# GuoYi0/alphaFive

Hardware: AMD Instinct MI355X
Metric: self-play moves/sec (11x11, 500 sims/move) (higher is better)
Workload: dtype f32 (fp16x2 split operands: 3 fp16 MFMA products per MAC, fp32 accumulate)

## Files before the change

alphafive_amd/csrc/af_conv_f16s.h:

```cpp
#ifndef AF_CONV_F16S_H
#define AF_CONV_F16S_H

#include <hip/hip_runtime.h>

#include <map>
#include <string>
#include <vector>

struct f16s_net;

int f16s_supported(int board_size);
int f16s_create(f16s_net** out, int board_size, int max_batch, int device, const std::map<std::string, std::vector<float>>& vars);
void f16s_destroy(f16s_net* n);
int f16s_trunk(f16s_net* n, hipStream_t st, const float* planes_dev, int batch);
int f16s_value_branch(f16s_net* n, hipStream_t st, int batch, float* o3_dev, int WP, int PP, float* value);
int f16s_policy_branch(f16s_net* n, hipStream_t st, int batch, float* o5_dev, int WP, int PP, float* policy);
int f16s_small_branches_ok(const f16s_net* n, int batch);
int f16s_small_branches(f16s_net* n, hipStream_t st, int batch, float* value, float* policy);
int f16s_small_forward_ok(const f16s_net* n, int batch);
int f16s_small_forward(f16s_net* n, hipStream_t st, const float* planes_dev, int batch, float* value, float* policy);
int f16s_small_forward_error(f16s_net* n);
void f16s_set_ablation(f16s_net* n, int bits);
int f16s_read_activation(f16s_net* n, int which, int batch, float* host);

#endif
```

alphafive_amd/csrc/af_conv_f16s.hip:

```cpp
#include <hip/hip_runtime.h>
#include <stdint.h>
#include <stdio.h>
#include <stdlib.h>
#include <string.h>

#include <algorithm>
#include <atomic>
#include <cmath>
#include <map>
#include <string>
#include <vector>

#include "af_conv_f16s.h"

typedef _Float16 h8 __attribute__((ext_vector_type(8)));
typedef float f32x16 __attribute__((ext_vector_type(16)));
typedef float f32x4 __attribute__((ext_vector_type(4)));

#define FS_HIP_OK(x) do { hipError_t e_ = (x); if (e_ != hipSuccess) { fprintf(stderr, "[af_conv_f16s] %s failed: %s\n", #x, hipGetErrorString(e_)); return -2; } } while (0)

namespace {

template <int S_> struct Geo;
template <> struct Geo<11> {
// ... 92 lines not shown
}
__device__ __forceinline__ f32x2 elu2(f32x2 x) {
    const f32x2 t = x * 1.44269504088896341f;
    f32x2 e;
    e.x = fminf(fmaxf(__builtin_amdgcn_exp2f(t.x), 0.0f), 1.0f);
    e.y = fminf(fmaxf(__builtin_amdgcn_exp2f(t.y), 0.0f), 1.0f);
    const f32x2 em1 = e - 1.0f;
    return f32x2{fmaxf(x.x, em1.x), fmaxf(x.y, em1.y)};
}

#ifndef AF_F16S_XCD_SWIZZLE
#define AF_F16S_XCD_SWIZZLE 1
#endif
#ifdef AF_F16S_TIMING
__device__ unsigned long long g_f16s_cycles[10][512][4][9];
__device__ unsigned long long g_f16s_wall[10][512][2];
#define AF_T(var) const unsigned long long var = __builtin_readcyclecounter()
#define AF_TACC(slot, a, b) tacc[slot] += (b) - (a)
#else
#define AF_T(var)
#define AF_TACC(slot, a, b)
#endif

#ifdef AF_DF_TIMING
__device__ unsigned long long g_df_wall[256][5];
#define DF_T(i) if (threadIdx.x == 0 && blockIdx.x < 256) g_df_wall[blockIdx.x][i] = wall_clock64()
#else
#define DF_T(i)
#endif
__device__ __forceinline__ void df_signal(int* ctr) {
    DF_T(2);
    asm volatile("s_waitcnt vmcnt(0)" ::: "memory");
    __syncthreads();
    if (threadIdx.x == 0) __hip_atomic_fetch_add(ctr, 1, __ATOMIC_RELAXED, __HIP_MEMORY_SCOPE_AGENT);
    DF_T(3);
}
__device__ __forceinline__ void df_poll(const int* ctr, int need, int* err) {
    int it = 0;
    while (__hip_atomic_load(ctr, __ATOMIC_RELAXED, __HIP_MEMORY_SCOPE_AGENT) < need) {
        __builtin_amdgcn_s_sleep(2);
        if (++it > (1 << 22)) { __hip_atomic_store(err, 1, __ATOMIC_RELAXED, __HIP_MEMORY_SCOPE_AGENT); break; }
    }
}
__device__ __forceinline__ void df_wait_one(const int* ctr, int need, int* err) {
    if (threadIdx.x == 0) df_poll(ctr, need, err);
    DF_T(1);
    __syncthreads();
}
__device__ __forceinline__ void df_wait_inv(const int* ctr, int need, int* err) {
    if (threadIdx.x == 0) {
        df_poll(ctr, need, err);
        __builtin_amdgcn_fence(__ATOMIC_ACQUIRE, "agent");
    }
    DF_T(1);
    __syncthreads();
}

struct F16sArgs {
    const char* in;
    const char* in2;
    const uint4* w;
    const float* bias;
    char* out;
    float* out32;
    float inv_scale;
    const uint4* pw;
    float* pbuf;
    float inv_scale_p;
    const uint4* hw;
    const float* hbias;
    char* hx;
    float inv_scale_h;
    int batch, WP, PP;
    const uint4* w2;
    const float* bias2;
    float inv_scale2;
    int gx0;
    char* stash;
    const int* df_wait;
    int df_need;
    int* df_done;
    int* df_err;
    int abl;
};

template <class G, int NSM, int NSP, int CT, int KS, int PS, bool OUT32, bool XACC, int PJ, int HD, int DIST, int WPE, int NTW, int HSEL, int FU = 0, int DF = 0>
__device__ __forceinline__ void f16s_body(const F16sArgs& A, char* smem, const int bx, const int gxw, const int tb = 0,
                                          const int by = (int)blockIdx.y, const int gy = (int)gridDim.y) {
    using L = Lay<G>;
    constexpr uint32_t kRowH = L::kRowH, kHalfH = L::kHalfH, kSlabH = L::kSlabH, kRowL = L::kRowL, kHalfL = L::kHalfL, kSlotL = L::kSlotL;
    constexpr uint32_t kZoff = Lds<G, DIST>::kZoff, kBiasOff = Lds<G, DIST>::kBiasOff, kScrOff = Lds<G, DIST>::kScrOff;
    constexpr int kDist = DIST, kRing = DIST + 2;
    constexpr int NPC = G::NPC, HV = G::HALVES;
    static_assert(FU == 0 || (G::HALVES == 1 && PJ == 1 && HD == 0 && !OUT32 && NSP == 0 && CT == 1 && HSEL < 0 &&
                              ((KS == 1 && NTW == 1) || (KS == 2 && NTW == 2))), "fused block: see above");
    constexpr uint32_t kScrBytes = KS == 2 ? (uint32_t)(CT * PS * NTW) * 4096u * (PJ == 1 ? 2u : 1u) : 0u;
    constexpr uint32_t kGOff = Lds<G, DIST>::kScrOff;
    constexpr uint32_t kW2Off = kGOff + (kScrBytes > Lay<G>::kSlotL ? kScrBytes : Lay<G>::kSlotL);
    constexpr int NT = NTW;
    static_assert(HSEL < 0 || (HV == 2 && PJ == 0 && HD == 0 && !OUT32), "half classes: plain 15x15 layers only");
    static_assert(NT % KS == 0 || PJ == 0, "an odd tile count under a k-split has no projection exchange");
    constexpr int C16 = 2 / KS;
    constexpr int ITP = C16, ITM = 9 * C16;
    constexpr int NIT = NSP * ITP + NSM * ITM;
    constexpr int SPP = NSP + NSM;
    constexpr int NFIN = NT / KS;
    static_assert(CT * KS * PS == 4 && NT >= KS, "4 waves");
    static_assert(PJ == 0 || NSP == 0, "a producer / consumer of the separate projection has no projection slabs");
    constexpr int NPW = PJ == 1 ? NSM * C16 : 0;
    static_assert(NPC * (DIST > 1 ? DIST - 1 : 1) < 64, "vmcnt is a 6-bit field");
    static_assert(DIST >= 2 || (NSP == 0 && ITM - 1 >= NPC), "distance 1: a slab's pieces must all be issued before its predecessor's last item");
    const int lane = threadIdx.x & 63, kg = lane >> 5, nn = lane & 31;
    const int wv = __builtin_amdgcn_readfirstlane((int)(threadIdx.x >> 6));
    const int ct = wv % CT, ks = (wv / CT) % KS, ps = wv / (CT * KS);
    const int rot = KS == 2 ? ks * ((NT + 1) / 2) : 0;
#define AF_OWN(jj) (KS == 1 || (jj) < NT / 2 || ((jj) < (NT + 1) / 2 && ks == 0))
    const int ctg = by * CT + ct, nso = gy * CT;
    const uint32_t lds = (uint32_t)(uintptr_t)smem;

    const int nq = HSEL >= 0 ? A.batch : A.batch * HV;
    int qpos = bx;
    if (AF_F16S_XCD_SWIZZLE && (gxw & (8 * (HSEL >= 0 ? 1 : HV) - 1)) == 0) qpos = (bx >> 3) + (gxw >> 3) * (bx & 7);
    if (qpos >= nq) return;
    const int hv = HSEL >= 0 ? HSEL : (HV == 1 ? 0 : qpos % HV);
    const uint32_t wsrc = G::wbase(hv) * 16u;
    AF_T(t_entry);
#ifdef AF_F16S_TIMING
    const unsigned long long wall_entry = wall_clock64();
#endif

    auto slab_src = [&](int qq, int j) -> const char* {
        const int p_ = (HV == 1 || HSEL >= 0) ? qq : qq / HV;
        const int p = (A.abl & 0x1000) ? (p_ & 127) : p_;
        return (j < NSM ? A.in + ((size_t)p * NSM + j) * kSlabH : A.in2 + ((size_t)p * NSP + (j - NSM)) * kSlabH) + wsrc;
    };
    auto dma_piece = [&](const char* src, uint32_t slot_off, int k) {
        const int piece = wv + 4 * k, row = piece / G::PR;
        const uint32_t su = G::seg_unit(piece % G::PR) * 16u;
        const uint32_t offh = (uint32_t)(row >> 2) * kHalfH + (uint32_t)(row & 3) * kRowH + su;
        const uint32_t offl = (uint32_t)(row >> 2) * kHalfL + (uint32_t)(row & 3) * kRowL + su;
        if (DF != 0) glds16_sc1(src + offh + lane * 16, (uint32_t)__builtin_amdgcn_readfirstlane((int)(lds + kLds0 + slot_off + offl)));
        else glds16(src + offh + lane * 16, (uint32_t)__builtin_amdgcn_readfirstlane((int)(lds + kLds0 + slot_off + offl)));
    };
    const int q0 = qpos;
    auto stream_src = [&](uint32_t idx) -> const char* {
        const int p = q0 + (int)(idx / SPP) * gxw, j = (int)(idx % SPP);
        return slab_src(p, j);
    };
    const uint32_t nslabs = (uint32_t)((nq - q0 + gxw - 1) / gxw) * SPP;

    if (DF == 0) {
#pragma unroll
        for (int d = 0; d < kDist; ++d) {
            if ((uint32_t)d < nslabs) {
#pragma unroll
                for (int k = 0; k < NPC; ++k) dma_piece(stream_src(d), (uint32_t)d * kSlotL, k);
            }
        }
    }

    h8 W[2 * NIT];
    {
        const uint4* wp = A.w + ((size_t)(ctg * KS + ks) * (2 * NIT)) * 64 + lane;
#pragma unroll
        for (int f = 0; f < 2 * NIT; ++f) {
            const uint4 v = wp[f * 64];
            __builtin_memcpy(&W[f], &v, 16);
        }
    }
    h8 PW[PJ == 1 ? 2 * NPW : 1];
    if (PJ == 1) {
        const uint4* wp = A.pw + ((size_t)(ctg * KS + ks) * (2 * NPW)) * 64 + lane;
#pragma unroll
        for (int f = 0; f < 2 * NPW; ++f) {
            const uint4 v = wp[f * 64];
            __builtin_memcpy(&PW[f], &v, 16);
        }
    }
    constexpr int HDS = HD > 0 ? HD : FU;
    h8 HA[HDS > 0 ? 4 : 1];
    float hb[HDS > 0 ? 8 : 1];
    if (FU > 0) {
        const uint4* w2 = A.w2;
#pragma unroll
        for (int i = 0; i < 9; ++i) *reinterpret_cast<uint4*>(smem + kW2Off + (uint32_t)(i * 256 + (int)threadIdx.x) * 16u) = w2[i * 256 + threadIdx.x];
        if (threadIdx.x < 32) reinterpret_cast<float*>(smem + kBiasOff + 256u)[threadIdx.x] = A.bias2[threadIdx.x];
        if (KS == 1) {
            for (uint32_t u = threadIdx.x; u < kSlotL / 16; u += 256) *reinterpret_cast<uint4*>(smem + kGOff + u * 16) = uint4{0, 0, 0, 0};
        }
    }
    if (HDS > 0) {
#pragma unroll
        for (int f = 0; f < 4; ++f) {
            const uint4 v = A.hw[f * 64 + lane];
            __builtin_memcpy(&HA[f], &v, 16);
        }
#pragma unroll
        for (int r = 0; r < 8; ++r) hb[r] = A.hbias[8 * kg + r];
    }
    if (threadIdx.x < kLds0 / 16) *reinterpret_cast<uint4*>(smem + threadIdx.x * 16) = uint4{0, 0, 0, 0};
    if (G::PADL + G::PADR > 0) {
        static_assert(G::PADL + G::PADR == 0 || (G::PADL == 8 && G::PADR == 8), "pad zeroing is written for 8 + 8 units");
        for (uint32_t u = threadIdx.x; u < (uint32_t)kRing * 128u; u += 256) {
            const uint32_t off = kLds0 + (u >> 7) * kSlotL + ((u >> 4) & 7u) * kRowL + (((u >> 3) & 1u) ? (G::WINU - 8u) * 16u : 0u) + (u & 7u) * 16u;
            *reinterpret_cast<uint4*>(smem + off) = uint4{0, 0, 0, 0};
        }
    }
    for (uint32_t u = threadIdx.x; u < kSlotL / 16; u += 256) *reinterpret_cast<uint4*>(smem + kZoff + u * 16) = uint4{0, 0, 0, 0};
    if (threadIdx.x < CT * 32) reinterpret_cast<float*>(smem + kBiasOff)[threadIdx.x] = A.bias[by * CT * 32 + threadIdx.x];
    uint32_t lb[NT], zb[NT];
    int pix[NT];
    bool ok[NT], edgeL[NT], edgeR[NT];
#pragma unroll
    for (int jj = 0; jj < NT; ++jj) {
        const int n = 128 * hv + 32 * (tb + ps * NT + ((jj + rot) % NT)) + nn;
        ok[jj] = n < G::NPIX;
        const int nc = ok[jj] ? n : 128 * hv;
        pix[jj] = nc;
        const int x = nc % G::S;
        edgeL[jj] = x == 0; edgeR[jj] = x == G::S - 1;
        lb[jj] = kLds0 + (uint32_t)((KS == 2 ? 2 * ks : 0) + kg) * kRowL + (uint32_t)((nc + G::POFF - G::S - 1 - (int)G::wbase(hv)) * 16);
        zb[jj] = kZoff + (lb[jj] & 255u);
    }
    constexpr int kAccRegs = 16 * NT * (1 + (XACC ? 1 : 0) + (PJ == 1 ? 1 : 0));
    constexpr int kWRegs = 4 * (2 * NIT + (PJ == 1 ? 2 * NPW : 0) + (HDS > 0 ? 4 : 0));
    constexpr int kNAmax = (256 - kAccRegs - 16) / 4, kNAwant = (kWRegs - AF_F16S_VW + 3) / 4;
    constexpr int NA = (AF_F16S_APIN && WPE == 1 && kNAwant > 0) ? (kNAwant < kNAmax ? kNAwant : kNAmax) : 0;
#pragma unroll
    for (int f = 0; f < 2 * NIT; ++f) {
        if (f < 2 * NIT - NA) asm volatile("" : "+v"(W[f]));
        else asm volatile("" : "+a"(W[f]));
    }
// ... 16 lines not shown
        }
    }
    asm volatile("s_waitcnt vmcnt(0) lgkmcnt(0)" ::: "memory");
    __builtin_amdgcn_s_barrier();
    AF_T(t_ready);

    auto rd = [](const char* sm, bool proj, int it, int p, uint32_t c_, uint32_t l_, uint32_t r_) -> h8 {
        const int c = proj ? it : it / 9, tap = proj ? 4 : it % 9, ky = tap / 3, kx = tap % 3;
        const uint32_t base = kx == 0 ? l_ : (kx == 2 ? r_ : c_);
        const uint32_t imm = (uint32_t)p * kHalfL + (KS == 1 ? 2u * c * kRowL : 0u) + (uint32_t)(ky * G::S + kx) * 16u;
        return *reinterpret_cast<const h8*>(sm + base + imm);
    };

    auto head_tile = [&](const float (&v)[16], const int jj, const int pos) {
      if constexpr (HDS > 0) {
        h8 bh[2], bl[2];
#pragma unroll
        for (int st_ = 0; st_ < 2; ++st_)
#pragma unroll
            for (int e = 0; e < 8; ++e) {
                const float f = v[8 * st_ + e];
                const _Float16 h = (_Float16)f;
                bh[st_][e] = h;
                bl[st_][e] = (_Float16)(f - (float)h);
            }
        f32x16 a2;
#pragma unroll
        for (int r = 0; r < 16; ++r) a2[r] = 0.0f;
#pragma unroll
        for (int st_ = 0; st_ < 2; ++st_) {
            a2 = __builtin_amdgcn_mfma_f32_32x32x16_f16(HA[2 * st_], bh[st_], a2, 0, 0, 0);
            a2 = __builtin_amdgcn_mfma_f32_32x32x16_f16(HA[2 * st_], bl[st_], a2, 0, 0, 0);
            a2 = __builtin_amdgcn_mfma_f32_32x32x16_f16(HA[2 * st_ + 1], bh[st_], a2, 0, 0, 0);
        }
        constexpr int NR = HDS == 1 ? 4 : 8;
        _Float16 uh[8], ul[8];
#pragma unroll
        for (int r = 0; r < NR; ++r) {
            const float f = elu1(a2[r] * A.inv_scale_h + hb[r]);
            const _Float16 h = (_Float16)f;
            uh[r] = h;
            ul[r] = (_Float16)(f - (float)h);
        }
        if (ok[jj] && !(A.abl & 2)) {
            if (HDS == 1) {
                if (kg == 0) {
                    typedef _Float16 h4 __attribute__((ext_vector_type(4)));
                    char* o = A.hx + (size_t)pos * Hx<G>::kValPos + (uint32_t)pix[jj] * 8u;
                    if (DF != 0) {
                        st8_sc1(o, h4{uh[0], uh[1], uh[2], uh[3]});
                        st8_sc1(o + Hx<G>::kValLo, h4{ul[0], ul[1], ul[2], ul[3]});
                    } else {
                        *reinterpret_cast<h4*>(o) = h4{uh[0], uh[1], uh[2], uh[3]};
                        *reinterpret_cast<h4*>(o + Hx<G>::kValLo) = h4{ul[0], ul[1], ul[2], ul[3]};
                    }
                }
            } else {
                char* o = A.hx + (size_t)pos * Hx<G>::kPolPos + (uint32_t)pix[jj] * 32u + (uint32_t)kg * 16u;
                if (DF != 0) {
                    st16_sc1(o, h8{uh[0], uh[1], uh[2], uh[3], uh[4], uh[5], uh[6], uh[7]});
                    st16_sc1(o + Hx<G>::kPolLo, h8{ul[0], ul[1], ul[2], ul[3], ul[4], ul[5], ul[6], ul[7]});
                } else {
                    *reinterpret_cast<h8*>(o) = h8{uh[0], uh[1], uh[2], uh[3], uh[4], uh[5], uh[6], uh[7]};
                    *reinterpret_cast<h8*>(o + Hx<G>::kPolLo) = h8{ul[0], ul[1], ul[2], ul[3], ul[4], ul[5], ul[6], ul[7]};
                }
            }
        }
      }
    };
    uint32_t t = 0;
    uint32_t cur = 0u, nxd = (uint32_t)kDist * kSlotL;
    constexpr bool XPOS = !(NT >= 3 && NIT >= 36) && FU == 0;
    h8 fr[2][NT][2];
#define AF_FIRST_ITEM(slot)                                                                                      \
    _Pragma("unroll") for (int jj = 0; jj < NT; ++jj) {                                                          \
        const uint32_t c_ = (AF_F16S_ZPAD && !ok[jj]) ? zb[jj] : lb[jj] + (slot), l_ = edgeL[jj] ? zb[jj] : c_, r_ = edgeR[jj] ? zb[jj] : c_; \
        fr[0][jj][0] = rd(smem, false, 0, 0, c_, l_, r_);                                                        \
        fr[0][jj][1] = rd(smem, false, 0, 1, c_, l_, r_);                                                        \
    }
    if (XPOS) { AF_FIRST_ITEM(0u) }
#ifdef AF_F16S_TIMING
    unsigned long long tacc[8] = {0, 0, 0, 0, 0, 0, 0, 0};
#endif
    for (; qpos < nq; qpos += gxw) {
        const int pos = (HV == 1 || HSEL >= 0) ? qpos : qpos / HV;
        AF_T(tp0);
        if (!XPOS) { AF_FIRST_ITEM(cur) }
#undef AF_FIRST_ITEM
        f32x16 acc[NT], acx[XACC ? NT : 1], pac[PJ == 1 ? NT : 1];
#pragma unroll
        for (int jj = 0; jj < NT; ++jj)
#pragma unroll
            for (int r = 0; r < 16; ++r) { acc[jj][r] = 0.0f; if (XACC) acx[jj][r] = 0.0f; if (PJ == 1) pac[jj][r] = 0.0f; }
        f32x4 padd[PJ == 2 ? NFIN : 1][4];
        if (PJ == 2) {
#pragma unroll
            for (int jf = 0; jf < NFIN; ++jf) {
                const int tile = tb + ps * NT + (KS == 2 ? ks * NFIN : 0) + jf;
                const f32x4* src = reinterpret_cast<const f32x4*>(A.pbuf) + ((((size_t)qpos * nso + ctg) * 4 + tile) * 4) * 64 + lane;
#pragma unroll
                for (int q = 0; q < 4; ++q) padd[jf][q] = src[q * 64];
            }
        }

#pragma clang loop unroll(full)
        for (int j = 0; j < SPP; ++j) {
            const bool proj = j >= NSM;
            const bool nproj = (j + 1) % SPP >= NSM;
            const int ms = j, pslab = j - NSM;
            const int NI = proj ? ITP : ITM;
            const int ibase = proj ? pslab * ITP : NSP * ITP + ms * ITM;
            const int seq = proj ? NSM * ITM + pslab * ITP : ms * ITM;
            const int npos = qpos + ((j + kDist) / SPP) * gxw;
            const bool more = npos < nq && !(A.abl & 1);
            const char* nsrc = slab_src((A.abl & 4) ? q0 : (more ? npos : qpos), (j + kDist) % SPP);
            const uint32_t nx1 = cur + kSlotL == kRing * kSlotL ? 0u : cur + kSlotL;
            uint32_t bC[NT], bL[NT], bR[NT];
#pragma unroll
            for (int jj = 0; jj < NT; ++jj) {
                bC[jj] = (AF_F16S_ZPAD && !ok[jj]) ? zb[jj] : lb[jj] + cur;
                bL[jj] = edgeL[jj] ? zb[jj] : bC[jj];
                bR[jj] = edgeR[jj] ? zb[jj] : bC[jj];
            }
            if (HSEL == 1 && wv == (j & 3) && by == 0 && lane < 32) {
                const uint32_t u = (uint32_t)(lane & 3), un = (u < 2 ? 128u + u : 141u + u);
                const uint4 q = *reinterpret_cast<const uint4*>(smem + kLds0 + cur + (uint32_t)(lane >> 4) * kHalfL + (uint32_t)((lane >> 2) & 3) * kRowL + un * 16u);
                *reinterpret_cast<uint4*>(A.stash + (((size_t)pos * SPP + j) * 32 + lane) * 16) = q;
            }
#pragma clang loop unroll(full)
            for (int it = 0; it < NI; ++it) {
                const int b = (seq + it) & 1;
                if (it + 1 < NI) {
#pragma unroll
                    for (int jj = 0; jj < NT; ++jj) {
                        fr[b ^ 1][jj][0] = rd(smem, proj, it + 1, 0, bC[jj], bL[jj], bR[jj]);
                        fr[b ^ 1][jj][1] = rd(smem, proj, it + 1, 1, bC[jj], bL[jj], bR[jj]);
                    }
                } else {
                    const int issued = NI - 1 < NPC ? NI - 1 : NPC;
                    AF_T(tw0);
                    if (more) {
                        wait_vmcnt(NPC * (kDist - 2) + issued);
                    } else {
                        asm volatile("s_waitcnt vmcnt(0)" ::: "memory");
                    }
                    AF_T(tw1);
                    __builtin_amdgcn_s_barrier();
                    AF_T(tw2);
                    AF_TACC(1, tw0, tw1);
                    AF_TACC(2, tw1, tw2);
                    if ((XPOS || j + 1 < SPP) && t + 1 < nslabs) {
#pragma unroll
                        for (int jj = 0; jj < NT; ++jj) {
                            const uint32_t c_ = (AF_F16S_ZPAD && !ok[jj]) ? zb[jj] : lb[jj] + nx1, l_ = edgeL[jj] ? zb[jj] : c_, r_ = edgeR[jj] ? zb[jj] : c_;
                            fr[b ^ 1][jj][0] = rd(smem, nproj, 0, 0, c_, l_, r_);
                            fr[b ^ 1][jj][1] = rd(smem, nproj, 0, 1, c_, l_, r_);
                        }
                    }
                }
                const h8 wh = W[2 * (ibase + it)], wl = W[2 * (ibase + it) + 1];
#pragma unroll
                for (int jj = 0; jj < NT; ++jj) acc[jj] = __builtin_amdgcn_mfma_f32_32x32x16_f16(wh, fr[b][jj][0], acc[jj], 0, 0, 0);
                if (XACC) {
#pragma unroll
                    for (int jj = 0; jj < NT; ++jj) acx[jj] = __builtin_amdgcn_mfma_f32_32x32x16_f16(wh, fr[b][jj][1], acx[jj], 0, 0, 0);
#pragma unroll
                    for (int jj = 0; jj < NT; ++jj) acx[jj] = __builtin_amdgcn_mfma_f32_32x32x16_f16(wl, fr[b][jj][0], acx[jj], 0, 0, 0);
                } else {
#pragma unroll
                    for (int jj = 0; jj < NT; ++jj) acc[jj] = __builtin_amdgcn_mfma_f32_32x32x16_f16(wh, fr[b][jj][1], acc[jj], 0, 0, 0);
#pragma unroll
                    for (int jj = 0; jj < NT; ++jj) acc[jj] = __builtin_amdgcn_mfma_f32_32x32x16_f16(wl, fr[b][jj][0], acc[jj], 0, 0, 0);
                }
                if (PJ == 1 && !proj && it % 9 == 4) {
                    const int pi = ms * C16 + it / 9;
                    const h8 ph = PW[2 * pi], pl = PW[2 * pi + 1];
#pragma unroll
                    for (int jj = 0; jj < NT; ++jj) pac[jj] = __builtin_amdgcn_mfma_f32_32x32x16_f16(ph, fr[b][jj][0], pac[jj], 0, 0, 0);
#pragma unroll
                    for (int jj = 0; jj < NT; ++jj) pac[jj] = __builtin_amdgcn_mfma_f32_32x32x16_f16(ph, fr[b][jj][1], pac[jj], 0, 0, 0);
#pragma unroll
                    for (int jj = 0; jj < NT; ++jj) pac[jj] = __builtin_amdgcn_mfma_f32_32x32x16_f16(pl, fr[b][jj][0], pac[jj], 0, 0, 0);
                }
#pragma unroll
                for (int q = 0; q < 2 * NT; ++q) {
                    __builtin_amdgcn_sched_group_barrier(0x008, 1, 0);
                    __builtin_amdgcn_sched_group_barrier(0x100, 1, 0);
                }
                __builtin_amdgcn_sched_group_barrier(0x008, NT, 0);
                if (more) {
                    if (it < NI - 1 && it < NPC) dma_piece(nsrc, nxd, it);
                    if (it == NI - 1) {
#pragma unroll
                        for (int k = (NI - 1 < NPC ? NI - 1 : NPC); k < NPC; ++k) dma_piece(nsrc, nxd, k);
                    }
                }
            }
// ... 163 lines not shown
            {
                const f32x4* bp = reinterpret_cast<const f32x4*>(smem + kBiasOff + 256u + (uint32_t)(16 * kg) * 4u);
#pragma unroll
                for (int q = 0; q < 4; ++q) { const f32x4 v = bp[q]; bs2[4 * q] = v[0]; bs2[4 * q + 1] = v[1]; bs2[4 * q + 2] = v[2]; bs2[4 * q + 3] = v[3]; }
            }
#pragma unroll
            for (int r = 0; r < 16; r += 2) {
                f32x2 pre = f32x2{a2[r], a2[r + 1]} * A.inv_scale2 + f32x2{bs2[r], bs2[r + 1]};
                pre += f32x2{pj[r], pj[r + 1]};
                const f32x2 y = elu2(pre);
                v2[r] = y.x; v2[r + 1] = y.y;
            }
            head_tile(v2, 0, pos);
        }
#ifdef AF_F16S_TIMING
        {
            AF_T(tp3);
            tacc[3] += tp2 - tp1; tacc[4] += tp3 - tp2; tacc[5] += tp3 - tp0; tacc[6] += 1;
        }
#endif
    }
    if (DF != 0) df_signal(A.df_done + q0);
#ifdef AF_F16S_TIMING
    if (lane == 0) {
        tacc[0] = tacc[5] - tacc[1] - tacc[2] - tacc[3] - tacc[4];
        const int layer = (A.abl >> 8) & 15;
        for (int q = 0; q < 8; ++q) g_f16s_cycles[layer][blockIdx.x + 256 * blockIdx.y][wv][q] = tacc[q];
        g_f16s_cycles[layer][blockIdx.x + 256 * blockIdx.y][wv][8] = t_ready - t_entry;
        if (wv == 0) { g_f16s_wall[layer][blockIdx.x + 256 * blockIdx.y][0] = wall_entry; g_f16s_wall[layer][blockIdx.x + 256 * blockIdx.y][1] = wall_clock64(); }
    }
#endif
#undef AF_OWN
}

template <class G, int NSM, int NSP, int CT, int KS, int PS, bool OUT32, bool XACC, int PJ, int HD, int DIST = kDist, int WPE = 1>
__global__ __launch_bounds__(256, WPE) __attribute__((amdgpu_waves_per_eu(WPE, WPE))) void af_conv_f16s(F16sArgs A) {
    extern __shared__ __attribute__((aligned(16))) char smem[];
    f16s_body<G, NSM, NSP, CT, KS, PS, OUT32, XACC, PJ, HD, DIST, WPE, 4 / PS, -1>(A, smem, (int)blockIdx.x, (int)gridDim.x);
}

template <class G, int NSM, int KS, int PS, bool XACC, int FU, int DIST>
__global__ __launch_bounds__(256, 1) __attribute__((amdgpu_waves_per_eu(1, 1))) void af_block_f16s(F16sArgs A) {
    extern __shared__ __attribute__((aligned(16))) char smem[];
    f16s_body<G, NSM, 0, 1, KS, PS, false, XACC, 1, 0, DIST, 1, 4 / PS, -1, FU>(A, smem, (int)blockIdx.x, (int)gridDim.x);
}

template <class G>
__global__ __launch_bounds__(256, 1) __attribute__((amdgpu_waves_per_eu(1, 1))) void af_small_pair_f16s(F16sArgs P, F16sArgs V) {
    extern __shared__ __attribute__((aligned(16))) char smem[];
    const int nb = P.batch, id = (int)blockIdx.x;
    if (id < 2 * nb) f16s_body<G, 4, 0, 2, 2, 1, false, false, 0, 0, kDist, 1, 2, -1>(P, smem, id % nb, nb, (id / nb) * 2);
    else f16s_body<G, 4, 0, 1, 2, 2, false, false, 1, 0, 2, 1, 2, -1, 1>(V, smem, id - 2 * nb, nb);
}

template <class G>
__global__ __launch_bounds__(256, 1) __attribute__((amdgpu_waves_per_eu(1, 1))) void af_big_pair_f16s(F16sArgs P, F16sArgs V) {
    extern __shared__ __attribute__((aligned(16))) char smem[];
    const int gp = P.gx0, id = (int)blockIdx.x;
    if (id < gp) f16s_body<G, 4, 0, 2, 2, 1, false, false, 0, 0, kDist, 1, 4, -1>(P, smem, id, gp);
    else f16s_body<G, 4, 0, 1, 2, 2, false, false, 1, 0, 2, 1, 2, -1, 1>(V, smem, id - gp, (int)gridDim.x - gp);
}

template <class G, int NSM, int NSP, int CT, int KS, int PS, bool OUT32, bool XACC, int PJ, int HD, int DIST, int WPE, int NTW>
__global__ __launch_bounds__(256, WPE) __attribute__((amdgpu_waves_per_eu(WPE, WPE))) void af_conv_f16s_sb(F16sArgs A) {
    extern __shared__ __attribute__((aligned(16))) char smem[];
    f16s_body<G, NSM, NSP, CT, KS, PS, OUT32, XACC, PJ, HD, DIST, WPE, NTW, -1>(A, smem, (int)blockIdx.x, (int)gridDim.x, (int)blockIdx.z * PS * NTW);
}

template <class G, int NSM, int NSP, int CT, int KS, bool XACC>
__global__ __launch_bounds__(256, 1) __attribute__((amdgpu_waves_per_eu(1, 1))) void af_conv_f16s_h15(F16sArgs A) {
    extern __shared__ __attribute__((aligned(16))) char smem[];
    const int gx0 = A.gx0;
    if ((int)blockIdx.x < gx0) f16s_body<G, NSM, NSP, CT, KS, 1, false, XACC, 0, 0, kDist, 1, 4, 0>(A, smem, (int)blockIdx.x, gx0);
    else f16s_body<G, NSM, NSP, CT, KS, 1, false, XACC, 0, 0, kDist, 1, 3, 1>(A, smem, (int)blockIdx.x - gx0, (int)gridDim.x - gx0);
}

struct CornerArgs {
    const char* stash;
    const uint4* w;
    const float* bias;
    char* out;
    float inv_scale;
    int batch, NCT;
};
template <class G, int KS, bool XACC, int NSM, int NSP>
__global__ __launch_bounds__(256) void af_corner_f16s(CornerArgs A) {
    using L = Lay<G>;
    constexpr int CPIX = G::NPIX - 1;
    constexpr int C16 = 2 / KS, NIT = NSP * C16 + NSM * 9 * C16;
    constexpr int NST = NSM * 8 + NSP * 2;
    constexpr int D = NST < 12 ? NST : 12;
    const int lane = threadIdx.x & 63, kg = lane >> 5, nn = lane & 31;
    const int tile = (int)blockIdx.y * 4 + (int)(threadIdx.x >> 6);
    if (tile >= A.NCT) return;
    const int p = 32 * (int)blockIdx.x + nn;
    const bool valid = p < A.batch;
    const size_t pc = (size_t)(valid ? p : A.batch - 1);
    f32x16 acc[KS], acx[XACC ? KS : 1];
#pragma unroll
    for (int h = 0; h < KS; ++h)
#pragma unroll
        for (int r = 0; r < 16; ++r) { acc[h][r] = 0.0f; if (XACC) acx[h][r] = 0.0f; }
    const uint4* const wbase = A.w + (size_t)tile * KS * NIT * 2 * 64 + lane;
    constexpr int SPP = NSM + NSP;
    const char* const st0 = A.stash + (pc * SPP * 32 + (uint32_t)kg * 4u) * 16;
    struct Ops { uint4 a0, a1, b0, b1; };
    auto half_of = [](int t) constexpr -> int {
        const int k16 = t < NSM * 8 ? (t >> 2) & 1 : (t - NSM * 8) & 1;
        return KS == 2 ? k16 : 0;
    };
    auto fetch = [&](int t) -> Ops {
        int k16, item;
        const char* bsrc;
        if (t < NSM * 8) {
            const int s_ = t >> 3, tq = t & 3, ky = tq >> 1, kx = tq & 1;
            k16 = (t >> 2) & 1;
            item = NSP * C16 + s_ * 9 * C16 + (KS == 2 ? 0 : k16) * 9 + 3 * ky + kx;
            bsrc = st0 + (uint32_t)((s_ * 32 + 2 * k16 * 4 + tq) * 16);
        } else {
            const int u = t - NSM * 8, s_ = u >> 1;
            k16 = u & 1;
            item = s_ * C16 + (KS == 2 ? 0 : k16);
            bsrc = st0 + (uint32_t)(((NSM + s_) * 32 + 2 * k16 * 4 + 3) * 16);
        }
        const uint4* wp = wbase + ((size_t)((KS == 2 ? k16 : 0) * NIT + item) * 2) * 64;
        Ops o;
        o.a0 = wp[0]; o.a1 = wp[64];
        o.b0 = *reinterpret_cast<const uint4*>(bsrc); o.b1 = *reinterpret_cast<const uint4*>(bsrc + 256);
        return o;
    };
    Ops ring[D];
#pragma unroll
    for (int t = 0; t < D; ++t) ring[t] = fetch(t);
    __builtin_amdgcn_sched_barrier(0);
#pragma unroll
    for (int t = 0; t < NST; ++t) {
        const Ops o = ring[t % D];
        if (t + D < NST) ring[t % D] = fetch(t + D);
        const int h = half_of(t);
        h8 wh, wl, bh, bl;
        __builtin_memcpy(&wh, &o.a0, 16); __builtin_memcpy(&wl, &o.a1, 16); __builtin_memcpy(&bh, &o.b0, 16); __builtin_memcpy(&bl, &o.b1, 16);
        acc[h] = __builtin_amdgcn_mfma_f32_32x32x16_f16(wh, bh, acc[h], 0, 0, 0);
        if (XACC) {
            acx[h] = __builtin_amdgcn_mfma_f32_32x32x16_f16(wh, bl, acx[h], 0, 0, 0);
            acx[h] = __builtin_amdgcn_mfma_f32_32x32x16_f16(wl, bh, acx[h], 0, 0, 0);
        } else {
            acc[h] = __builtin_amdgcn_mfma_f32_32x32x16_f16(wh, bl, acc[h], 0, 0, 0);
            acc[h] = __builtin_amdgcn_mfma_f32_32x32x16_f16(wl, bh, acc[h], 0, 0, 0);
        }
        __builtin_amdgcn_sched_group_barrier(0x008, 3, 0);
        __builtin_amdgcn_sched_group_barrier(0x020, 4, 0);
    }
    if (XACC) {
#pragma unroll
        for (int h = 0; h < KS; ++h)
#pragma unroll
            for (int r = 0; r < 16; ++r) acc[h][r] += acx[h][r];
    }
    if (KS == 2) {
#pragma unroll
        for (int r = 0; r < 16; ++r) acc[0][r] = acc[KS - 1][r] + acc[0][r];
    }
    if (!valid) return;
    float v[16];
#pragma unroll
    for (int r = 0; r < 16; r += 2) {
        const f32x2 pre = f32x2{acc[0][r], acc[0][r + 1]} * A.inv_scale + f32x2{A.bias[32 * tile + 16 * kg + r], A.bias[32 * tile + 16 * kg + r + 1]};
        const f32x2 y = elu2(pre);
        v[r] = y.x; v[r + 1] = y.y;
    }
    char* o = A.out + ((size_t)p * A.NCT + tile) * L::kSlabH + (uint32_t)(2 * kg) * L::kRowH + (uint32_t)(CPIX + G::POFF) * 16u;
#pragma unroll
    for (int hf = 0; hf < 2; ++hf) {
        h8 hi, lo;
#pragma unroll
        for (int e = 0; e < 8; ++e) {
            const float f = v[8 * hf + e];
            const _Float16 h = (_Float16)f;
            hi[e] = h;
            lo[e] = (_Float16)(f - (float)h);
        }
        st16(o + hf * L::kRowH, hi);
        st16(o + hf * L::kRowH + L::kHalfH, lo);
    }
}

template <class G>
__global__ __launch_bounds__(256) void af_stem_f16s(const float* __restrict__ planes, const float* __restrict__ w,
                                                    const float* __restrict__ bias, char* __restrict__ out, int batch) {
    constexpr int S = G::S, NPIX = G::NPIX, SP = S + 4;
    constexpr uint32_t kRowH = Lay<G>::kRowH, kHalfH = Lay<G>::kHalfH, kSlabH = Lay<G>::kSlabH;
    __shared__ float sx[3 * SP * SP];
    __shared__ float sw[75 * 32];
    __shared__ float sb[32];
    const int t = threadIdx.x;
    for (int i = t; i < 75 * 32; i += 256) sw[i] = w[i];
    if (t < 32) sb[t] = bias[t];
    for (int i = t; i < 3 * SP * SP; i += 256) sx[i] = 0.0f;
    for (int b = blockIdx.x; b < batch; b += gridDim.x) {
        __syncthreads();
        for (int i = t; i < 3 * NPIX; i += 256) {
            const int c = i / NPIX, p = i - c * NPIX, y = p / S, x = p - y * S;
            sx[c * SP * SP + (y + 2) * SP + x + 2] = planes[(size_t)b * 3 * NPIX + i];
        }
        __syncthreads();
        if (t < NPIX) {
            const int y = t / S, x = t - y * S;
            float acc[32];
#pragma unroll
            for (int co = 0; co < 32; ++co) acc[co] = sb[co];
            for (int ky = 0; ky < 5; ++ky)
                for (int kx = 0; kx < 5; ++kx)
#pragma unroll
                    for (int c = 0; c < 3; ++c) {
                        const float xv = sx[c * SP * SP + (y + ky) * SP + x + kx];
                        const float* wr = sw + ((ky * 5 + kx) * 3 + c) * 32;
#pragma unroll
                        for (int co = 0; co < 32; ++co) acc[co] = fmaf(xv, wr[co], acc[co]);
                    }
            char* o = out + (size_t)b * kSlabH + (uint32_t)(t + G::POFF) * 16u;
#pragma unroll
            for (int u = 0; u < 4; ++u) {
                h8 hi, lo;
#pragma unroll
                for (int e = 0; e < 8; ++e) {
                    const float f = elu1(acc[8 * u + e]);
                    const _Float16 h = (_Float16)f;
                    hi[e] = h;
                    lo[e] = (_Float16)(f - (float)h);
                }
                *reinterpret_cast<h8*>(o + u * kRowH) = hi;
                *reinterpret_cast<h8*>(o + u * kRowH + kHalfH) = lo;
            }
        }
    }
}

template <class G> struct StemLds {
    static constexpr int SR = G::S + 4, IW = G::S + 5;
    static constexpr int kEnt = 3 * SR * G::S + 1, kImg = 3 * SR * IW;
    static constexpr uint32_t kImgOff = (uint32_t)((kEnt * 16 + 255) / 256 * 256), kBytes = kImgOff + (uint32_t)kImg * 2u;
};
template <class G, bool SC1 = false>
__device__ __forceinline__ void f16s_stem_body(const float* __restrict__ planes, const uint4* __restrict__ w ,
                                               const float* __restrict__ bias, float inv_scale, char* __restrict__ out, int batch,
                                               const int bx, const int gx, uint4* ent, _Float16* img) {
    constexpr int S = G::S, NPIX = G::NPIX, SR = S + 4, IW = S + 5;
    constexpr int NPL = 3 * NPIX, NLD = (NPL + 255) / 256;
    constexpr int NTL = (NPIX + 31) / 32, NRND = (NTL + 3) / 4;
    constexpr uint32_t kRowH = Lay<G>::kRowH, kHalfH = Lay<G>::kHalfH, kSlabH = Lay<G>::kSlabH;
    const int lane = threadIdx.x & 63, kg = lane >> 5, nn = lane & 31;
    const int wv = __builtin_amdgcn_readfirstlane((int)(threadIdx.x >> 6));
    h8 W[16];
#pragma unroll
    for (int f = 0; f < 16; ++f) {
        const uint4 v = w[f * 64 + lane];
        __builtin_memcpy(&W[f], &v, 16);
    }
    float bs[16];
#pragma unroll
    for (int r = 0; r < 16; ++r) bs[r] = bias[16 * kg + r];
    for (int i = threadIdx.x; i < 3 * SR * IW; i += 256) img[i] = (_Float16)0.0f;
    auto img_at = [](int i) -> int { const int c = i / NPIX, p = i - c * NPIX, y = p / S, x = p - y * S; return (c * SR + y + 2) * IW + x + 2; };
    int at[NLD];
    float nx[NLD];
#pragma unroll
    for (int q = 0; q < NLD; ++q) {
        const int i = (int)threadIdx.x + 256 * q;
        at[q] = img_at(i < NPL ? i : 0);
        nx[q] = 0.0f;
        if (i < NPL && bx < batch) nx[q] = planes[(size_t)bx * NPL + i];
    }
    for (int pos = bx; pos < batch; pos += gx) {
        __syncthreads();
#pragma unroll
        for (int q = 0; q < NLD; ++q)
            if ((int)threadIdx.x + 256 * q < NPL) img[at[q]] = (_Float16)nx[q];
        if (pos + gx < batch) {
            const float* pl = planes + (size_t)(pos + gx) * NPL;
#pragma unroll
            for (int q = 0; q < NLD; ++q)
                if ((int)threadIdx.x + 256 * q < NPL) nx[q] = pl[threadIdx.x + 256 * q];
        }
        __syncthreads();
        for (int en = threadIdx.x; en < 3 * SR * S; en += 256) {
            const int cin = en / (SR * S), rem = en - cin * SR * S, yy = rem / S, x = rem - yy * S;
            const _Float16* src = img + (cin * SR + yy) * IW + x;
            const h8 v = {src[0], src[1], src[2], src[3], src[4], 0, 0, 0};
            __builtin_memcpy(&ent[en], &v, 16);
        }
        __syncthreads();
#pragma unroll
        for (int rd_ = 0; rd_ < NRND; ++rd_) {
            const int n = 32 * (wv + 4 * rd_) + nn;
            const bool ok = n < NPIX;
            const int nc = ok ? n : 0;
            if (32 * (wv + 4 * rd_) >= NPIX) continue;
            f32x16 acc;
#pragma unroll
            for (int r = 0; r < 16; ++r) acc[r] = 0.0f;
#pragma unroll
            for (int s_ = 0; s_ < 8; ++s_) {
                const int ga = 2 * s_, gb = 2 * s_ + 1 < 15 ? 2 * s_ + 1 : 0;
                const uint32_t offa = (uint32_t)((ga / 5) * SR + ga % 5) * S, offb = (uint32_t)((gb / 5) * SR + gb % 5) * S;
                h8 b;
                __builtin_memcpy(&b, &ent[(uint32_t)nc + (kg ? offb : offa)], 16);
                acc = __builtin_amdgcn_mfma_f32_32x32x16_f16(W[2 * s_], b, acc, 0, 0, 0);
                acc = __builtin_amdgcn_mfma_f32_32x32x16_f16(W[2 * s_ + 1], b, acc, 0, 0, 0);
            }
            char* o = out + (size_t)pos * kSlabH + (uint32_t)(2 * kg) * kRowH + (uint32_t)(nc + G::POFF) * 16u;
#pragma unroll
            for (int hf = 0; hf < 2; ++hf) {
                h8 hi, lo;
#pragma unroll
                for (int e = 0; e < 8; ++e) {
                    const float f = elu1(acc[8 * hf + e] * inv_scale + bs[8 * hf + e]);
                    const _Float16 h = (_Float16)f;
                    hi[e] = h;
                    lo[e] = (_Float16)(f - (float)h);
                }
                if (ok) {
                    if (SC1) { st16_sc1(o + hf * kRowH, hi); st16_sc1(o + hf * kRowH + kHalfH, lo); }
                    else {
                        *reinterpret_cast<h8*>(o + hf * kRowH) = hi;
                        *reinterpret_cast<h8*>(o + hf * kRowH + kHalfH) = lo;
                    }
                }
            }
        }
    }
}

template <class G>
__global__ __launch_bounds__(256) void af_stem_mfma_f16s(const float* __restrict__ planes, const uint4* __restrict__ w, const float* __restrict__ bias,
                                                         float inv_scale, char* __restrict__ out, int batch) {
    __shared__ __attribute__((aligned(16))) uint4 ent[StemLds<G>::kEnt];
    __shared__ _Float16 img[StemLds<G>::kImg];
    f16s_stem_body<G>(planes, w, bias, inv_scale, out, batch, (int)blockIdx.x, (int)gridDim.x, ent, img);
}

template <class G>
__device__ __forceinline__ void f16s_vfc_body(const char* __restrict__ xv, const uint4* __restrict__ a, const float* __restrict__ b1,
                                              const float* __restrict__ w2, const float* __restrict__ b2, float inv_scale,
                                              float* __restrict__ value, int batch, const int bx) {
    __shared__ float red[2][32];
    constexpr int NS = Hx<G>::VSTEPS;
    const bool act = threadIdx.x < 128;
    const int lane = threadIdx.x & 63, mt = (threadIdx.x >> 6) & 1, n = lane & 31, kg = lane >> 5;
    const int pos = bx * 32 + n, posc = pos < batch ? pos : batch - 1;
    const char* xb = xv + (size_t)posc * Hx<G>::kValPos + (uint32_t)kg * 16u;
    const uint4* ap = a + (size_t)mt * 128 + lane;
    f32x16 acc;
#pragma unroll
    for (int r = 0; r < 16; ++r) acc[r] = 0.0f;
#pragma unroll
    for (int half = 0; half < (NS + 15) / 16; ++half) {
        uint4 bh[16], bl[16], ah[16], al[16];
#pragma unroll
        for (int q = 0; q < 16; ++q) {
            const int s_ = 16 * half + q;
            if (s_ < NS) {
                bh[q] = *reinterpret_cast<const uint4*>(xb + s_ * 32);
                bl[q] = *reinterpret_cast<const uint4*>(xb + Hx<G>::kValLo + s_ * 32);
                ah[q] = ap[(size_t)s_ * 256];
                al[q] = ap[(size_t)s_ * 256 + 64];
            }
        }
        typedef uint32_t u32x4 __attribute__((ext_vector_type(4)));
#pragma unroll
        for (int q = 0; q < 16; ++q) {
            if (16 * half + q < NS) {
                u32x4 t0, t1, t2, t3;
                __builtin_memcpy(&t0, &bh[q], 16); __builtin_memcpy(&t1, &bl[q], 16); __builtin_memcpy(&t2, &ah[q], 16); __builtin_memcpy(&t3, &al[q], 16);
                asm volatile("" : "+v"(t0), "+v"(t1), "+v"(t2), "+v"(t3));
                __builtin_memcpy(&bh[q], &t0, 16); __builtin_memcpy(&bl[q], &t1, 16); __builtin_memcpy(&ah[q], &t2, 16); __builtin_memcpy(&al[q], &t3, 16);
            }
        }
#pragma unroll
        for (int q = 0; q < 16; ++q) {
            if (16 * half + q < NS) {
                h8 xh, xl, wh, wl;
                __builtin_memcpy(&xh, &bh[q], 16); __builtin_memcpy(&xl, &bl[q], 16);
                __builtin_memcpy(&wh, &ah[q], 16); __builtin_memcpy(&wl, &al[q], 16);
                acc = __builtin_amdgcn_mfma_f32_32x32x16_f16(wh, xh, acc, 0, 0, 0);
                acc = __builtin_amdgcn_mfma_f32_32x32x16_f16(wh, xl, acc, 0, 0, 0);
                acc = __builtin_amdgcn_mfma_f32_32x32x16_f16(wl, xh, acc, 0, 0, 0);
            }
        }
    }
    float part = 0.0f;
#pragma unroll
    for (int r = 0; r < 16; ++r) {
        const int j = 32 * mt + 16 * kg + r;
        part += elu1(acc[r] * inv_scale + b1[j]) * w2[j];
    }
    part += __shfl_xor(part, 32);
    if (act && kg == 0) red[mt][n] = part;
    __syncthreads();
    if (act && mt == 0 && kg == 0 && pos < batch) value[pos] = tanhf((red[0][n] + red[1][n] + b2[0]) * 0.5f);
}
template <class G>
__global__ __launch_bounds__(128) __attribute__((amdgpu_waves_per_eu(1, 2))) void af_value_fc_f16s(
    const char* __restrict__ xv, const uint4* __restrict__ a , const float* __restrict__ b1, const float* __restrict__ w2,
    const float* __restrict__ b2, float inv_scale, float* __restrict__ value, int batch) {
    f16s_vfc_body<G>(xv, a, b1, w2, b2, inv_scale, value, batch, (int)blockIdx.x);
}
struct VfcArgs { const char* xv; const uint4* a; const float *b1, *w2, *b2; float inv_scale; float* value; };
template <class G>
__global__ __launch_bounds__(256, 1) __attribute__((amdgpu_waves_per_eu(1, 1))) void af_small_l7v_f16s(F16sArgs P, VfcArgs V) {
    extern __shared__ __attribute__((aligned(16))) char smem[];
    const int nb = P.batch, id = (int)blockIdx.x;
    if (id < 2 * nb) f16s_body<G, 2, 4, 2, 2, 1, false, true, 0, 0, kDist, 1, 2, -1>(P, smem, id % nb, nb, (id / nb) * 2);
    else f16s_vfc_body<G>(V.xv, V.a, V.b1, V.w2, V.b2, V.inv_scale, V.value, nb, id - 2 * nb);
}
template <class G>
__global__ __launch_bounds__(256, 1) __attribute__((amdgpu_waves_per_eu(1, 1))) void af_big_l7v_f16s(F16sArgs P, VfcArgs V) {
    extern __shared__ __attribute__((aligned(16))) char smem[];
    const int gp = P.gx0, id = (int)blockIdx.x;
    if (id < gp) f16s_body<G, 2, 4, 2, 2, 1, false, true, 0, 0, kDist, 1, 4, -1>(P, smem, id, gp);
    else f16s_vfc_body<G>(V.xv, V.a, V.b1, V.w2, V.b2, V.inv_scale, V.value, P.batch, id - gp);
}
// ... 412 lines not shown
int launch_cfg(hipStream_t st, const F16sArgs& a, int gy, int ncu) {
    constexpr int NT = 4 / PS;
    constexpr size_t lds = Lds<G, DIST>::kScrOff + (KS == 2 ? (size_t)CT * PS * NT * 4096 * (PJ == 1 ? 2 : 1) : 0);
    static_assert(WPE * lds <= 160 * 1024, "LDS budget of the workgroups sharing a CU");
#ifndef AF_F16S_NO_LDS_ASSERT
    static_assert(lds <= 160 * 1024, "LDS budget");
#endif
    static std::atomic<uint64_t> attr_devs{0};
    int dev = 0;
    FS_HIP_OK(hipGetDevice(&dev));
    const uint64_t bit = 1ull << (dev & 63);
    if (!(attr_devs.load(std::memory_order_relaxed) & bit)) {
        FS_HIP_OK(hipFuncSetAttribute(reinterpret_cast<const void*>(af_conv_f16s<G, NSM, NSP, CT, KS, PS, OUT32, XACC, PJ, HD, DIST, WPE>),
                                      hipFuncAttributeMaxDynamicSharedMemorySize, 160 * 1024));
        attr_devs.fetch_or(bit, std::memory_order_relaxed);
    }
    constexpr int NTS = KS == 2 ? 2 : 1;
    if constexpr (NTS < NT && HD == 0) {
        if (a.batch <= kSmallBatch && !(a.abl & 128)) {
            static std::atomic<uint64_t> attr_sb{0};
            if (!(attr_sb.load(std::memory_order_relaxed) & bit)) {
                FS_HIP_OK(hipFuncSetAttribute(reinterpret_cast<const void*>(af_conv_f16s_sb<G, NSM, NSP, CT, KS, PS, OUT32, XACC, PJ, HD, DIST, WPE, NTS>),
                                              hipFuncAttributeMaxDynamicSharedMemorySize, 160 * 1024));
                attr_sb.fetch_or(bit, std::memory_order_relaxed);
            }
            hipLaunchKernelGGL((af_conv_f16s_sb<G, NSM, NSP, CT, KS, PS, OUT32, XACC, PJ, HD, DIST, WPE, NTS>),
                               dim3(a.batch * G::HALVES, gy, NT / NTS), dim3(256), lds, st, a);
            FS_HIP_OK(hipGetLastError());
            return 0;
        }
    }
    int gx = std::max(1, std::min(a.batch * G::HALVES, WPE * ncu / gy));
    gx = std::max(G::HALVES, gx / G::HALVES * G::HALVES);
    hipLaunchKernelGGL((af_conv_f16s<G, NSM, NSP, CT, KS, PS, OUT32, XACC, PJ, HD, DIST, WPE>), dim3(gx, gy), dim3(256), lds, st, a);
    FS_HIP_OK(hipGetLastError());
    return 0;
}

template <class G, int NSM, int KS, int PS, bool XACC, int FU>
int launch_block(hipStream_t st, const F16sArgs& a, int ncu) {
    constexpr int DIST = 2;
    constexpr size_t scr = KS == 2 ? (size_t)PS * (4 / PS) * 4096 * 2 : 0;
    constexpr size_t lds = Lds<G, DIST>::kScrOff + (scr > Lay<G>::kSlotL ? scr : Lay<G>::kSlotL) + 36864;
    static_assert(lds <= 160 * 1024, "LDS budget of the fused block");
    static std::atomic<uint64_t> attr_devs{0};
    int dev = 0;
    FS_HIP_OK(hipGetDevice(&dev));
    const uint64_t bit = 1ull << (dev & 63);
    if (!(attr_devs.load(std::memory_order_relaxed) & bit)) {
        FS_HIP_OK(hipFuncSetAttribute(reinterpret_cast<const void*>(af_block_f16s<G, NSM, KS, PS, XACC, FU, DIST>),
                                      hipFuncAttributeMaxDynamicSharedMemorySize, 160 * 1024));
        attr_devs.fetch_or(bit, std::memory_order_relaxed);
    }
    const int gx = std::max(1, std::min(a.batch, ncu));
    hipLaunchKernelGGL((af_block_f16s<G, NSM, KS, PS, XACC, FU, DIST>), dim3(gx), dim3(256), lds, st, a);
    FS_HIP_OK(hipGetLastError());
    return 0;
}

template <class G, int NSM, int NSP, int CT, int KS, bool XACC>
int launch_h15(hipStream_t st, F16sArgs a, int gy, int ncu) {
    constexpr size_t lds = Lds<G, kDist>::kScrOff + (KS == 2 ? (size_t)CT * 4 * 4096 : 0);
    static_assert(lds <= 160 * 1024, "LDS budget");
    static std::atomic<uint64_t> attr_devs{0};
    int dev = 0;
    FS_HIP_OK(hipGetDevice(&dev));
    const uint64_t bit = 1ull << (dev & 63);
    if (!(attr_devs.load(std::memory_order_relaxed) & bit)) {
        FS_HIP_OK(hipFuncSetAttribute(reinterpret_cast<const void*>(af_conv_f16s_h15<G, NSM, NSP, CT, KS, XACC>),
                                      hipFuncAttributeMaxDynamicSharedMemorySize, 160 * 1024));
        attr_devs.fetch_or(bit, std::memory_order_relaxed);
    }
    const int gx = std::max(16, ncu / gy / 16 * 16);
    static const int num1 = [] { const char* e = getenv("AF_F16S_H15_NUM1"); const int v = e ? atoi(e) : 0; return v > 0 && v < 32 ? v : 18; }();
    static const int num2 = [] { const char* e = getenv("AF_F16S_H15_NUM2"); const int v = e ? atoi(e) : 0; return v > 0 && v < 32 ? v : 17; }();
    static const int rnd = [] { const char* e = getenv("AF_F16S_H15_ROUND"); return e ? atoi(e) : 1; }();
    const int num = KS == 1 ? num1 : num2;
    a.gx0 = rnd ? std::max(8, (gx * num / 32 + 4) / 8 * 8) : std::max(1, gx * num / 32);
    if (a.gx0 >= gx) a.gx0 = gx - 8;
    hipLaunchKernelGGL((af_conv_f16s_h15<G, NSM, NSP, CT, KS, XACC>), dim3(gx, gy), dim3(256), lds, st, a);
    FS_HIP_OK(hipGetLastError());
    CornerArgs c;
    c.stash = a.stash; c.w = a.w; c.bias = a.bias; c.out = a.out; c.inv_scale = a.inv_scale;
    c.batch = a.batch; c.NCT = gy * CT;
    hipLaunchKernelGGL((af_corner_f16s<G, KS, XACC, NSM, NSP>), dim3((a.batch + 31) / 32, (c.NCT + 3) / 4), dim3(256), 0, st, c);
    FS_HIP_OK(hipGetLastError());
    return 0;
}

}

struct f16s_net {
    int S = 11;
    int max_batch = 0, device = 0, ncu = 256;
    std::vector<void*> allocs;
    float *stem_w = nullptr, *stem_b = nullptr;
    uint4* stem_wm = nullptr;
    float stem_inv_scale = 1.0f;
    uint4* w[10] = {};
    uint4* pw[10] = {};
    float* pbuf[5] = {};
    float* bias[10] = {};
    float inv_scale[10] = {}, inv_scale_p[10] = {};
    char *f0 = nullptr, *g[5] = {}, *o[5] = {};
    uint4 *hcw[2] = {}, *hfw[2] = {};
    float *hcb[2] = {}, *hfb[2] = {}, *v2w = nullptr, *v2b = nullptr;
    float hc_inv[2] = {}, hf_inv[2] = {};
    char* hx[2] = {};
    int* df = nullptr;
    float* pfx = nullptr;
    char* stash = nullptr;
    int abl = 0;
};

int f16s_supported(int board_size) { return board_size == 11 || board_size == 15; }

int f16s_create(f16s_net** out, int board_size, int max_batch, int device, const std::map<std::string, std::vector<float>>& V) {
    if (!f16s_supported(board_size)) return -1;
    FS_HIP_OK(hipSetDevice(device));
    f16s_net* n = new f16s_net();
    n->S = board_size; n->max_batch = max_batch; n->device = device;
    const bool s11 = board_size == 11;
    const int halves = s11 ? 1 : 2;
    const size_t slab_bytes = s11 ? Lay<Geo<11>>::kSlabH : Lay<Geo<15>>::kSlabH;
    FS_HIP_OK(hipDeviceGetAttribute(&n->ncu, hipDeviceAttributeMultiprocessorCount, device));
    if (const char* e = getenv("AF_F16S_NCU")) {
        const int v = atoi(e);
        if (v >= 8 && v <= n->ncu) n->ncu = v / 8 * 8;
    }
    int rc = 0;
    auto get = [&](const std::string& k) -> const std::vector<float>& { return V.at(k); };
    rc = dev_upload(n->allocs, &n->stem_w, get("bone/conv1/kernel").data(), 75 * 32 * 4);
    if (!rc) rc = dev_upload(n->allocs, &n->stem_b, get("bone/conv1/bias").data(), 32 * 4);
    if (!rc) {
        const std::vector<float>& ks = get("bone/conv1/kernel");
        const float sc = pick_scale(ks, nullptr);
        std::vector<_Float16> pk((size_t)8 * 2 * 64 * 8, (_Float16)0.0f);
        for (int s_ = 0; s_ < 8; ++s_)
            for (int lane = 0; lane < 64; ++lane)
                for (int e = 0; e < 5; ++e) {
                    const int m = lane & 31, g = 2 * s_ + (lane >> 5);
                    if (g >= 15) continue;
                    const int co = 16 * ((m >> 2) & 1) + 8 * (m >> 4) + 4 * ((m >> 3) & 1) + (m & 3), cin = g / 5, ky = g % 5;
                    const float v = ks[(size_t)((ky * 5 + e) * 3 + cin) * 32 + co] * sc;
                    const _Float16 h = (_Float16)v;
                    pk[(((size_t)s_ * 2 + 0) * 64 + lane) * 8 + e] = h;
                    pk[(((size_t)s_ * 2 + 1) * 64 + lane) * 8 + e] = (_Float16)(v - (float)h);
                }
        rc = dev_upload(n->allocs, &n->stem_wm, pk.data(), pk.size() * 2);
        n->stem_inv_scale = 1.0f / sc;
    }
    for (int b = 0; b < 5 && !rc; ++b) {
        const std::string s = kBlockNames[b];
        const std::vector<float>&k1 = get(s + "_conv1/kernel"), &k2 = get(s + "_conv2/kernel"), &kr = get(s + "_res/kernel");
        const LayerCfg &L1 = kLayers[2 * b], &L2 = kLayers[2 * b + 1];
        const bool split_proj = L1.pj == 1;
        const float s1 = pick_scale(k1, nullptr), s2 = pick_scale(k2, split_proj ? nullptr : &kr);
        const std::vector<_Float16> p1 = pack_layer(L1, k1.data(), nullptr, s1), p2 = pack_layer(L2, k2.data(), kr.data(), s2);
        rc = dev_upload(n->allocs, &n->w[2 * b], p1.data(), p1.size() * 2);
        if (!rc && split_proj) {
            const float sp = pick_scale(kr, nullptr);
            const std::vector<_Float16> pp = pack_proj(L1, L2.cout, kr.data(), sp);
            rc = dev_upload(n->allocs, &n->pw[2 * b], pp.data(), pp.size() * 2);
            n->inv_scale_p[2 * b] = 1.0f / sp;
            void* q = nullptr;
            const size_t bytes = (size_t)max_batch * halves * (L2.cout / 32) * 4 * 4 * 64 * 16;
            if (!rc) { FS_HIP_OK(hipMalloc(&q, bytes)); n->allocs.push_back(q); n->pbuf[b] = (float*)q; }
        }

        if (!rc) rc = dev_upload(n->allocs, &n->w[2 * b + 1], p2.data(), p2.size() * 2);
        std::vector<float> bsum(get(s + "_conv2/bias"));
        for (size_t i = 0; i < bsum.size(); ++i) bsum[i] += get(s + "_res/bias")[i];
        if (!rc) rc = dev_upload(n->allocs, &n->bias[2 * b], get(s + "_conv1/bias").data(), L1.cout * 4);
        if (!rc) rc = dev_upload(n->allocs, &n->bias[2 * b + 1], bsum.data(), L2.cout * 4);
        n->inv_scale[2 * b] = 1.0f / s1; n->inv_scale[2 * b + 1] = 1.0f / s2;
    }
    auto act = [&](char** p, int ch) -> int {
        void* q = nullptr;
        const size_t bytes = (size_t)max_batch * (ch / 32) * slab_bytes;
        FS_HIP_OK(hipMalloc(&q, bytes));
        FS_HIP_OK(hipMemset(q, 0, bytes));
        n->allocs.push_back(q);
        *p = (char*)q;
        return 0;
    };
    if (!rc && !s11) {
        void* q = nullptr;
        FS_HIP_OK(hipMalloc(&q, (size_t)max_batch * 6 * 512));
        n->allocs.push_back(q);
        n->stash = (char*)q;
    }
    if (!rc) {
        void* q = nullptr;
        FS_HIP_OK(hipMalloc(&q, kDfWords * sizeof(int)));
        FS_HIP_OK(hipMemset(q, 0, kDfWords * sizeof(int)));
        n->allocs.push_back(q);
        n->df = (int*)q;
        FS_HIP_OK(hipMalloc(&q, 4 * 4 * 64 * 16));
        n->allocs.push_back(q);
        n->pfx = (float*)q;
    }
    if (!rc) rc = act(&n->f0, 32);
    for (int b = 0; b < 5 && !rc; ++b) {
        rc = act(&n->g[b], kLayers[2 * b].cout);
        if (!rc && b != 2 && b != 4) rc = act(&n->o[b], kLayers[2 * b + 1].cout);
    }
    if (!rc) {
        const int npix = board_size * board_size, hxp = 128 * halves, vsteps = (npix + 3) / 4, nlt = (npix + 31) / 32;
        const char* cname[2] = {"value/conv", "policy/conv"};
        const int nco[2] = {4, 16};
        for (int h = 0; h < 2 && !rc; ++h) {
            const std::vector<float>& wc = get(std::string(cname[h]) + "/kernel");
            const float sc = pick_scale(wc, nullptr);
            const int NC = nco[h];
            const std::vector<_Float16> pk = pack_frags(2, [&](int st_, int lane, int e) -> float {
                const int m = lane & 31, co = m < 16 ? 8 * ((m >> 2) & 1) + 4 * (m >> 3) + (m & 3) : 99, ci = 16 * (lane >> 5) + 8 * st_ + e;
                return co < NC ? wc[(size_t)ci * NC + co] * sc : 0.0f;
            });
            rc = dev_upload(n->allocs, &n->hcw[h], pk.data(), pk.size() * 2);
            std::vector<float> bpad(16, 0.0f);
            const std::vector<float>& bc = get(std::string(cname[h]) + "/bias");
            for (int i = 0; i < NC; ++i) bpad[i] = bc[i];
            if (!rc) rc = dev_upload(n->allocs, &n->hcb[h], bpad.data(), 64);
            n->hc_inv[h] = 1.0f / sc;
            void* q = nullptr;
            const size_t bytes = (size_t)max_batch * hxp * (h == 0 ? 16 : 64);
            if (!rc) { FS_HIP_OK(hipMalloc(&q, bytes)); FS_HIP_OK(hipMemset(q, 0, bytes)); n->allocs.push_back(q); n->hx[h] = (char*)q; }
        }
        if (!rc) {
            const std::vector<float>& w1 = get("value/fc1/kernel");
            const float sc = pick_scale(w1, nullptr);
            const std::vector<_Float16> pk = pack_frags(vsteps * 2, [&](int f, int lane, int e) -> float {
                const int s_ = f >> 1, mt = f & 1, px = 4 * s_ + 2 * (lane >> 5) + (e >> 2), ch = e & 3, j = 32 * mt + row_perm(lane & 31);
                return px < npix ? w1[(size_t)(ch * npix + px) * 64 + j] * sc : 0.0f;
            });
            rc = dev_upload(n->allocs, &n->hfw[0], pk.data(), pk.size() * 2);
            n->hf_inv[0] = 1.0f / sc;
            if (!rc) rc = dev_upload(n->allocs, &n->hfb[0], get("value/fc1/bias").data(), 64 * 4);
            if (!rc) rc = dev_upload(n->allocs, &n->v2w, get("value/fc2/kernel").data(), 64 * 4);
            if (!rc) rc = dev_upload(n->allocs, &n->v2b, get("value/fc2/bias").data(), 4);
        }
        if (!rc) {
            const std::vector<float>& wf = get("policy/fc/kernel");
            const float sc = pick_scale(wf, nullptr);
            const std::vector<_Float16> pk = pack_frags(npix * nlt, [&](int f, int lane, int e) -> float {
                const int px = f / nlt, mt = f % nlt, c16 = 8 * (lane >> 5) + e, j = 32 * mt + row_perm(lane & 31);
                return j < npix ? wf[(size_t)(c16 * npix + px) * npix + j] * sc : 0.0f;
            });
            rc = dev_upload(n->allocs, &n->hfw[1], pk.data(), pk.size() * 2);
            n->hf_inv[1] = 1.0f / sc;
            if (!rc) rc = dev_upload(n->allocs, &n->hfb[1], get("policy/fc/bias").data(), npix * 4);
        }
        if (!rc) FS_HIP_OK(hipFuncSetAttribute(reinterpret_cast<const void*>(af_policy_fc_f16s<Geo<11>>), hipFuncAttributeMaxDynamicSharedMemorySize, (int)kPfLds));
        if (!rc) FS_HIP_OK(hipFuncSetAttribute(reinterpret_cast<const void*>(af_policy_fc_f16s<Geo<15>>), hipFuncAttributeMaxDynamicSharedMemorySize, (int)kPfLds));
    }
    if (rc) { f16s_destroy(n); return rc; }
    *out = n;
    return 0;
}

void f16s_destroy(f16s_net* n) {
    if (!n) return;
    (void)hipSetDevice(n->device);
    for (void* p : n->allocs) (void)hipFree(p);
    delete n;
}

void f16s_set_ablation(f16s_net* n, int bits) { if (n) n->abl = bits; }

template <class G>
static int launch_layer_g(f16s_net* n, hipStream_t st, int li, const F16sArgs& a, int head) {
    switch (li) {
        case 0:
            if constexpr (G::S == 11) { if (!(n->abl & 32)) return launch_cfg<G, 1, 0, 2, 1, 2, false, false, 0, 0, 1, 2>(st, a, 1, n->ncu); }
            return launch_cfg<G, 1, 0, 2, 1, 2, false, true>(st, a, 1, n->ncu);
        case 1: return launch_cfg<G, 2, 1, 2, 1, 2, false, true>(st, a, 1, n->ncu);
        case 2:
            if constexpr (G::S == 15) { if (!(n->abl & 64) && a.batch >= 128) return launch_h15<G, 2, 0, 4, 1, false>(st, a, 1, n->ncu); }
            return launch_cfg<G, 2, 0, 4, 1, 1, false, false>(st, a, 1, n->ncu);
        case 3:
            if constexpr (G::S == 15) { if (!(n->abl & 64) && a.batch >= 128) return launch_h15<G, 4, 2, 2, 2, false>(st, a, 2, n->ncu); }
            return launch_cfg<G, 4, 2, 2, 2, 1, false, false>(st, a, 2, n->ncu);
        case 4: return launch_cfg<G, 4, 0, 1, 2, 2, false, false, 1>(st, a, 1, n->ncu);
        case 5:
            if constexpr (G::S == 11) { if (head == 0 && !(n->abl & 32)) return launch_cfg<G, 1, 0, 1, 1, 4, true, true, 2, 1, 1, 2>(st, a, 1, n->ncu); }
            if (head == 0) return launch_cfg<G, 1, 0, 1, 1, 4, true, true, 2, 1>(st, a, 1, n->ncu);
            return launch_cfg<G, 1, 0, 1, 1, 4, true, true, 2>(st, a, 1, n->ncu);
        case 6:
            if constexpr (G::S == 15) { if (!(n->abl & 64) && a.batch >= 128) return launch_h15<G, 4, 0, 2, 2, false>(st, a, 1, n->ncu); }
            return launch_cfg<G, 4, 0, 2, 2, 1, false, false>(st, a, 1, n->ncu);
        case 7:
            if constexpr (G::S == 15) { if (!(n->abl & 64) && a.batch >= 128) return launch_h15<G, 2, 4, 2, 2, true>(st, a, 1, n->ncu); }
            return launch_cfg<G, 2, 4, 2, 2, 1, false, true>(st, a, 1, n->ncu);
        case 8: return launch_cfg<G, 2, 0, 1, 1, 4, false, true, 1>(st, a, 1, n->ncu);
        default:
            if constexpr (G::S == 11) { if (head == 1 && !(n->abl & 32)) return launch_cfg<G, 1, 0, 1, 1, 4, true, true, 2, 2, 1, 2>(st, a, 1, n->ncu); }
            if (head == 1) return launch_cfg<G, 1, 0, 1, 1, 4, true, true, 2, 2>(st, a, 1, n->ncu);
            return launch_cfg<G, 1, 0, 1, 1, 4, true, true, 2>(st, a, 1, n->ncu);
    }
}

static int launch_layer(f16s_net* n, hipStream_t st, int li, const char* in, const char* in2, char* out, float* out32, int batch,
                        int WP, int PP, int head = -1) {
    F16sArgs a;
    a.hw = nullptr; a.hbias = nullptr; a.hx = nullptr; a.inv_scale_h = 1.0f;
    if (head >= 0) { a.hw = n->hcw[head]; a.hbias = n->hcb[head]; a.hx = n->hx[head]; a.inv_scale_h = n->hc_inv[head]; }
    a.in = in; a.in2 = in2; a.w = n->w[li]; a.bias = n->bias[li]; a.out = out; a.out32 = out32;
    a.inv_scale = n->inv_scale[li]; a.batch = batch; a.WP = WP; a.PP = PP; a.abl = (n->abl & 0xf0ff) | (li << 8); a.gx0 = 0; a.stash = n->stash;
    {
        static const int mask = [] { const char* e = getenv("AF_F16S_ABL_LAYERS"); return e ? (int)strtol(e, nullptr, 0) : 0x3ff; }();
        if (!((mask >> li) & 1)) a.abl &= ~0x100f;
    }
    a.w2 = nullptr; a.bias2 = nullptr; a.inv_scale2 = 1.0f;
    a.pw = n->pw[li]; a.pbuf = n->pbuf[li / 2]; a.inv_scale_p = n->inv_scale_p[li];
    return n->S == 11 ? launch_layer_g<Geo<11>>(n, st, li, a, head) : launch_layer_g<Geo<15>>(n, st, li, a, head);
}

int f16s_trunk(f16s_net* n, hipStream_t st, const float* planes, int batch) {
    if (!n || batch < 1 || batch > n->max_batch) return -1;
    if (n->abl & 16) {
        if (n->S == 15) hipLaunchKernelGGL(af_stem_f16s<Geo<15>>, dim3(std::min(batch, 2048)), dim3(256), 0, st, planes, n->stem_w, n->stem_b, n->f0, batch);
        else hipLaunchKernelGGL(af_stem_f16s<Geo<11>>, dim3(std::min(batch, 2048)), dim3(256), 0, st, planes, n->stem_w, n->stem_b, n->f0, batch);
    } else if (n->S == 15) {
        hipLaunchKernelGGL(af_stem_mfma_f16s<Geo<15>>, dim3(std::min(batch, 1024)), dim3(256), 0, st, planes, n->stem_wm, n->stem_b, n->stem_inv_scale,
                           n->f0, batch);
    } else {
        hipLaunchKernelGGL(af_stem_mfma_f16s<Geo<11>>, dim3(std::min(batch, 1024)), dim3(256), 0, st, planes, n->stem_wm, n->stem_b, n->stem_inv_scale,
                           n->f0, batch);
    }
    int rc = launch_layer(n, st, 0, n->f0, nullptr, n->g[0], nullptr, batch, 0, 0);
    if (!rc) rc = launch_layer(n, st, 1, n->g[0], n->f0, n->o[0], nullptr, batch, 0, 0);
    if (!rc) rc = launch_layer(n, st, 2, n->o[0], nullptr, n->g[1], nullptr, batch, 0, 0);
    if (!rc) rc = launch_layer(n, st, 3, n->g[1], n->o[0], n->o[1], nullptr, batch, 0, 0);
    return rc;
}

static F16sArgs block_args(f16s_net* n, int li, const char* in, int batch, int head) {
    F16sArgs a;
    memset(&a, 0, sizeof(a));
    a.in = in; a.w = n->w[li]; a.bias = n->bias[li]; a.inv_scale = n->inv_scale[li];
    a.pw = n->pw[li]; a.inv_scale_p = n->inv_scale_p[li];
    a.w2 = n->w[li + 1]; a.bias2 = n->bias[li + 1]; a.inv_scale2 = n->inv_scale[li + 1];
    a.hw = n->hcw[head]; a.hbias = n->hcb[head]; a.hx = n->hx[head]; a.inv_scale_h = n->hc_inv[head];
    a.batch = batch; a.abl = (n->abl & 0xf0ff) | (li << 8); a.stash = n->stash;
    return a;
}

int f16s_value_branch(f16s_net* n, hipStream_t st, int batch, float* o3, int WP, int PP, float* value) {
    int rc;
    if (n->S == 11 && value && !(n->abl & 256)) {
        rc = launch_block<Geo<11>, 4, 2, 2, false, 1>(st, block_args(n, 4, n->o[1], batch, 0), n->ncu);
    } else {
        rc = launch_layer(n, st, 4, n->o[1], nullptr, n->g[2], nullptr, batch, 0, 0);
        if (!rc) rc = launch_layer(n, st, 5, n->g[2], n->o[1], nullptr, o3, batch, WP, PP, value ? 0 : -1);
    }
    if (!rc && value) {
        if (n->S == 11)
            hipLaunchKernelGGL(af_value_fc_f16s<Geo<11>>, dim3((batch + 31) / 32), dim3(128), 0, st, n->hx[0], n->hfw[0], n->hfb[0], n->v2w, n->v2b,
                               n->hf_inv[0], value, batch);
        else
            hipLaunchKernelGGL(af_value_fc_f16s<Geo<15>>, dim3((batch + 31) / 32), dim3(128), 0, st, n->hx[0], n->hfw[0], n->hfb[0], n->v2w, n->v2b,
                               n->hf_inv[0], value, batch);
    }
    return rc;
}

int f16s_policy_branch(f16s_net* n, hipStream_t st, int batch, float* o5, int WP, int PP, float* policy) {
    int rc = launch_layer(n, st, 6, n->o[1], nullptr, n->g[3], nullptr, batch, 0, 0);
    if (!rc) rc = launch_layer(n, st, 7, n->g[3], n->o[1], n->o[3], nullptr, batch, 0, 0);
    if (!rc && n->S == 11 && policy && !(n->abl & 256)) {
        rc = launch_block<Geo<11>, 2, 1, 4, true, 2>(st, block_args(n, 8, n->o[3], batch, 1), n->ncu);
    } else {
        if (!rc) rc = launch_layer(n, st, 8, n->o[3], nullptr, n->g[4], nullptr, batch, 0, 0);
        if (!rc) rc = launch_layer(n, st, 9, n->g[4], n->o[3], nullptr, o5, batch, WP, PP, policy ? 1 : -1);
    }
    if (!rc && policy) {
        if (n->S == 11)
            hipLaunchKernelGGL(af_policy_fc_f16s<Geo<11>>, dim3((batch + kPfPos - 1) / kPfPos), dim3(512), kPfLds, st, n->hx[1], n->hfw[1], n->hfb[1],
                               n->hf_inv[1], policy, batch);
        else
            hipLaunchKernelGGL(af_policy_fc_f16s<Geo<15>>, dim3((batch + kPfPos - 1) / kPfPos), dim3(512), kPfLds, st, n->hx[1], n->hfw[1], n->hfb[1],
                               n->hf_inv[1], policy, batch);
    }
    return rc;
}

int f16s_small_branches(f16s_net* n, hipStream_t st, int batch, float* value, float* policy) {
    if (!n || n->S != 11 || batch < 1 || !value || !policy) return -1;
    using G = Geo<11>;
    const bool small = batch <= kSmallBatch;
    F16sArgs P;
    memset(&P, 0, sizeof(P));
    P.in = n->o[1]; P.w = n->w[6]; P.bias = n->bias[6]; P.out = n->g[3]; P.inv_scale = n->inv_scale[6];
    P.batch = batch; P.abl = (n->abl & 0xf0ff) | (6 << 8); P.stash = n->stash; P.inv_scale2 = 1.0f; P.inv_scale_h = 1.0f;
    const F16sArgs V = block_args(n, 4, n->o[1], batch, 0);
    constexpr size_t ldsP = Lds<G, kDist>::kScrOff + (size_t)2 * 1 * 4 * 4096;
    constexpr size_t ldsV = Lds<G, 2>::kScrOff + (size_t)2 * 2 * 4096 * 2 + 36864;
    constexpr size_t lds = ldsP > ldsV ? ldsP : ldsV;
    static_assert(lds <= 160 * 1024, "LDS budget");
    static std::atomic<uint64_t> attr_devs{0};
    int dev = 0;
    FS_HIP_OK(hipGetDevice(&dev));
    const uint64_t bit = 1ull << (dev & 63);
    if (!(attr_devs.load(std::memory_order_relaxed) & bit)) {
        FS_HIP_OK(hipFuncSetAttribute(reinterpret_cast<const void*>(af_small_pair_f16s<G>), hipFuncAttributeMaxDynamicSharedMemorySize, 160 * 1024));
        FS_HIP_OK(hipFuncSetAttribute(reinterpret_cast<const void*>(af_big_pair_f16s<G>), hipFuncAttributeMaxDynamicSharedMemorySize, 160 * 1024));
        attr_devs.fetch_or(bit, std::memory_order_relaxed);
    }
    const int gp = std::max(1, std::min(batch, n->ncu));
    if (small) {
        hipLaunchKernelGGL(af_small_pair_f16s<G>, dim3(3 * batch), dim3(256), lds, st, P, V);
    } else {
        P.gx0 = gp;
        hipLaunchKernelGGL(af_big_pair_f16s<G>, dim3(2 * gp), dim3(256), lds, st, P, V);
    }
    FS_HIP_OK(hipGetLastError());
    {
        F16sArgs Q;
        memset(&Q, 0, sizeof(Q));
        Q.in = n->g[3]; Q.in2 = n->o[1]; Q.w = n->w[7]; Q.bias = n->bias[7]; Q.out = n->o[3]; Q.inv_scale = n->inv_scale[7];
        Q.batch = batch; Q.abl = (n->abl & 0xf0ff) | (7 << 8); Q.stash = n->stash; Q.inv_scale2 = 1.0f; Q.inv_scale_h = 1.0f;
        const VfcArgs F = {n->hx[0], n->hfw[0], n->hfb[0], n->v2w, n->v2b, n->hf_inv[0], value};
        constexpr size_t lds7 = Lds<G, kDist>::kScrOff + (size_t)2 * 1 * 4 * 4096;
        static std::atomic<uint64_t> attr7{0};
        if (!(attr7.load(std::memory_order_relaxed) & bit)) {
            FS_HIP_OK(hipFuncSetAttribute(reinterpret_cast<const void*>(af_small_l7v_f16s<G>), hipFuncAttributeMaxDynamicSharedMemorySize, (int)lds7));
            FS_HIP_OK(hipFuncSetAttribute(reinterpret_cast<const void*>(af_big_l7v_f16s<G>), hipFuncAttributeMaxDynamicSharedMemorySize, (int)lds7));
            attr7.fetch_or(bit, std::memory_order_relaxed);
        }
        if (small) {
            hipLaunchKernelGGL(af_small_l7v_f16s<G>, dim3(2 * batch + 1), dim3(256), lds7, st, Q, F);
        } else {
            Q.gx0 = gp;
            hipLaunchKernelGGL(af_big_l7v_f16s<G>, dim3(gp + (batch + 31) / 32), dim3(256), lds7, st, Q, F);
        }
        FS_HIP_OK(hipGetLastError());
    }
    int rc = launch_block<G, 2, 1, 4, true, 2>(st, block_args(n, 8, n->o[3], batch, 1), n->ncu);
    if (!rc) hipLaunchKernelGGL(af_policy_fc_f16s<G>, dim3((batch + kPfPos - 1) / kPfPos), dim3(512), kPfLds, st, n->hx[1], n->hfw[1], n->hfb[1],
                                n->hf_inv[1], policy, batch);
    FS_HIP_OK(hipGetLastError());
    return rc;
}

int f16s_small_forward_ok(const f16s_net* n, int batch) {
    return n && n->S == 11 && batch >= 1 && batch <= kSmallBatch && !(n->abl & (16 | 32 | 128 | 256 | 512 | 2048));
}
static F16sArgs layer_args(f16s_net* n, int li, const char* in, const char* in2, char* out, int batch) {
    F16sArgs a;
    memset(&a, 0, sizeof(a));
    a.in = in; a.in2 = in2; a.w = n->w[li]; a.bias = n->bias[li]; a.out = out; a.inv_scale = n->inv_scale[li]; a.batch = batch;
    a.abl = (n->abl & 0xf0ff) | (li << 8); a.stash = n->stash; a.inv_scale2 = 1.0f; a.inv_scale_h = 1.0f;
    a.pw = n->pw[li]; a.pbuf = n->pbuf[li / 2]; a.inv_scale_p = n->inv_scale_p[li];
    return a;
}
int f16s_small_forward(f16s_net* n, hipStream_t st, const float* planes, int batch, float* value, float* policy) {
    if (!f16s_small_forward_ok(n, batch) || !planes || !value || !policy) return -1;
    using G = Geo<11>;
    SmallFwdArgs S;
    memset(&S, 0, sizeof(S));
    S.planes = planes; S.stem_w = n->stem_wm; S.stem_b = n->stem_b; S.stem_inv = n->stem_inv_scale; S.f0 = n->f0;
    S.df = n->df; S.batch = batch;
    auto role = [&](F16sArgs a, int wait, int need, int done) { a.df_wait = n->df + wait; a.df_need = need; a.df_done = n->df + done; a.df_err = n->df + kDfErr; return a; };
    S.L0 = role(layer_args(n, 0, n->f0, nullptr, n->g[0], batch), kDfStem, 1, kDfL0);
    S.L1 = role(layer_args(n, 1, n->g[0], n->f0, n->o[0], batch), kDfL0, 2, kDfL1);
    S.L2 = role(layer_args(n, 2, n->o[0], nullptr, n->g[1], batch), kDfL1, 2, kDfL2);
    S.L3 = role(layer_args(n, 3, n->g[1], n->o[0], n->o[1], batch), kDfL2, 4, kDfL3);
    S.P = role(layer_args(n, 6, n->o[1], nullptr, n->g[3], batch), kDfL3, 4, kDfP);
    S.P.pw = nullptr; S.P.pbuf = nullptr;
    S.V = role(block_args(n, 4, n->o[1], batch, 0), kDfL3, 4, kDfV);
    S.Q = role(layer_args(n, 7, n->g[3], n->o[1], n->o[3], batch), kDfP, 2, kDfQ);
    S.Q.pw = nullptr; S.Q.pbuf = nullptr;
    S.B5 = role(block_args(n, 8, n->o[3], batch, 1), kDfQ, 2, kDfB5);
    S.F = VfcArgs{n->hx[0], n->hfw[0], n->hfb[0], n->v2w, n->v2b, n->hf_inv[0], value};
    constexpr size_t ldsC = Lds<G, kDist>::kScrOff + (size_t)2 * 1 * 4 * 4096;
    constexpr size_t ldsV = Lds<G, 2>::kScrOff + (size_t)2 * 2 * 4096 * 2 + 36864;
    constexpr size_t ldsB = Lds<G, 2>::kScrOff + Lay<G>::kSlotL + 36864;
    constexpr size_t lds = std::max(std::max(ldsC, ldsV), std::max(ldsB, (size_t)StemLds<G>::kBytes));
    static_assert(lds + 256 <= 160 * 1024, "LDS budget (dynamic + the value head's static reduction buffer)");
    static std::atomic<uint64_t> attr_devs{0};
    int dev = 0;
    FS_HIP_OK(hipGetDevice(&dev));
    const uint64_t bit = 1ull << (dev & 63);
    if (!(attr_devs.load(std::memory_order_relaxed) & bit)) {
        FS_HIP_OK(hipFuncSetAttribute(reinterpret_cast<const void*>(af_small_forward_f16s<G>), hipFuncAttributeMaxDynamicSharedMemorySize, (int)lds));
        attr_devs.fetch_or(bit, std::memory_order_relaxed);
    }
    S.xp = n->hx[1]; S.pfa = n->hfw[1]; S.pfb = n->hfb[1]; S.pf_inv = n->hf_inv[1]; S.policy = policy; S.pfx = n->pfx;
    hipLaunchKernelGGL(af_small_forward_f16s<G>, dim3(19 * batch + 3), dim3(256), lds, st, S);
    FS_HIP_OK(hipGetLastError());
    return 0;
}
int f16s_small_forward_error(f16s_net* n) {
    if (!n || !n->df) return -1;
    int e = 0;
    FS_HIP_OK(hipDeviceSynchronize());
    FS_HIP_OK(hipMemcpy(&e, n->df + kDfErr, sizeof(int), hipMemcpyDeviceToHost));
    return e;
}
int f16s_small_branches_ok(const f16s_net* n, int batch) {
    if (!n || n->S != 11 || (n->abl & 256)) return 0;
    return batch <= kSmallBatch ? !(n->abl & (128 | 512)) : !(n->abl & 1024);
}

// ... 42 lines not shown
```

alphafive_amd/csrc/af_engine.hip:

```cpp

#include <hip/hip_runtime.h>
#include <stdint.h>
#include <stdio.h>
#include <stdlib.h>
#include <string.h>

#include <type_traits>
#include <vector>

#include "af_engine.h"
#include "af_noise.h"

typedef unsigned long long u64;

enum { PH_IDLE = 0, PH_MOVE_START = 1, PH_SEARCH = 2, PH_MOVE_DONE = 3, PH_ERROR = 4, PH_DESCENT = 5  };
enum { CT_SIMS = 0, CT_SELECTS, CT_EXPANDS, CT_TERMINALS, CT_PLIES, CT_EPISODES, CT_LSUM, CT_LEXP,
       CT_GC, CT_GC_SCANNED, CT_YIELDS, CT_STALLS, CT_N };
enum { HIST_WORK = 0, HIST_TIME = 64, HIST_MAXTIME = 96, HIST_N = 97 };

struct EngineParams {
    int G, S, C, goal, sims, upper, training, mode, node_cap, max_ply, budget, budget_hard;
    uint32_t hash_mask;
    double init_temp, tau_decay, tau_decay_r, alpha, c_puct;
    float c_puct32;
// ... 738 lines not shown
            }
            uint32_t slot = 0xffffffffu;
            int idx;
            if (hint) {
                idx = hint - 1;
            } else {
                idx = tree_lookup<KW>(P, g, cm, ctb, lane, &slot);
                if (idx >= 0 && pidx >= 0 && lane == 0) ec[(size_t)pidx * CP + pcl] = idx + 1;
            }
            if (idx < 0) {
                if constexpr (MEMO) {
                    if (slot != 0xffffffffu && bb_count<KW>(cm) + bb_count<KW>(ctb) <= P.memo_max_stones) {
                        uint32_t unused;
                        const int me = memo_probe<KW>(P, memo_bucket<KW>(P, cm, ctb, last), cm, ctb, last, lane, &unused);
                        ++memo_probes;
                        if (me >= 0) {
                            ++memo_hits;
#pragma unroll
                            for (int k = 0; k < KW; ++k) { lm[k] = cm[k]; lt[k] = ctb[k]; }
                            c_depth = depth; c_slot = slot;
                            c_pol = P.memo_pv + (size_t)me * CP;
                            c_val = P.memo_val + me;
                            have_eval = true;
                            break;
                        }
                    }
                }
                if (lane < 2 * KW) P.leaf[(size_t)g * 2 * KW + lane] = key_word<KW>(cm, ctb, lane);
                if (lane == 0) { P.depth[g] = depth; P.leaf_last[g] = last; P.leaf_slot[g] = (int32_t)slot; }
                float* out = planes_out + (size_t)g * 3 * C;
#pragma unroll
                for (int k = 0; k < KW; ++k) {
                    const int c = lane + 64 * k;
                    if (c < C) {
                        out[c] = ((cm[k] >> lane) & 1ull) ? 1.0f : 0.0f;
                        out[C + c] = ((ctb[k] >> lane) & 1ull) ? 1.0f : 0.0f;
                        out[2 * C + c] = c == last ? 1.0f : 0.0f;
                    }
                }
                status = AF_STATUS_NEED_EVAL;
                parked = true;
                break;
            }
            if (work >= P.budget_hard) {
                if (lane < 2 * KW) P.leaf[(size_t)g * 2 * KW + lane] = key_word<KW>(cm, ctb, lane);
                if (lane == 0) { P.depth[g] = depth; P.leaf_last[g] = last; }
                phase = PH_DESCENT; status = AF_STATUS_YIELD; parked = true; ct[CT_YIELDS]++;
                break;
            }
            TK_T(tk_b);
            TK_ACC(3, tk_a, tk_b);
            const bool is_root = depth == 0;
            u64 legal[KW];
#pragma unroll
            for (int k = 0; k < KW; ++k) legal[k] = ~(cm[k] | ctb[k]) & P.boardmask[k];
            if (!r_have) {
                r_sum = nsum[idx];
#pragma unroll
                for (int k = 0; k < KW; ++k) {
                    const size_t off = (size_t)idx * CP + lane + 64 * k;
                    r_raw[k] = en[off];
                    r_c[k] = ec[off];
                    if constexpr (W64) r_w[k] = ew64[off]; else r_w[k] = ew[off];
                    r_p[k] = ep[off];
                }
            }
            r_have = false;
            const int sum_n = rfli(r_sum) + 1;
            if (lane == 0) nsum[idx] = sum_n;
            const uint32_t sel_id = sel++;
            int nn[KW];
            float pp[KW];
            wrow_t ww[KW];
            bool ff[KW];
            int32_t cc[KW];
#pragma unroll
            for (int k = 0; k < KW; ++k) {
                nn[k] = r_raw[k] & 0x7fffffff;
                ff[k] = r_raw[k] < 0;
                cc[k] = r_c[k];
                ww[k] = r_w[k];
                pp[k] = r_p[k];
            }
            double dd[KW];
            if (P.training) {
#ifdef AF_TICK_TIMING
                int tk_myit = 0;
#endif
                {
                    const float a_ = (float)P.alpha, inv_a = 1.0f / a_, one_m_a = 1.0f - a_;
                    uint32_t todo = 0;
#pragma unroll
                    for (int k = 0; k < KW; ++k) { dd[k] = 0.0; todo |= ((legal[k] >> lane) & 1ull) ? (1u << k) : 0u; }
                    af_u32x4 rk[KW];
                    uint32_t pend = 0;
#pragma unroll
                    for (int k = 0; k < KW; ++k) {
                        rk[k] = af_philox4x32(sel_id, episode, (AF_STREAM_GAMMA << 24) | (uint32_t)(lane + 64 * k), 0u, k0, k1);
                        float X;
                        const int ok = af_gamma_round(a_, inv_a, one_m_a, rk[k].v[0], rk[k].v[1], &X);
                        const bool lg = (todo >> k) & 1u;
                        dd[k] = (lg && ok) ? (double)X : 0.0;
                        pend |= (lg && !ok) ? (1u << k) : 0u;
                        if (KW > 2 && (k & 1)) __builtin_amdgcn_sched_barrier(0);
                    }
#ifdef AF_TICK_TIMING
                    ++tk_myit;
#endif
                    todo = pend;
                    {
                    uint32_t it = 1;
                    af_u32x4 r = rk[0];
#pragma unroll
                    for (int q = 1; q < KW; ++q) if (!(todo & ((1u << q) - 1u))) r = rk[q];
                    while (todo) {
#ifdef AF_TICK_TIMING
                        ++tk_myit;
#endif
                        const int k = __builtin_ctz(todo);
                        if ((it & 1u) == 0u) r = af_philox4x32(sel_id, episode, (AF_STREAM_GAMMA << 24) | (uint32_t)(lane + 64 * k), it >> 1, k0, k1);
                        const uint32_t wu = (it & 1u) ? r.v[2] : r.v[0], wv = (it & 1u) ? r.v[3] : r.v[1];
                        float X;
                        const int ok = af_gamma_round(a_, inv_a, one_m_a, wu, wv, &X);
                        if (ok || it == 0xFFFFu) {
                            const double Xd = ok ? (double)X : 0.0;
#pragma unroll
                            for (int q = 0; q < KW; ++q) dd[q] = q == k ? Xd : dd[q];
                            todo &= todo - 1u;
                            it = 1;
#pragma unroll
                            for (int q = 1; q < KW; ++q) if (todo && !(todo & ((1u << q) - 1u))) r = rk[q];
                        } else {
                            ++it;
                        }
                    }
                    }
                }
#ifdef AF_TICK_TIMING
                tk[12] += (unsigned long long)wave_max_i32(tk_myit);
#endif
                TK_T(tk_n1);
                TK_ACC(8, tk_b, tk_n1);
                double acc = 0.0;
#pragma unroll
                for (int k = 0; k < KW; ++k) acc = k == 0 ? dd[0] : acc + dd[k];
                acc = wave_sum_f64_tree(acc);
                if (acc == 0.0) {
                    int cnt = 0;
#pragma unroll
                    for (int k = 0; k < KW; ++k) cnt += __popcll(legal[k]);
                    const double u = 1.0 / (double)cnt;
#pragma unroll
                    for (int k = 0; k < KW; ++k) dd[k] = ((legal[k] >> lane) & 1ull) ? u : 0.0;
                } else {
                    const double inv = 1.0 / acc;
#pragma unroll
                    for (int k = 0; k < KW; ++k) dd[k] = dd[k] * inv;
                }
                TK_T(tk_n1e);
                TK_ACC(9, tk_n1, tk_n1e);
            }
            TK_T(tk_n2);
            const double sq = sqrt((double)(sum_n + 1));
            float sc[KW];
            float mx = -3.0e38f;
#pragma unroll
            for (int k = 0; k < KW; ++k) {
                const bool lg = (legal[k] >> lane) & 1ull;
                double q64;
                if (nn[k] == 0) q64 = 0.0;
                else if (!W64 && ff[k]) q64 = (double)((float)ww[k] / (float)nn[k]);
                else q64 = (double)ww[k] / (double)nn[k];
                double t;
                if (P.training) {
                    double p_;
                    if (is_root) p_ = (double)(0.75f * pp[k]) + 0.25 * dd[k];
                    else p_ = (double)(0.9f * pp[k]) + 0.1 * dd[k];
                    t = ((P.c_puct * p_) * sq) / (double)(1 + nn[k]);
                } else {
                    t = ((double)(P.c_puct32 * pp[k]) * sq) / (double)(1 + nn[k]);
                }
                sc[k] = lg ? (float)(q64 + t) : -3.0e38f;
                mx = sc[k] > mx ? sc[k] : mx;
            }
            TK_T(tk_n3);
            TK_ACC(10, tk_n2, tk_n3);
            int cell = -1;
            if (is_root && P.training) {
                u64 cand[KW];
#pragma unroll
                for (int k = 0; k < KW; ++k) cand[k] = __ballot(((legal[k] >> lane) & 1ull) && nn[k] == 0);
                int m = bb_count<KW>(cand);
                if (m == 0) {
#pragma unroll
                    for (int k = 0; k < KW; ++k) cand[k] = __ballot(((legal[k] >> lane) & 1ull) && nn[k] == 1);
                    m = bb_count<KW>(cand);
                }
                if (m > 0) cell = bb_select_wave<KW>(cand, (int)af_pick((uint32_t)m, sel_id, episode, AF_STREAM_PICK, k0, k1), lane);
            }
            if (cell < 0) {
                mx = wave_max_f32(mx);
                u64 cand[KW];
#pragma unroll
                for (int k = 0; k < KW; ++k) cand[k] = __ballot(((legal[k] >> lane) & 1ull) && sc[k] == mx);
                const int m = bb_count<KW>(cand);
                cell = bb_select_wave<KW>(cand, (int)af_pick((uint32_t)m, sel_id, episode, AF_STREAM_PICK, k0, k1), lane);
            }
            cell = rfli(cell);
            hint = 0;
#pragma unroll
            for (int k = 0; k < KW; ++k) { const int t_ = __builtin_amdgcn_readlane(cc[k], cell & 63); if ((cell >> 6) == k) hint = t_; }
            hint = rfli(hint);
            pidx = idx; pcl = cell;
            if (hint) {
                const int ci = hint - 1;
                r_sum = nsum[ci];
#pragma unroll
                for (int k = 0; k < KW; ++k) {
                    const size_t off = (size_t)ci * CP + lane + 64 * k;
                    r_raw[k] = en[off];
                    r_c[k] = ec[off];
                    if constexpr (W64) r_w[k] = ew64[off]; else r_w[k] = ew[off];
                    r_p[k] = ep[off];
                }
                r_have = true;
            }
            ++work;
            ct[CT_SELECTS]++;
            ct[CT_LSUM] += (uint32_t)bb_count<KW>(legal);
            if (lane == 0) { pnode[depth] = idx; pcell[depth] = cell; }
            ++depth;
            {
                u64 nm[KW], nt[KW];
#pragma unroll
                for (int k = 0; k < KW; ++k) { nm[k] = ctb[k]; nt[k] = cm[k]; }
                bb_set<KW>(nt, cell);
#pragma unroll
                for (int k = 0; k < KW; ++k) { cm[k] = nm[k]; ctb[k] = nt[k]; }
            }
            last = cell;
            __syncthreads();
            TK_T(tk_c);
            TK_ACC(4, tk_b, tk_c);
            TK_ACC(11, tk_n3, tk_c);
#ifdef AF_TICK_TIMING
            tk[7] += 1;
#endif
        }
    }
    if (!MEMO || !have_eval) break;
  }
    TK_T(tk_parked);
    if constexpr (MEMO) {
        if (lane == 0 && memo_probes) {
            atomicAdd(reinterpret_cast<unsigned long long*>(&P.memo_stats[MEMO_PROBES]), (unsigned long long)memo_probes);
            if (memo_hits) atomicAdd(reinterpret_cast<unsigned long long*>(&P.memo_stats[MEMO_HITS]), (unsigned long long)memo_hits);
        }
    }

    if (err) { phase = PH_ERROR; status = err; }
    if (lane < 2 * KW) P.root[(size_t)g * 2 * KW + lane] = key_word<KW>(root_m, root_t, lane);
    if (lane == 0) {
        P.phase[g] = phase;
        P.pending[g] = status == AF_STATUS_NEED_EVAL ? 1 : 0;
        P.root_last[g] = root_last;
        P.sims_left[g] = sims_left;
        P.ply[g] = ply;
        P.nodes[g] = nodes;
        P.nfree[g] = nfree;
        P.tau[g] = tau;
        P.episode[g] = episode;
        P.sel[g] = sel;
        P.plyctr[g] = plyctr;
        P.status[g] = status;
        for (int i = 0; i < CT_N; ++i)
            if (ct[i]) atomicAdd(reinterpret_cast<unsigned long long*>(&P.counters[(size_t)g * CT_N + i]), (unsigned long long)ct[i]);
        const u64 dt = wall_clock64() - t_start;
        atomicAdd(&P.hist[HIST_WORK + (work < 63 ? work : 63)], 1ull);
        const u64 tb = dt / 800ull;
        atomicAdd(&P.hist[HIST_TIME + (tb < 31ull ? tb : 31ull)], 1ull);
        atomicMax(&P.hist[HIST_MAXTIME], dt);
    }
#ifdef AF_TICK_TIMING
// ... 286 lines not shown
}

int32_t af_engine_num_games(const af_engine* e) { return e->P.G; }
int32_t af_engine_cells(const af_engine* e) { return e->P.C; }
int32_t af_engine_key_words(const af_engine* e) { return 2 * e->KW; }
int32_t af_engine_max_plies(const af_engine* e) { return e->P.max_ply; }

int af_engine_tick(af_engine* e, void* stream, const float* policy_dev, const float* value_dev, float* planes_dev) {
    if (!e || !planes_dev) return AF_ERR_ARG;
    hipStream_t st = (hipStream_t)stream;
#define AF_TICK(KW_, W_, M_) hipLaunchKernelGGL((af_tick_kernel<KW_, W_, M_>), dim3(e->P.G), dim3(64), 0, st, e->P, policy_dev, value_dev, planes_dev)
    if (e->memo) {
        if (e->KW == 2) { if (e->P.w64) AF_TICK(2, true, true); else AF_TICK(2, false, true); }
        else { if (e->P.w64) AF_TICK(4, true, true); else AF_TICK(4, false, true); }
    } else {
        if (e->KW == 2) { if (e->P.w64) AF_TICK(2, true, false); else AF_TICK(2, false, false); }
        else { if (e->P.w64) AF_TICK(4, true, false); else AF_TICK(4, false, false); }
    }
#undef AF_TICK
    HIP_OK(hipGetLastError());
    return AF_OK;
}

int af_engine_memo_enable(af_engine* e, int32_t log2_buckets, int32_t max_stones) {
    if (!e || e->memo || log2_buckets < 4 || log2_buckets > 28 || max_stones < 0) return AF_ERR_ARG;
    HIP_OK(hipSetDevice(e->device));
    EngineParams& P = e->P;
    const size_t NE = (size_t)4 << log2_buckets, CP = 64 * (size_t)e->KW, MK = 4 * (size_t)e->KW;
    int rc = AF_OK;
    if (rc == AF_OK) rc = dalloc(e, &P.memo_key, NE * MK);
    if (rc == AF_OK) rc = dalloc(e, &P.memo_pv, NE * CP);
    if (rc == AF_OK) rc = dalloc(e, &P.memo_val, NE);
    if (rc == AF_OK) rc = dalloc(e, &P.memo_lock, NE);
    if (rc == AF_OK) rc = dalloc(e, &P.memo_stats, (size_t)MEMO_N);
    if (rc != AF_OK) return rc;
    P.memo_bucket_mask = (uint32_t)((1ull << log2_buckets) - 1ull);
    P.memo_max_stones = max_stones;
    P.memo_epoch = 1;
    P.memo_budget = P.budget < 6 ? P.budget : 6;
    if (const char* b = getenv("AF_MEMO_BUDGET")) { const int v = atoi(b); if (v > 0) { P.memo_budget = v; e->memo_budget_fixed = true; } }
    e->memo_entries = NE;
    e->memo = true;
    return AF_OK;
}

int af_engine_memo_insert(af_engine* e, void* stream, const float* policy_dev, const float* value_dev) {
    if (!e || !e->memo || !policy_dev || !value_dev) return AF_ERR_ARG;
    hipStream_t st = (hipStream_t)stream;
    if (e->KW == 2) hipLaunchKernelGGL((af_memo_insert_kernel<2>), dim3(e->P.G), dim3(64), 0, st, e->P, policy_dev, value_dev);
    else hipLaunchKernelGGL((af_memo_insert_kernel<4>), dim3(e->P.G), dim3(64), 0, st, e->P, policy_dev, value_dev);
    HIP_OK(hipGetLastError());
    return AF_OK;
}

int af_engine_memo_clear(af_engine* e, void* stream) {
    if (!e || !e->memo) return AF_ERR_ARG;
    hipStream_t st = (hipStream_t)stream;
    if (e->P.memo_epoch == 0xffffffffu) {
        HIP_OK(hipMemsetAsync(e->P.memo_key, 0, e->memo_entries * 4 * (size_t)e->KW * 8, st));
        e->P.memo_epoch = 1;
    } else {
        ++e->P.memo_epoch;
    }
    return AF_OK;
}

int64_t af_engine_memo_epoch(af_engine* e) { return (e && e->memo) ? (int64_t)e->P.memo_epoch : 0; }

int af_engine_memo_stats(af_engine* e, void* stream, uint64_t* out) {
    if (!e || !e->memo || !out) return AF_ERR_ARG;
    hipStream_t st = (hipStream_t)stream;
    HIP_OK(hipMemcpyAsync(out, e->P.memo_stats, (size_t)MEMO_N * 8, hipMemcpyDeviceToHost, st));
    HIP_OK(hipStreamSynchronize(st));
    out[MEMO_N] = (uint64_t)e->memo_entries;
    return AF_OK;
}

int af_engine_status(af_engine* e, void* stream, int32_t* status_host) {
    if (!e || !status_host) return AF_ERR_ARG;
    hipStream_t st = (hipStream_t)stream;
    HIP_OK(hipMemcpyAsync(status_host, e->P.status, (size_t)e->P.G * 4, hipMemcpyDeviceToHost, st));
    HIP_OK(hipStreamSynchronize(st));
    for (int g = 0; g < e->P.G; ++g) if (status_host[g] < 0) return status_host[g];
    return AF_OK;
}

int af_engine_set_training(af_engine* e, int32_t training) {
    if (!e) return AF_ERR_ARG;
    e->P.training = training ? 1 : 0;
    return AF_OK;
}

int af_engine_set_simulations(af_engine* e, int32_t sims, int32_t upper) {
    if (!e || sims < 1 || upper < 1 || sims + 8 > e->P.node_cap) return AF_ERR_ARG;
    e->P.sims = sims;
    e->P.upper = upper;
    return AF_OK;
}

int af_engine_set_root(af_engine* e, int32_t game, const uint64_t* key, int32_t last_cell, int32_t random_a,
                       int32_t reset_tree) {
    if (!e || !key || game < 0 || game >= e->P.G || e->P.mode != AF_MODE_EXTERNAL) return AF_ERR_ARG;
    EngineParams& P = e->P;
    const int KW = e->KW;
    for (int k = 0; k < KW; ++k) {
        if ((key[k] | key[KW + k]) & ~P.boardmask[k]) return AF_ERR_ARG;
        if (key[k] & key[KW + k]) return AF_ERR_ARG;
    }
    if (last_cell < -1 || last_cell >= P.C) return AF_ERR_ARG;
    HIP_OK(hipDeviceSynchronize());
    if (reset_tree) {
        const size_t hcap = (size_t)P.hash_mask + 1;
        HIP_OK(hipMemset(P.hash + (size_t)game * hcap, 0, hcap * 4));
        int32_t zero = 0;
        HIP_OK(hipMemcpy(P.nodes + game, &zero, 4, hipMemcpyHostToDevice));
        HIP_OK(hipMemcpy(P.nfree + game, &zero, 4, hipMemcpyHostToDevice));
        double tau = P.init_temp;
        HIP_OK(hipMemcpy(P.tau + game, &tau, 8, hipMemcpyHostToDevice));
        uint32_t ep;
        HIP_OK(hipMemcpy(&ep, P.episode + game, 4, hipMemcpyDeviceToHost));
        ep += 1;
        HIP_OK(hipMemcpy(P.episode + game, &ep, 4, hipMemcpyHostToDevice));
        uint32_t z = 0;
        HIP_OK(hipMemcpy(P.sel + game, &z, 4, hipMemcpyHostToDevice));
        HIP_OK(hipMemcpy(P.plyctr + game, &z, 4, hipMemcpyHostToDevice));
    }
    HIP_OK(hipMemcpy(P.root + (size_t)game * 2 * KW, key, (size_t)2 * KW * 8, hipMemcpyHostToDevice));
    int32_t v = last_cell;
    HIP_OK(hipMemcpy(P.root_last + game, &v, 4, hipMemcpyHostToDevice));
    v = random_a ? 1 : 0;
    HIP_OK(hipMemcpy(P.random_a + game, &v, 4, hipMemcpyHostToDevice));
    v = PH_MOVE_START;
    HIP_OK(hipMemcpy(P.phase + game, &v, 4, hipMemcpyHostToDevice));
    v = 0;
    HIP_OK(hipMemcpy(P.pending + game, &v, 4, hipMemcpyHostToDevice));
    HIP_OK(hipMemcpy(P.status + game, &v, 4, hipMemcpyHostToDevice));
    return AF_OK;
}

int af_engine_set_roots(af_engine* e, void* stream, int32_t n, const int32_t* games, const uint64_t* keys, const int32_t* last_cells,
                        const int32_t* random_a, const int32_t* reset_tree) {
    if (!e || e->P.mode != AF_MODE_EXTERNAL || n < 0 || (n > 0 && (!games || !keys || !last_cells))) return AF_ERR_ARG;
    if (n == 0) return AF_OK;
    EngineParams& P = e->P;
    const int KW = e->KW, KW2 = 2 * KW;
    std::vector<int32_t> req((size_t)4 * n);
    for (int i = 0; i < n; ++i) {
        if (games[i] < 0 || games[i] >= P.G || last_cells[i] < -1 || last_cells[i] >= P.C) return AF_ERR_ARG;
        const uint64_t* k = keys + (size_t)i * KW2;
        for (int q = 0; q < KW; ++q)
            if (((k[q] | k[KW + q]) & ~P.boardmask[q]) || (k[q] & k[KW + q])) return AF_ERR_ARG;
        req[4 * i] = games[i]; req[4 * i + 1] = last_cells[i]; req[4 * i + 2] = random_a ? random_a[i] : 0; req[4 * i + 3] = reset_tree ? reset_tree[i] : 0;
    }
    hipStream_t st = (hipStream_t)stream;
    const size_t rb = (size_t)4 * n * 4, kb = (size_t)n * KW2 * 8, need = rb + kb;
    if (e->stage_cap < need) {
        if (e->stage_dev) (void)hipFree(e->stage_dev);
        e->stage_dev = nullptr; e->stage_cap = 0;
        HIP_OK(hipMalloc((void**)&e->stage_dev, need * 2));
        e->stage_cap = need * 2;
    }
    HIP_OK(hipMemcpyAsync(e->stage_dev, req.data(), rb, hipMemcpyHostToDevice, st));
    HIP_OK(hipMemcpyAsync(e->stage_dev + rb, keys, kb, hipMemcpyHostToDevice, st));
    hipLaunchKernelGGL(af_set_roots_kernel, dim3(n), dim3(64), 0, st, P, n, (const int32_t*)e->stage_dev, (const u64*)(e->stage_dev + rb), KW2);
    HIP_OK(hipGetLastError());
    HIP_OK(hipStreamSynchronize(st));
// ... 369 lines not shown
```

alphafive_amd/csrc/af_net.hip:

```cpp

#include <hip/hip_runtime.h>
#include <stdint.h>
#include <stdio.h>
#include <string.h>

#include <map>
#include <string>
#include <vector>

#include "af_net.h"
#include "af_conv_f16s.h"

typedef float f32x16 __attribute__((ext_vector_type(16)));
typedef float f4u __attribute__((ext_vector_type(4), aligned(4)));
typedef float f2u __attribute__((ext_vector_type(2), aligned(4)));
typedef float f2a __attribute__((ext_vector_type(2)));

__device__ __forceinline__ float elu1(float x) { return x > 0.0f ? x : __expf(x) - 1.0f; }

struct WinoArgs {
    const float* in;
    const float* u;
    const float* in2;
    const float* u2;
// ... 427 lines not shown
    const float* xb = X + i16 * KS + kq;
    f32x4 acc0 = {0, 0, 0, 0}, acc1 = {0, 0, 0, 0};
    constexpr int PF = 16;
    float a0[PF], a1[PF];
    const int nsteps = K / 4;
#pragma unroll
    for (int q = 0; q < PF; ++q) { a0[q] = w0[(size_t)q * 4 * HW]; a1[q] = w1[(size_t)q * 4 * HW]; }
    int s0 = 0;
    for (; s0 + PF <= nsteps; s0 += PF) {
#pragma unroll
        for (int q = 0; q < PF; ++q) {
            const int s_ = s0 + q;
            const float bx = xb[s_ * 4];
            const float ca0 = a0[q], ca1 = a1[q];
            const int sn = s_ + PF < nsteps ? s_ + PF : nsteps - 1;
            a0[q] = w0[(size_t)sn * 4 * HW];
            a1[q] = w1[(size_t)sn * 4 * HW];
            acc0 = __builtin_amdgcn_mfma_f32_16x16x4f32(ca0, bx, acc0, 0, 0, 0);
            acc1 = __builtin_amdgcn_mfma_f32_16x16x4f32(ca1, bx, acc1, 0, 0, 0);
        }
    }
#pragma unroll
    for (int q = 0; q < PF; ++q) {
        if (s0 + q < nsteps) {
            const float bx = xb[(s0 + q) * 4];
            acc0 = __builtin_amdgcn_mfma_f32_16x16x4f32(a0[q], bx, acc0, 0, 0, 0);
            acc1 = __builtin_amdgcn_mfma_f32_16x16x4f32(a1[q], bx, acc1, 0, 0, 0);
        }
    }
    __syncthreads();
    float* Lg = smem;
#pragma unroll
    for (int r = 0; r < 4; ++r) {
        const int ja = wave * 32 + kq * 4 + r, jb = ja + 16;
        Lg[i16 * 128 + ja] = acc0[r] + (ja < HW ? bf[ja] : 0.0f);
        Lg[i16 * 128 + jb] = acc1[r] + (jb < HW ? bf[jb] : 0.0f);
    }
    __syncthreads();
    const int p = t >> 4, sub = t & 15;
    float v[8], m = -3.0e38f;
#pragma unroll
    for (int q = 0; q < 8; ++q) {
        const int j = sub + 16 * q;
        v[q] = j < HW ? Lg[p * 128 + j] : -3.0e38f;
        m = fmaxf(m, v[q]);
    }
#pragma unroll
    for (int off = 8; off >= 1; off >>= 1) m = fmaxf(m, __shfl_xor(m, off));
    float sum = 0.0f;
#pragma unroll
    for (int q = 0; q < 8; ++q) { v[q] = (sub + 16 * q) < HW ? expf(v[q] - m) : 0.0f; sum += v[q]; }
#pragma unroll
    for (int off = 8; off >= 1; off >>= 1) sum += __shfl_xor(sum, off);
    if (b0 + p < batch) {
#pragma unroll
        for (int q = 0; q < 8; ++q) {
            const int j = sub + 16 * q;
            if (j < HW) policy[(size_t)(b0 + p) * HW + j] = v[q] / sum;
        }
    }
}

#define NET_HIP_OK(x) do { hipError_t e_ = (x); if (e_ != hipSuccess) { fprintf(stderr, "[af_net] %s failed: %s\n", #x, hipGetErrorString(e_)); return AF_NET_ERR_HIP; } } while (0)

struct Block { const char* name; int cin, cout; };
static const Block kBlocks[5] = {{"bone/block1", 32, 64}, {"bone/block2", 64, 128}, {"value/block3", 128, 32},
                                 {"policy/block4", 128, 64}, {"policy/block5", 64, 32}};

struct af_net {
    int S, HW, WP, PP, max_batch, device;
    bool ready = false;
    std::map<std::string, std::vector<float>> vars;
    std::map<std::string, size_t> expect;
    std::vector<void*> allocs;
    float *stem_w, *stem_b;
    float *conv1_b[5], *sum_b[5];
    float *wino1_u[5], *wino2_u[5], *winor_u[5];
    int T;
    hipStream_t branch_stream = nullptr;
    hipEvent_t ev_trunk = nullptr, ev_value = nullptr;
    float *vc_w, *vc_b, *v1_w, *v1_b, *v2_w, *v2_b, *pc_w, *pc_b, *pf_w, *pf_b;
    float *f0, *g[5], *o[5];
    f16s_net* f16s = nullptr;
};

static int pad32(int c) { return (c + 31) / 32 * 32; }

template <typename T>
static int net_alloc(af_net* n, T** p, size_t count, bool zero) {
    void* q = nullptr;
    NET_HIP_OK(hipMalloc(&q, count * sizeof(T)));
    if (zero) NET_HIP_OK(hipMemset(q, 0, count * sizeof(T)));
    n->allocs.push_back(q);
    *p = (T*)q;
    return AF_NET_OK;
}
static int net_upload(af_net* n, float** p, const std::vector<float>& h) {
    int rc = net_alloc(n, p, h.size(), false);
    if (rc) return rc;
    NET_HIP_OK(hipMemcpy(*p, h.data(), h.size() * 4, hipMemcpyHostToDevice));
    return AF_NET_OK;
}

static std::vector<float> pack_wino(const std::vector<float>& w, int taps, int cin, int cout) {
    static const double G[4][3] = {{1, 0, 0}, {0.5, 0.5, 0.5}, {0.5, -0.5, 0.5}, {0, 0, 1}};
    static const int kCentre[4] = {5, 6, 9, 10};
    const int npos = taps == 9 ? 16 : 4;
    std::vector<float> out((size_t)cin * npos * cout, 0.0f);
    for (int c = 0; c < cin; ++c)
        for (int co = 0; co < cout; ++co) {
            double g[3][3] = {{0, 0, 0}, {0, 0, 0}, {0, 0, 0}};
            if (taps == 9) {
                for (int t = 0; t < 9; ++t) g[t / 3][t % 3] = w[((size_t)t * cin + c) * cout + co];
            } else {
                g[1][1] = w[(size_t)c * cout + co];
            }
            for (int p = 0; p < npos; ++p) {
                const int x = taps == 9 ? p : kCentre[p];
                const int xi = x / 4, nu = x % 4;
                double u = 0.0;
                for (int i = 0; i < 3; ++i)
                    for (int j = 0; j < 3; ++j) u += G[xi][i] * g[i][j] * G[nu][j];
                out[((((size_t)(c / 2) * 2) + (c & 1)) * cout + co) * npos + p] = (float)u;
            }
        }
    return out;
}
static std::vector<float> pad_bias(const std::vector<float>& a, const std::vector<float>* b, int cout) {
    std::vector<float> out(pad32(cout), 0.0f);
    for (int i = 0; i < cout; ++i) out[i] = a[i] + (b ? (*b)[i] : 0.0f);
    return out;
}

extern "C" {

const char* af_net_strerror(int code) {
    switch (code) {
        case AF_NET_OK: return "ok";
        case AF_NET_ERR_ARG: return "bad argument";
        case AF_NET_ERR_HIP: return "HIP runtime error";
        case AF_NET_ERR_NAME: return "unknown variable name or wrong element count";
        case AF_NET_ERR_STATE: return "network not finalized or variables missing";
        default: return "unknown error";
    }
}

int af_net_create(int32_t S, int32_t max_batch, int32_t device, af_net** out) {
    if (!out || S < 3 || S > 16 || max_batch < 1) return AF_NET_ERR_ARG;
    NET_HIP_OK(hipSetDevice(device));
    af_net* n = new af_net();
    n->S = S; n->HW = S * S;
    n->T = (S + 1) / 2;
    n->WP = 2 * n->T + 2;
    n->PP = (n->WP * n->WP + 15) / 16 * 16;
    n->max_batch = max_batch; n->device = device;
    if ((uint64_t)max_batch * 128u * (uint64_t)n->PP * 4u >= (1ull << 32)) { delete n; return AF_NET_ERR_ARG; }
    const size_t HW = n->HW;
    n->expect["bone/conv1/kernel"] = 75 * 32; n->expect["bone/conv1/bias"] = 32;
    for (const Block& b : kBlocks) {
        const std::string s = b.name;
        n->expect[s + "_res/kernel"] = (size_t)b.cin * b.cout; n->expect[s + "_res/bias"] = b.cout;
        n->expect[s + "_conv1/kernel"] = (size_t)9 * b.cin * b.cout; n->expect[s + "_conv1/bias"] = b.cout;
        n->expect[s + "_conv2/kernel"] = (size_t)9 * b.cout * b.cout; n->expect[s + "_conv2/bias"] = b.cout;
    }
    n->expect["value/conv/kernel"] = 32 * 4; n->expect["value/conv/bias"] = 4;
    n->expect["value/fc1/kernel"] = 4 * HW * 64; n->expect["value/fc1/bias"] = 64;
    n->expect["value/fc2/kernel"] = 64; n->expect["value/fc2/bias"] = 1;
    n->expect["policy/conv/kernel"] = 32 * 16; n->expect["policy/conv/bias"] = 16;
    n->expect["policy/fc/kernel"] = 16 * HW * HW; n->expect["policy/fc/bias"] = HW;
    *out = n;
    return AF_NET_OK;
}

void af_net_destroy(af_net* n) {
    if (!n) return;
    (void)hipSetDevice(n->device);
    for (void* p : n->allocs) (void)hipFree(p);
    f16s_destroy(n->f16s);
    if (n->branch_stream) (void)hipStreamDestroy(n->branch_stream);
    if (n->ev_trunk) (void)hipEventDestroy(n->ev_trunk);
    if (n->ev_value) (void)hipEventDestroy(n->ev_value);
    delete n;
}

int af_net_set_variable(af_net* n, const char* name, const float* data, int64_t count) {
    if (!n || !name || !data) return AF_NET_ERR_ARG;
    auto it = n->expect.find(name);
    if (it == n->expect.end() || (int64_t)it->second != count) return AF_NET_ERR_NAME;
    n->vars[name].assign(data, data + count);
    n->ready = false;
    return AF_NET_OK;
}

int af_net_finalize(af_net* n) {
    if (!n) return AF_NET_ERR_ARG;
    for (auto& kv : n->expect) if (!n->vars.count(kv.first)) return AF_NET_ERR_STATE;
    NET_HIP_OK(hipSetDevice(n->device));
    for (void* p : n->allocs) (void)hipFree(p);
    n->allocs.clear();
    f16s_destroy(n->f16s);
    n->f16s = nullptr;
    if (f16s_supported(n->S) && f16s_create(&n->f16s, n->S, n->max_batch, n->device, n->vars) != 0) return AF_NET_ERR_HIP;
    auto& V = n->vars;
    int rc = AF_NET_OK;
#define UP(dst, vec) if (!rc) rc = net_upload(n, &n->dst, (vec))
    UP(stem_w, V["bone/conv1/kernel"]); UP(stem_b, V["bone/conv1/bias"]);
    for (int i = 0; i < 5; ++i) {
        const Block& b = kBlocks[i];
        const std::string s = b.name;
        UP(conv1_b[i], pad_bias(V[s + "_conv1/bias"], nullptr, b.cout));
        UP(sum_b[i], pad_bias(V[s + "_conv2/bias"], &V[s + "_res/bias"], b.cout));
        UP(wino1_u[i], pack_wino(V[s + "_conv1/kernel"], 9, b.cin, b.cout));
        UP(wino2_u[i], pack_wino(V[s + "_conv2/kernel"], 9, b.cout, b.cout));
        UP(winor_u[i], pack_wino(V[s + "_res/kernel"], 1, b.cin, b.cout));
    }
    UP(vc_w, V["value/conv/kernel"]); UP(vc_b, V["value/conv/bias"]); UP(v1_w, V["value/fc1/kernel"]);
    UP(v1_b, V["value/fc1/bias"]); UP(v2_w, V["value/fc2/kernel"]); UP(v2_b, V["value/fc2/bias"]);
    UP(pc_w, V["policy/conv/kernel"]); UP(pc_b, V["policy/conv/bias"]); UP(pf_w, V["policy/fc/kernel"]);
    UP(pf_b, V["policy/fc/bias"]);
#undef UP
    const size_t plane = (size_t)n->max_batch * n->PP;
    if (!rc) rc = net_alloc(n, &n->f0, plane * 32, true);
    for (int i = 0; i < 5 && !rc; ++i) {
        rc = net_alloc(n, &n->g[i], plane * kBlocks[i].cout, true);
        if (!rc) rc = net_alloc(n, &n->o[i], plane * kBlocks[i].cout, true);
    }
    if (rc) return rc;
    NET_HIP_OK(hipFuncSetAttribute(reinterpret_cast<const void*>(af_policy_head_mfma), hipFuncAttributeMaxDynamicSharedMemorySize,
                                   160 * 1024));
    if (!n->branch_stream) {
        NET_HIP_OK(hipStreamCreateWithFlags(&n->branch_stream, hipStreamNonBlocking));
        NET_HIP_OK(hipEventCreateWithFlags(&n->ev_trunk, hipEventDisableTiming));
        NET_HIP_OK(hipEventCreateWithFlags(&n->ev_value, hipEventDisableTiming));
    }
    n->ready = true;
    return AF_NET_OK;
}

}

static int g_f16s_abl = 0;
static int g_wino = 5;

static void launch_wino(hipStream_t st, const af_net* n, int batch, const float* in, const float* u, int cin,
                        const float* in2, const float* u2, int cin2, const float* bias, float* out, int cout) {
    WinoArgs a;
    a.in = in; a.u = u; a.in2 = in2; a.u2 = u2; a.bias = bias; a.out = out;
    a.cin = cin; a.cin2 = cin2; a.cout = cout; a.T = n->T; a.S = n->S; a.WP = n->WP; a.PP = n->PP;
    a.ntiles = batch * n->T * n->T;
    const int ntb = (a.ntiles + 31) / 32;
    const int ngrp8 = (((ntb + 3) / 4) + 7) / 8 * 8;
    hipLaunchKernelGGL(af_conv_wino, dim3(ngrp8 * (cout / 32)), dim3(256), 0, st, a);
}


static int g_phead = 1;
static int g_branch = 1;
static int g_fhead = 1;

static int forward_range(af_net* n, hipStream_t st, const float* planes_all, int b0, int batch, float* policy_all, float* value_all) {
    const int S = n->S, HW = n->HW, WP = n->WP, PP = n->PP;
    const float* planes = planes_all + (size_t)b0 * 3 * HW;
    float* policy = policy_all + (size_t)b0 * HW;
    float* value = value_all + b0;
    const size_t po = (size_t)b0 * PP;
    float* f0 = n->f0 + po * 32;
    float* g[5];
    float* o[5];
    for (int i = 0; i < 5; ++i) { g[i] = n->g[i] + po * kBlocks[i].cout; o[i] = n->o[i] + po * kBlocks[i].cout; }
    const bool split16 = g_wino == 5 && n->f16s != nullptr;
    const bool fhead = split16 && g_fhead;
    if (split16) {
        f16s_set_ablation(n->f16s, g_f16s_abl);
        if (fhead && f16s_small_forward_ok(n->f16s, batch)) {
            if (f16s_small_forward(n->f16s, st, planes, batch, value, policy)) return AF_NET_ERR_HIP;
            return AF_NET_OK;
        }
        if (f16s_trunk(n->f16s, st, planes, batch)) return AF_NET_ERR_HIP;
    } else {
        hipLaunchKernelGGL(af_stem_conv, dim3(batch), dim3(256), 0, st, planes, n->stem_w, n->stem_b, f0, S, WP, PP);
    }
    if (fhead && f16s_small_branches_ok(n->f16s, batch)) {
        if (f16s_small_branches(n->f16s, st, batch, value, policy)) return AF_NET_ERR_HIP;
        NET_HIP_OK(hipGetLastError());
        return AF_NET_OK;
    }
    const float* block_in[5] = {f0, o[0], o[1], o[1], o[3]};
    hipStream_t vs = st;
    if (g_branch && n->branch_stream && (!split16 || g_branch == 2)) {
        vs = n->branch_stream;
    }
    for (int i = split16 ? 2 : 0; i < 5; ++i) {
        const Block& b = kBlocks[i];
        hipStream_t st_main = st;
        if (i == 2 && vs != st_main) {
            NET_HIP_OK(hipEventRecord(n->ev_trunk, st_main));
            NET_HIP_OK(hipStreamWaitEvent(vs, n->ev_trunk, 0));
        }
        hipStream_t st = (i == 2) ? vs : st_main;
        if (split16) {
            if (i == 2 && f16s_value_branch(n->f16s, st, batch, o[2], WP, PP, fhead ? value : nullptr)) return AF_NET_ERR_HIP;
            if (i == 4 && f16s_policy_branch(n->f16s, st, batch, o[4], WP, PP, fhead ? policy : nullptr)) return AF_NET_ERR_HIP;
        } else {
            launch_wino(st, n, batch, block_in[i], n->wino1_u[i], b.cin, nullptr, nullptr, 0, n->conv1_b[i], g[i], b.cout);
            launch_wino(st, n, batch, g[i], n->wino2_u[i], b.cout, block_in[i], n->winor_u[i], b.cin, n->sum_b[i], o[i], b.cout);
        }
        if (i == 2) {
            if (!fhead)
            hipLaunchKernelGGL(af_value_head, dim3((batch + VPB - 1) / VPB), dim3(256), 0, st, o[2], n->vc_w, n->vc_b, n->v1_w, n->v1_b,
                               n->v2_w, n->v2_b, value, batch, S, WP, PP);
            if (vs != st_main) NET_HIP_OK(hipEventRecord(n->ev_value, vs));
        }
    }
    if (fhead) {
    } else if (HW <= 128 && g_phead) {
        const int K = 16 * HW, KS = K + ((2 - K % 32) + 32) % 32;
        const size_t lds = (size_t)16 * KS * 4;
        hipLaunchKernelGGL(af_policy_head_mfma, dim3((batch + 15) / 16), dim3(256), lds, st, o[4], n->pc_w, n->pc_b, n->pf_w,
                           n->pf_b, policy, batch, S, WP, PP);
    } else if (HW <= 128) {
        const size_t lds = ((size_t)16 * HW * 8 + 512 + 32) * 4;
        hipLaunchKernelGGL((af_policy_head<8>), dim3((batch + 7) / 8), dim3(256), lds, st, o[4], n->pc_w, n->pc_b, n->pf_w,
                           n->pf_b, policy, batch, S, WP, PP);
    } else {
        const size_t lds = ((size_t)16 * HW * 4 + 512 + 16) * 4;
        hipLaunchKernelGGL((af_policy_head<4>), dim3((batch + 3) / 4), dim3(256), lds, st, o[4], n->pc_w, n->pc_b, n->pf_w,
                           n->pf_b, policy, batch, S, WP, PP);
    }
    if (vs != st) NET_HIP_OK(hipStreamWaitEvent(st, n->ev_value, 0));
    NET_HIP_OK(hipGetLastError());
    return AF_NET_OK;
}

extern "C" {

int af_net_forward(af_net* n, void* stream, const float* planes, int32_t batch, float* policy, float* value) {
    if (!n || !planes || !policy || !value || batch < 1 || batch > n->max_batch) return AF_NET_ERR_ARG;
    if (!n->ready) return AF_NET_ERR_STATE;
    return forward_range(n, (hipStream_t)stream, planes, 0, batch, policy, value);
}

int af_net_tune(int32_t key, int32_t value) {
    if (key == 0) { if (value != 1 && value != 5) return AF_NET_ERR_ARG; g_wino = value; return AF_NET_OK; }
    if (key == 5) { g_phead = value; return AF_NET_OK; }
    if (key == 4) { g_branch = value; return AF_NET_OK; }
    if (key == 9) { g_fhead = value ? 1 : 0; return AF_NET_OK; }
    if (key == 7) { g_f16s_abl = value; return AF_NET_OK; }
    return AF_NET_ERR_ARG;
}

int af_net_debug_activation(af_net* n, int32_t which, int32_t batch, float* host_out) {
    if (!n || !host_out || !n->f16s) return AF_NET_ERR_ARG;
    const int c = f16s_read_activation(n->f16s, which, batch, host_out);
    return c < 0 ? AF_NET_ERR_ARG : c;
}

int af_net_small_forward_error(af_net* n) {
    if (!n || !n->f16s) return AF_NET_ERR_ARG;
    return f16s_small_forward_error(n->f16s);
}

int64_t af_net_flops_per_position(const af_net* n) {
    const int64_t HW = n->HW;
    int64_t mac = 75 * 32 * HW;
    for (const Block& b : kBlocks) mac += ((int64_t)9 * b.cin * b.cout + (int64_t)9 * b.cout * b.cout + (int64_t)b.cin * b.cout) * HW;
    mac += 32 * 4 * HW + 4 * HW * 64 + 64 + 32 * 16 * HW + 16 * HW * HW;
    return 2 * mac;
}

}
```

alphafive_amd/engine.py:

```python
import ctypes as C
import os

import numpy as np

_PKG = os.path.dirname(os.path.abspath(__file__))
_LIBPATH = os.environ.get("AF_HIP_LIB") or os.path.join(_PKG, "_lib", "libaf_hip.so")

MODE_SELFPLAY, MODE_EXTERNAL = 0, 1
MODE_VALUE_F64 = 0x100
STATUS_IDLE, STATUS_NEED_EVAL, STATUS_MOVE_DONE, STATUS_YIELD = 0, 1, 2, 3
STAMP_SLOTS = 64
BLACK_WIN, WHITE_WIN, DRAW = 1, -1, 0

CFG_ATTRS = ("board_size", "goal", "simulation_per_step", "upper_simulation_per_step", "init_temp", "gamma",
             "tau_decay_rate", "tau_decay_rate_r", "dirichlet_alpha", "c_puct")


class AfConfig(C.Structure):
    _fields_ = [("board_size", C.c_int32), ("goal", C.c_int32), ("simulation_per_step", C.c_int32),
                ("upper_simulation_per_step", C.c_int32), ("init_temp", C.c_double), ("gamma", C.c_double),
                ("tau_decay_rate", C.c_double), ("tau_decay_rate_r", C.c_double), ("dirichlet_alpha", C.c_double),
                ("c_puct", C.c_double)]

    @classmethod
    def from_cfg(cls, cfg):
        return cls(*[getattr(cfg, a) for a in CFG_ATTRS])


class EngineError(RuntimeError):
    pass


_lib = None


def lib():
    global _lib
    if _lib is None:
        if not os.path.exists(_LIBPATH):
            raise EngineError(f"{_LIBPATH} not found: build the HIP engine first "
                              f"(python -m alphafive_amd.build). There is no CPU fallback.")
        import torch
        L = C.CDLL(_LIBPATH)
        vp = C.c_void_p
        i32p, f32p, u64p, u8p = (C.POINTER(C.c_int32), C.POINTER(C.c_float), C.POINTER(C.c_uint64),
                                 C.POINTER(C.c_uint8))
        L.af_abi_version.restype = C.c_int
        L.af_strerror.restype = C.c_char_p
        L.af_strerror.argtypes = [C.c_int]
        L.af_engine_create.argtypes = [C.POINTER(AfConfig), C.c_int32, C.c_int32, C.c_int32, C.c_int32, C.c_uint64,
                                       C.c_uint32, C.c_int32, C.POINTER(vp)]
        L.af_engine_destroy.argtypes = [vp]
        L.af_engine_destroy.restype = None
        for fn in ("af_engine_num_games", "af_engine_cells", "af_engine_key_words", "af_engine_max_plies"):
            getattr(L, fn).argtypes = [vp]
            getattr(L, fn).restype = C.c_int32
        L.af_engine_tick.argtypes = [vp, vp, vp, vp, vp]
        L.af_engine_status.argtypes = [vp, vp, i32p]
        L.af_engine_set_root.argtypes = [vp, C.c_int32, u64p, C.c_int32, C.c_int32, C.c_int32]
        L.af_engine_move_result.argtypes = [vp, C.c_int32, i32p, i32p, f32p, i32p, C.POINTER(C.c_double)]
        L.af_engine_set_training.argtypes = [vp, C.c_int32]
        L.af_engine_set_simulations.argtypes = [vp, C.c_int32, C.c_int32]
        L.af_engine_set_roots.argtypes = [vp, vp, C.c_int32, i32p, u64p, i32p, i32p, i32p]
        L.af_engine_move_results.argtypes = [vp, vp, C.c_int32, i32p, i32p, i32p, f32p, i32p, C.POINTER(C.c_double)]
        L.af_engine_pop_episodes.argtypes = [vp, vp, C.c_int32, i32p, f32p, u64p, f32p, i32p, i32p, i32p]
        L.af_engine_pack_ints.argtypes = [vp, C.c_int32, C.c_int32]
        L.af_engine_pack_ints.restype = C.c_int64
        L.af_engine_pack_episodes.argtypes = [vp, vp, C.c_int32, C.c_int32, vp]
        L.af_engine_counters.argtypes = [vp, vp, u64p]
        L.af_engine_tree_w64.argtypes = [vp, C.c_int32, C.c_int32, C.POINTER(C.c_double)]
        L.af_engine_set_tree_w64.argtypes = [vp, C.c_int32, C.c_int32, C.POINTER(C.c_double)]
        L.af_engine_progress.argtypes = [vp, vp, u64p]
        L.af_engine_progress_async.argtypes = [vp, vp, vp]
        L.af_engine_stamp.argtypes = [vp, vp, C.c_int32]
        L.af_engine_stamps_async.argtypes = [vp, vp, vp]
        L.af_engine_tick_histogram.argtypes = [vp, vp, u64p, C.c_int32]
        L.af_engine_set_tick_budget.argtypes = [vp, C.c_int32]
        L.af_engine_memo_enable.argtypes = [vp, C.c_int32, C.c_int32]
        L.af_engine_memo_insert.argtypes = [vp, vp, vp, vp]
        L.af_engine_memo_clear.argtypes = [vp, vp]
        L.af_engine_memo_stats.argtypes = [vp, vp, u64p]
        L.af_engine_memo_epoch.argtypes = [vp]
        L.af_engine_memo_epoch.restype = C.c_int64
        L.af_engine_tree_dump.argtypes = [vp, C.c_int32, C.c_int32, u64p, i32p, i32p, f32p, f32p, u8p]
        L.af_engine_load_tree.argtypes = [vp, C.c_int32, C.c_int32, u64p, i32p, i32p, f32p, f32p, u8p]
        L.af_state_to_key.argtypes = [C.c_char_p, C.c_int32, u64p]
        L.af_key_to_state.argtypes = [u64p, C.c_int32, C.c_char_p, C.c_int32]
        _lib = L
    return _lib


def _check(rc, what):
    if rc < 0:
        raise EngineError(f"{what}: {lib().af_strerror(rc).decode()} (code {rc})")
    return rc


def _p(a, ct):
    return a.ctypes.data_as(C.POINTER(ct))


def key_words(S):
    return 4 if S * S <= 128 else 8


def state_to_key(state, S):
    key = np.zeros(key_words(S), np.uint64)
    _check(lib().af_state_to_key(state.encode(), S, _p(key, C.c_uint64)), "af_state_to_key")
    return key


def key_to_state(key, S):
    key = np.ascontiguousarray(key, np.uint64)
    out = C.create_string_buffer(288)
    _check(lib().af_key_to_state(_p(key, C.c_uint64), S, out, 288), "af_key_to_state")
    return out.value.decode()


COUNTER_NAMES = ("sims", "selects", "expands", "terminals", "plies", "episodes", "legal_sum", "legal_sum_expand",
                 "nodes", "collector_runs", "collector_scanned", "yields", "stalls")


class Engine:

    def __init__(self, cfg, num_games, device=0, mode=MODE_SELFPLAY, training=True, seed=0, first_game_id=0,
                 node_cap=0, value_f64=False):
        self._h = C.c_void_p()
        self.cfg = AfConfig.from_cfg(cfg) if not isinstance(cfg, AfConfig) else cfg
        self.value_f64 = bool(value_f64) or bool(mode & MODE_VALUE_F64)
        mode = (mode & ~MODE_VALUE_F64) | (MODE_VALUE_F64 if self.value_f64 else 0)
        _check(lib().af_engine_create(C.byref(self.cfg), num_games, device, mode, int(training), seed, first_game_id,
                                      node_cap, C.byref(self._h)), "af_engine_create")
        self.G = num_games
        self.S = self.cfg.board_size
        self.C = self.S * self.S
        self.KW2 = lib().af_engine_key_words(self._h)
        self.max_plies = lib().af_engine_max_plies(self._h)
        self.mode = mode & ~MODE_VALUE_F64
        self.device = device
        self._status = np.zeros(num_games, np.int32)
        self._params = {"training": int(bool(training)), "sims": int(self.cfg.simulation_per_step),
                        "upper": int(self.cfg.upper_simulation_per_step), "tick_budget": None}

    def close(self):
        if getattr(self, "_h", None):
            lib().af_engine_destroy(self._h)
            self._h = None

    __del__ = close

    def tick(self, policy_ptr, value_ptr, planes_ptr, stream=None):
        _check(lib().af_engine_tick(self._h, stream, policy_ptr, value_ptr, planes_ptr), "af_engine_tick")

    def status(self, stream=None):
        rc = lib().af_engine_status(self._h, stream, _p(self._status, C.c_int32))
        _check(rc, "engine status")
        return self._status

    def params_key(self):
        p = self._params
        return (p["training"], p["sims"], p["upper"], p["tick_budget"], p.get("memo_epoch"), p.get("memo"))

    def set_training(self, training):
        _check(lib().af_engine_set_training(self._h, int(training)), "af_engine_set_training")
        self._params["training"] = int(bool(training))

    def set_simulations(self, sims, upper):
        _check(lib().af_engine_set_simulations(self._h, int(sims), int(upper)), "af_engine_set_simulations")
        self._params["sims"], self._params["upper"] = int(sims), int(upper)

    def set_root(self, game, key, last_cell=-1, random_a=False, reset_tree=False):
        key = np.ascontiguousarray(key, np.uint64)
        _check(lib().af_engine_set_root(self._h, game, _p(key, C.c_uint64), last_cell, int(random_a), int(reset_tree)),
               "af_engine_set_root")

    def move_result(self, game):
        a, hp, tau = C.c_int32(-1), C.c_int32(0), C.c_double(0)
        pol = np.zeros(self.C, np.float32)
        vis = np.zeros(self.C, np.int32)
        _check(lib().af_engine_move_result(self._h, game, C.byref(a), C.byref(hp), _p(pol, C.c_float),
                                           _p(vis, C.c_int32), C.byref(tau)), "af_engine_move_result")
        return a.value, (pol if hp.value else None), vis, tau.value

    def set_roots(self, games, keys, last_cells, random_a=False, reset_tree=False, stream=None):
        n = len(games)
        g = np.ascontiguousarray(games, np.int32)
        k = np.ascontiguousarray(keys, np.uint64).reshape(n, self.KW2)
        lc = np.ascontiguousarray(last_cells, np.int32)
        ra = np.ascontiguousarray(np.broadcast_to(np.asarray(random_a, np.int32), (n,)))
        rt = np.ascontiguousarray(np.broadcast_to(np.asarray(reset_tree, np.int32), (n,)))
        _check(lib().af_engine_set_roots(self._h, stream, n, _p(g, C.c_int32), _p(k, C.c_uint64), _p(lc, C.c_int32),
                                         _p(ra, C.c_int32), _p(rt, C.c_int32)), "af_engine_set_roots")

    def move_results(self, games, stream=None):
        n = len(games)
        g = np.ascontiguousarray(games, np.int32)
        act, hp = np.zeros(n, np.int32), np.zeros(n, np.int32)
        pol, vis, tau = np.zeros((n, self.C), np.float32), np.zeros((n, self.C), np.int32), np.zeros(n, np.float64)
        _check(lib().af_engine_move_results(self._h, stream, n, _p(g, C.c_int32), _p(act, C.c_int32), _p(hp, C.c_int32),
                                            _p(pol, C.c_float), _p(vis, C.c_int32), _p(tau, C.c_double)), "af_engine_move_results")
        return act, hp, pol, vis, tau

    def counters(self, stream=None):
        out = np.zeros(len(COUNTER_NAMES), np.uint64)
        _check(lib().af_engine_counters(self._h, stream, _p(out, C.c_uint64)), "af_engine_counters")
        return {k: int(v) for k, v in zip(COUNTER_NAMES, out)}

    def tick_histogram(self, stream=None, reset=False):
        out = np.zeros(97, np.uint64)
        _check(lib().af_engine_tick_histogram(self._h, stream, _p(out, C.c_uint64), int(reset)), "tick_histogram")
        return dict(selects=out[:64].astype(np.int64), wave_us=out[64:96].astype(np.int64),
                    max_wave_us=float(out[96]) * 0.01)

    def memo_enable(self, log2_buckets=18, max_stones=5):
        _check(lib().af_engine_memo_enable(self._h, int(log2_buckets), int(max_stones)), "af_engine_memo_enable")
        kw = self.KW2 // 2
        self.memo_bytes = (4 << int(log2_buckets)) * (32 * kw + 256 * kw + 12)
        self._params["memo"] = (int(log2_buckets), int(max_stones))
        self._params["memo_epoch"] = int(lib().af_engine_memo_epoch(self._h))

    @property
    def memo(self):
        return self._params.get("memo")

    def memo_insert(self, policy_ptr, value_ptr, stream=None):
        _check(lib().af_engine_memo_insert(self._h, stream, policy_ptr, value_ptr), "af_engine_memo_insert")

    def memo_clear(self, stream=None):
        _check(lib().af_engine_memo_clear(self._h, stream), "af_engine_memo_clear")
        self._params["memo_epoch"] = int(lib().af_engine_memo_epoch(self._h))

    def memo_stats(self, stream=None):
        out = np.zeros(6, np.uint64)
        _check(lib().af_engine_memo_stats(self._h, stream, _p(out, C.c_uint64)), "af_engine_memo_stats")
        return {k: int(v) for k, v in zip(("launches", "probes", "hits", "inserts", "replaced", "entries"), out)}

    def set_tick_budget(self, selects_per_launch):
        _check(lib().af_engine_set_tick_budget(self._h, int(selects_per_launch)), "af_engine_set_tick_budget")
        self._params["tick_budget"] = int(selects_per_launch)

# ... 13 lines not shown

    def tree_dump(self, game):
        cnt = _check(lib().af_engine_tree_dump(self._h, game, 0, None, None, None, None, None, None), "tree_dump")
        keys = np.zeros((cnt, self.KW2), np.uint64)
        sum_n = np.zeros(cnt, np.int32)
        n = np.zeros((cnt, self.C), np.int32)
        w = np.zeros((cnt, self.C), np.float32)
        p = np.zeros((cnt, self.C), np.float32)
        f = np.zeros((cnt, self.C), np.uint8)
        if cnt:
            _check(lib().af_engine_tree_dump(self._h, game, cnt, _p(keys, C.c_uint64), _p(sum_n, C.c_int32),
                                             _p(n, C.c_int32), _p(w, C.c_float), _p(p, C.c_float), _p(f, C.c_uint8)),
                   "tree_dump")
            if self.value_f64:
                w = np.zeros((cnt, self.C), np.float64)
                _check(lib().af_engine_tree_w64(self._h, game, cnt, _p(w, C.c_double)), "af_engine_tree_w64")
        return dict(keys=keys, sum_n=sum_n, n=n, w=w, p=p, f32=f)

    def load_tree(self, game, dump):
        cnt = len(dump["sum_n"])
        arr = {k: np.ascontiguousarray(dump[k], t) for k, t in (("keys", np.uint64), ("sum_n", np.int32), ("n", np.int32),
                                                                 ("w", np.float32), ("p", np.float32), ("f32", np.uint8))}
        _check(lib().af_engine_load_tree(self._h, game, cnt, _p(arr["keys"], C.c_uint64), _p(arr["sum_n"], C.c_int32),
                                         _p(arr["n"], C.c_int32), _p(arr["w"], C.c_float), _p(arr["p"], C.c_float),
                                         _p(arr["f32"], C.c_uint8)), "af_engine_load_tree")
        if self.value_f64:
            w64 = np.ascontiguousarray(dump["w"], np.float64)
            _check(lib().af_engine_set_tree_w64(self._h, game, cnt, _p(w64, C.c_double)), "af_engine_set_tree_w64")

    def pack_ints(self, max_eps, max_plies):
        return int(_check(lib().af_engine_pack_ints(self._h, max_eps, max_plies), "af_engine_pack_ints"))

    def pack_episodes(self, out_ptr, max_eps, max_plies, stream=None):
        _check(lib().af_engine_pack_episodes(self._h, stream, max_eps, max_plies, out_ptr), "af_engine_pack_episodes")


def unpack_episodes(buf, max_eps):
    buf = np.ascontiguousarray(buf, np.int32)
    n, _, K, Cc = (int(x) for x in buf[:4])
    R = 2 * K + 2 * Cc + 2
    head = 4 + 5 * max_eps
    out = []
    for i in range(n):
        g, seq, T, p0 = (int(x) for x in buf[4 + 4 * i:8 + 4 * i])
        rec = buf[head + p0 * R:head + (p0 + T) * R].reshape(T, R)
        out.append(dict(game=g, seq=seq, T=T, final_value=float(buf[4 + 4 * max_eps + i:5 + 4 * max_eps + i].view(np.float32)[0]),
                        keys=np.ascontiguousarray(rec[:, :2 * K]).view(np.uint64).reshape(T, K).copy(),
                        policies=np.ascontiguousarray(rec[:, 2 * K:2 * K + Cc]).view(np.float32).copy(),
                        visits=rec[:, 2 * K + Cc:2 * K + 2 * Cc].copy(),
                        lasts=rec[:, 2 * K + 2 * Cc].copy(), actions=rec[:, 2 * K + 2 * Cc + 1].copy()))
    return out


def packed_used_ints(hdr, max_eps):
    n_plies, K, Cc = int(hdr[1]), int(hdr[2]), int(hdr[3])
    return 4 + 5 * max_eps + n_plies * (2 * K + 2 * Cc + 2)


def assemble_episode(raw, S, gamma):
    from . import utils
    T = raw["T"]
    value = float(raw["final_value"])
    if T % 2 == 1:
        value = -value
    weights = utils.construct_weights(T, gamma=gamma)
    rec = []
    for t in range(T):
        la = None if raw["lasts"][t] < 0 else (int(raw["lasts"][t]) // S, int(raw["lasts"][t]) % S)
        rec.append((key_to_state(raw["keys"][t], S), raw["policies"][t].reshape(S, S).copy(), la, value, weights[t]))
        value = -value
    last_value = rec[-1][-2]
    if last_value == 0.0:
        result = DRAW
    elif T % 2 == 1:
        result = BLACK_WIN
    else:
        result = WHITE_WIN
    return rec, result


class SelfPlayEngine:

    def __init__(self, cfg, num_games, pv_device, device=0, seed=0, first_game_id=0, training=True, node_cap=0,
                 value_f64=False, weights_version=None, eval_memo=None):
        import torch
        if not torch.cuda.is_available():
            raise EngineError("SelfPlayEngine needs a HIP device (torch.cuda.is_available() is False)")
        self.torch = torch
        self.cfg = cfg
        self.dev = torch.device("cuda", device)
        torch.cuda.set_device(self.dev)
        self.engine = Engine(cfg, num_games, device=device, mode=MODE_SELFPLAY, training=training, seed=seed,
                             first_game_id=first_game_id, node_cap=node_cap, value_f64=value_f64)
        S = cfg.board_size
        self.G, self.S, self.C = num_games, S, S * S
        self.planes = torch.zeros((num_games, 3, S, S), dtype=torch.float32, device=self.dev)
        self.policy = torch.zeros((num_games, S * S), dtype=torch.float32, device=self.dev)
        self.value = torch.zeros((num_games,), dtype=torch.float32, device=self.dev)
        self.pv_device = pv_device
        self._weights_version = self._resolve_weights_version(weights_version)
        if hasattr(pv_device, "bind_outputs"):
            pv_device.bind_outputs(self.policy, self.value)
        self._memo_version = None
        if eval_memo:
            if self._weights_version is None:
                raise EngineError("eval_memo: the evaluator exposes no weights_version (the memo could not tell when to forget); "
                                  "pass SelfPlayEngine(..., weights_version=lambda: net.version)")
            self.engine.memo_enable(**({} if eval_memo is True else dict(eval_memo)))
            self._memo_version = self._weights_version()
        self.ticks = 0
        self._boxes = {}
        self._graph = None
        self._prog_host, self._prog_events, self._prog_turn, self._prog_replays = None, None, 0, 0
        self.replay_events = []
        self._graph_stamped, self._stamp_host, self._stamp_event, self._stamp_pending, self.stamp_samples = None, None, None, False, []

    def tick(self, stamp_base=None):
        torch = self.torch
        stream = torch.cuda.current_stream(self.dev).cuda_stream
        if stamp_base is not None:
            self.engine.stamp(stamp_base, stream)
        memo = self.engine.memo is not None
        if memo:
            ver = self._weights_version()
            if ver != self._memo_version:
                self.engine.memo_clear(stream)
                self._memo_version = ver
        self.engine.tick(self.policy.data_ptr(), self.value.data_ptr(), self.planes.data_ptr(), stream)
        if stamp_base is not None:
            self.engine.stamp(stamp_base + 1, stream)
        p, v = self.pv_device(self.planes)
        if p.data_ptr() != self.policy.data_ptr():
            self.policy.copy_(p.reshape(self.G, self.C))
        if v.data_ptr() != self.value.data_ptr():
            self.value.copy_(v.reshape(self.G))
        if memo:
            self.engine.memo_insert(self.policy.data_ptr(), self.value.data_ptr(), stream)
        if stamp_base is not None:
            self.engine.stamp(stamp_base + 2, stream)
        self.ticks += 1

    def run_ticks(self, n, check_every=0):
        for i in range(n):
            self.tick()
            if check_every and (i + 1) % check_every == 0:
                self.check()

    def _resolve_weights_version(self, explicit):
        if explicit is not None:
            return explicit if callable(explicit) else (lambda: explicit)
        pv = self.pv_device
        ver = getattr(pv, "weights_version", None)
        if callable(ver):
            return ver
        owner = getattr(pv, "__self__", None)
        if owner is not None and hasattr(owner, "version"):
            return lambda: owner.version
        if hasattr(pv, "bind_outputs"):
            self._weights_version_missing = True
        return None

    def _graph_key(self, n):
        ver = self._weights_version
        return (int(n), self.engine.params_key(), ver() if ver is not None else None)

    def run_ticks_graph(self, n=16, timed=False, stamped=False):
        torch = self.torch
        if getattr(self, "_weights_version_missing", False):
            raise EngineError("run_ticks_graph: pv_device takes bind_outputs but exposes no weights_version (a replayed graph "
                              "would keep evaluating with stale weights); pass SelfPlayEngine(..., weights_version=lambda: net.version)")
        key = self._graph_key(n)
        if stamped:
            if 3 * n > STAMP_SLOTS:
                raise EngineError("run_ticks_graph(stamped=True): at most %d ticks per replay" % (STAMP_SLOTS // 3))
            if self._graph_stamped is None or self._graph_stamped[0] != key:
                self._graph_stamped = None
                if self._graph is None or self._graph[0] != key:
                    self.run_ticks_graph(n)
                if self._stamp_host is None:
                    self._stamp_host = torch.zeros(STAMP_SLOTS, dtype=torch.int64, pin_memory=True)
                    self._stamp_event = torch.cuda.Event()
                    self.engine.stamp(0, torch.cuda.current_stream(self.dev).cuda_stream)
                torch.cuda.synchronize(self.dev)
                g = torch.cuda.CUDAGraph()
                with torch.cuda.graph(g, capture_error_mode="thread_local"):
                    for i in range(n):
                        self.tick(stamp_base=3 * i)
                    st = torch.cuda.current_stream(self.dev).cuda_stream
                    self.engine.stamps_async(self._stamp_host.data_ptr(), st)
                    self.engine.progress_async(self._prog_host.data_ptr(), st)
                self.ticks -= n
                self._graph_stamped = (self._graph_key(n), g, n)
            if self._stamp_pending:
                self._collect_stamps()
            self._graph_stamped[1].replay()
            self._stamp_event.record(torch.cuda.current_stream(self.dev))
            self._stamp_pending = True
            self.ticks += n
            self._prog_turn ^= 1
            self._prog_events[self._prog_turn].record(torch.cuda.current_stream(self.dev))
            self._prog_replays += 1
            return
        if self._graph is None or self._graph[0] != key:
            self._graph = None
            if self._prog_host is None:
                self._prog_host = torch.zeros(2, dtype=torch.int64, pin_memory=True)
                self._prog_events = [torch.cuda.Event(), torch.cuda.Event()]
            self.tick()
            torch.cuda.synchronize(self.dev)
            g = torch.cuda.CUDAGraph()
            with torch.cuda.graph(g, capture_error_mode="thread_local"):
                for _ in range(n):
                    self.tick()
                st = torch.cuda.current_stream(self.dev).cuda_stream
                self.engine.progress_async(self._prog_host.data_ptr(), st)
            self.ticks -= n
            self._graph = (self._graph_key(n), g)
        if timed:
            e0, e1 = torch.cuda.Event(enable_timing=True), torch.cuda.Event(enable_timing=True)
            e0.record(torch.cuda.current_stream(self.dev))
        self._graph[1].replay()
        if timed:
            e1.record(torch.cuda.current_stream(self.dev))
            self.replay_events.append((n, e0, e1))
        self.ticks += n
        self._prog_turn ^= 1
        self._prog_events[self._prog_turn].record(torch.cuda.current_stream(self.dev))
        self._prog_replays += 1

    def _collect_stamps(self):
        self._stamp_event.synchronize()
        t = self._stamp_host.numpy().astype(np.int64)[:3 * self._graph_stamped[2]].reshape(-1, 3)
        self.stamp_samples.append(np.stack([(t[:, 1] - t[:, 0]) * 1e-5, (t[:, 2] - t[:, 1]) * 1e-5], axis=1))
        self._stamp_pending = False

    def read_stamps(self):
        if self._stamp_pending:
            self._collect_stamps()
        return np.concatenate(self.stamp_samples) if self.stamp_samples else np.zeros((0, 2))

    def progress_lagged(self):
        if self._prog_replays < 2:
            return 0, 0
        self._prog_events[self._prog_turn ^ 1].synchronize()
        return int(self._prog_host[0]), int(self._prog_host[1])

    def check(self):
        stream = self.torch.cuda.current_stream(self.dev).cuda_stream
        return self.engine.status(stream)

    def counters(self):
        return self.engine.counters(self.torch.cuda.current_stream(self.dev).cuda_stream)

    def progress(self):
        return self.engine.progress(self.torch.cuda.current_stream(self.dev).cuda_stream)

    def _pack_plies(self, cap):
        return max(cap * 40, int(self.engine.max_plies))

    def _outbox(self, cap):
        box = self._boxes.get(cap)
        if box is None:
            torch = self.torch
            max_plies = self._pack_plies(cap)
            ints = self.engine.pack_ints(cap, max_plies)
            box = dict(cap=cap, max_plies=max_plies, buf=torch.zeros(ints, dtype=torch.int32, pin_memory=True),
                       event=torch.cuda.Event(), posted=False)
            self._boxes[cap] = box
        return box

    def post_episodes(self, cap=256):
        box = self._outbox(cap)
        if box["posted"]:
            raise EngineError("post_episodes: the previous post has not been collected")
        stream = self.torch.cuda.current_stream(self.dev)
        self.engine.pack_episodes(box["buf"].data_ptr(), cap, box["max_plies"], stream.cuda_stream)
        box["event"].record(stream)
        box["posted"] = True
        return box

    def collect_episodes(self, cap=256, unpack=True):
        box = self._outbox(cap)
        if not box["posted"]:
            return [] if unpack else None
        box["event"].synchronize()
        box["posted"] = False
        return unpack_episodes(box["buf"].numpy(), cap) if unpack else box["buf"].numpy()

    def pop_raw(self, cap=256):
        self.post_episodes(cap)
        return self.collect_episodes(cap)

    def post_episodes_device(self, cap=256):
        key = ("dev", cap)
        buf = self._boxes.get(key)
        if buf is None:
            buf = self.torch.zeros(self.engine.pack_ints(cap, self._pack_plies(cap)), dtype=self.torch.int32, device=self.dev)
            self._boxes[key] = buf
        self.engine.pack_episodes(buf.data_ptr(), cap, self._pack_plies(cap), self.torch.cuda.current_stream(self.dev).cuda_stream)
        return buf

    def pop_episodes(self, cap=256):
        return [assemble_episode(r, self.S, self.cfg.gamma) for r in self.pop_raw(cap)]

    def close(self):
        self.engine.close()
```

alphafive_amd/net_hip.py:

```python
import ctypes as C
import os

import numpy as np
import torch

_PKG = os.path.dirname(os.path.abspath(__file__))
_LIBPATH = os.environ.get("AF_NET_LIB") or os.path.join(_PKG, "_lib", "libaf_net.so")
_lib = None


class NetError(RuntimeError):
    pass


def lib():
    global _lib
    if _lib is None:
        if not os.path.exists(_LIBPATH):
            raise ImportError(f"{_LIBPATH} not built (python -m alphafive_amd.build)")
        import torch
        L = C.CDLL(_LIBPATH)
        vp = C.c_void_p
        L.af_net_create.argtypes = [C.c_int32, C.c_int32, C.c_int32, C.POINTER(vp)]
        L.af_net_destroy.argtypes = [vp]
        L.af_net_destroy.restype = None
        L.af_net_set_variable.argtypes = [vp, C.c_char_p, C.POINTER(C.c_float), C.c_int64]
        L.af_net_finalize.argtypes = [vp]
        L.af_net_forward.argtypes = [vp, vp, vp, C.c_int32, vp, vp]
        L.af_net_flops_per_position.argtypes = [vp]
        L.af_net_flops_per_position.restype = C.c_int64
        L.af_net_small_forward_error.argtypes = [vp]
        L.af_net_strerror.argtypes = [C.c_int]
        L.af_net_strerror.restype = C.c_char_p
        _lib = L
    return _lib


def _check(rc, what):
    if rc < 0:
        raise NetError(f"{what}: {lib().af_net_strerror(rc).decode()} (code {rc})")


class HipNet(object):

    def __init__(self, variables, board_size, max_batch, device):
        self.S, self.max_batch, self.device = board_size, max_batch, torch.device(device)
        self._h = C.c_void_p()
        self._version = 0
        idx = self.device.index if self.device.index is not None else torch.cuda.current_device()
        _check(lib().af_net_create(board_size, max_batch, idx, C.byref(self._h)), "af_net_create")
        self.load(variables)
        self.flops_per_position = int(lib().af_net_flops_per_position(self._h))
        self.policy = torch.empty((max_batch, board_size * board_size), dtype=torch.float32, device=self.device)
        self.value = torch.empty((max_batch,), dtype=torch.float32, device=self.device)

    def load(self, variables):
        torch.cuda.synchronize(self.device)
        for name, arr in variables.items():
            a = np.ascontiguousarray(arr, np.float32)
            _check(lib().af_net_set_variable(self._h, name.encode(), a.ctypes.data_as(C.POINTER(C.c_float)), a.size),
                   f"af_net_set_variable({name})")
        _check(lib().af_net_finalize(self._h), "af_net_finalize")
        self._version += 1

    def weights_version(self):
        return self._version

    def bind_outputs(self, policy, value):
        assert policy.is_contiguous() and value.is_contiguous() and policy.dtype == torch.float32
        assert policy.shape[0] >= self.max_batch or policy.shape[0] == value.shape[0]
        self.policy, self.value = policy, value

    def __call__(self, planes):
        B = planes.shape[0]
        assert B <= self.max_batch and planes.is_contiguous() and planes.dtype == torch.float32
        stream = torch.cuda.current_stream(self.device).cuda_stream
        _check(lib().af_net_forward(self._h, stream, planes.data_ptr(), B, self.policy.data_ptr(), self.value.data_ptr()),
               "af_net_forward")
        return self.policy[:B], self.value[:B]

    def small_forward_error(self):
        return int(lib().af_net_small_forward_error(self._h))

    def close(self):
        if getattr(self, "_h", None):
            try:
                lib().af_net_destroy(self._h)
            except Exception:
                pass
            self._h = None

    __del__ = close


def make_eval(resnet):
    if resnet.device.type != "cuda" or not (3 <= resnet.board_size <= 15):
        return None
    lib()
    state = {"net": None, "out": None, "version": None}

    def pv(planes):
        B = planes.shape[0]
        if state["net"] is None or state["net"].max_batch < B:
            if state["net"] is not None:
                state["net"].close()
            state["net"] = HipNet(resnet.variables, resnet.board_size, B, resnet.device)
            state["version"] = getattr(resnet, "version", None)
            if state["out"] is not None and state["out"][0].shape[0] >= B:
                state["net"].bind_outputs(*state["out"])
        elif state["version"] != getattr(resnet, "version", None):
            state["net"].load(resnet.variables)
            state["version"] = getattr(resnet, "version", None)
        return state["net"](planes)

    def bind_outputs(policy, value):
        state["out"] = (policy, value)
        if state["net"] is not None and policy.shape[0] >= state["net"].max_batch:
            state["net"].bind_outputs(policy, value)

    def close():
        if state["net"] is not None:
            state["net"].close()
            state["net"] = None

    pv.bind_outputs = bind_outputs
    pv.close = close
    pv.weights_version = lambda: getattr(resnet, "version", None)
    return pv


_SPLIT_MAC_PER_PIXEL = sum(9 * ci * co + 9 * co * co + ci * co for ci, co in ((32, 64), (64, 128), (128, 32), (128, 64), (64, 32)))
_SPLIT_BYTES_PER_POSITION = (28 * 16384 + 17 * 15488 + 2 * (4 + 16) * 121 * 2 * 2 + 3 * 121 * 4 + 122 * 4)


_conv_mode = 5


def roofline_info(board_size=11):
    if board_size == 15 and _conv_mode == 5:
        return {"backend": "hip (af_conv_f16s.hip on 15x15: two half-board pseudo-positions per board, fp16 split operands, fp32 "
                           "accumulation; MFMA stem and fused heads as on 11x11)",
                "kernel": "af_net_forward = af_stem_mfma_f16s<Geo<15>> + 10x af_conv_f16s<Geo<15>> (the last conv of each branch also "
                          "applies the head's 1x1 convolution) + af_value_fc_f16s<Geo<15>> + af_policy_fc_f16s<Geo<15>> (whole "
                          "forward timed)",
                "peak_tflops": 2500.0, "issued_flop_per_position": 2 * 3 * _SPLIT_MAC_PER_PIXEL * 256,
                "algorithmic_bytes_per_position": (30 * 2 * 20480 + 19 * 30720 + 2 * 2 * 2 * 16384 + 2 * (4 + 16) * 225 * 2 * 2 + 3 * 225 * 4 + 226 * 4)}
    if board_size == 11 and _conv_mode == 5:
        return {"backend": "hip (af_conv_f16s.hip: stem, convs and heads on v_mfma_f32_32x32x16_f16 with fp16 split operands and "
                           "fp32 accumulation; convs weight-stationary with an LDS-DMA slab ring)",
                "kernel": "af_net_forward = af_stem_mfma_f16s + 6x af_conv_f16s + 2x af_block_f16s (blocks 3 and 5: both convolutions "
                          "and the head's 1x1 convolution in one kernel, the intermediate in LDS) + af_value_fc_f16s + af_policy_fc_f16s "
                          "(whole forward timed; the convolution kernels carry 99 % of the algorithmic FLOPs, each MAC issued as 3 fp16 MFMA MACs)",
                "peak_tflops": 2500.0, "issued_flop_per_position": 2 * 3 * _SPLIT_MAC_PER_PIXEL * 121,
                "algorithmic_bytes_per_position": _SPLIT_BYTES_PER_POSITION}
    return {"backend": "hip (af_net.hip: fp32 MFMA Winograd F(2x2,3x3) convs, fused transforms/bias/ELU/residual)",
            "kernel": "af_net_forward = af_stem_conv + 10x af_conv_wino + af_value_head + af_policy_head "
                      "(whole forward timed; af_conv_wino carries 97 % of the algorithmic FLOPs; achieved = "
                      "direct-convolution FLOPs / time, the MFMAs issued are 2.25x fewer on the 3x3 layers)",
            "peak_tflops": 157.3}


def tune(key, value):
    global _conv_mode
    lib().af_net_tune.argtypes = [C.c_int32, C.c_int32]
    _check(lib().af_net_tune(key, value), "af_net_tune")
    if key == 0:
        _conv_mode = int(value)
```

include/af_engine.h:

```cpp
#ifndef AF_ENGINE_H
#define AF_ENGINE_H

#include <stdint.h>

#ifdef __cplusplus
extern "C" {
#endif

#define AF_ABI_VERSION 6

#define AF_MODE_SELFPLAY 0
#define AF_MODE_EXTERNAL 1
#define AF_MODE_VALUE_F64 0x100

#define AF_STATUS_IDLE      0
#define AF_STATUS_NEED_EVAL 1
#define AF_STATUS_MOVE_DONE 2
#define AF_STATUS_YIELD     3

#define AF_DEFAULT_TICK_BUDGET 8
#define AF_DEFAULT_TICK_BUDGET_HARD 12

#define AF_OK 0
#define AF_ERR_ARG        (-1)
#define AF_ERR_HIP        (-2)
#define AF_ERR_NODE_CAP   (-3)
#define AF_ERR_NO_ROOT    (-4)
#define AF_ERR_EP_OVERRUN (-5)
#define AF_ERR_STATE      (-6)

typedef struct {
    int32_t board_size;
    int32_t goal;
    int32_t simulation_per_step;
    int32_t upper_simulation_per_step;
    double init_temp;
    double gamma;
    double tau_decay_rate;
    double tau_decay_rate_r;
    double dirichlet_alpha;
    double c_puct;
} af_config;

typedef struct af_engine af_engine;

int af_engine_create(const af_config* cfg, int32_t num_games, int32_t device, int32_t mode, int32_t training,
                     uint64_t seed, uint32_t first_game_id, int32_t node_cap, af_engine** out);
void af_engine_destroy(af_engine* e);

int32_t af_engine_num_games(const af_engine* e);
int32_t af_engine_cells(const af_engine* e);
int32_t af_engine_key_words(const af_engine* e);
int32_t af_engine_max_plies(const af_engine* e);

int af_engine_tick(af_engine* e, void* stream, const float* policy_dev, const float* value_dev, float* planes_dev);

int af_engine_status(af_engine* e, void* stream, int32_t* status_host);

int af_engine_set_root(af_engine* e, int32_t game, const uint64_t* key, int32_t last_cell, int32_t random_a,
                       int32_t reset_tree);
int af_engine_move_result(af_engine* e, int32_t game, int32_t* action_cell, int32_t* has_policy, float* policy,
                          int32_t* visits, double* tau);
int af_engine_set_training(af_engine* e, int32_t training);
int af_engine_set_simulations(af_engine* e, int32_t simulation_per_step, int32_t upper_simulation_per_step);

int af_engine_set_roots(af_engine* e, void* stream, int32_t n, const int32_t* games, const uint64_t* keys, const int32_t* last_cells,
                        const int32_t* random_a, const int32_t* reset_tree);
int af_engine_move_results(af_engine* e, void* stream, int32_t n, const int32_t* games, int32_t* action_cells, int32_t* has_policy,
                           float* policies, int32_t* visits, double* taus);

int64_t af_engine_pack_ints(const af_engine* e, int32_t max_episodes, int32_t max_plies);
int af_engine_pack_episodes(af_engine* e, void* stream, int32_t max_episodes, int32_t max_plies, int32_t* out);

int af_engine_pop_episodes(af_engine* e, void* stream, int32_t cap, int32_t* meta, float* final_value,
                           uint64_t* keys, float* policies, int32_t* visits, int32_t* lasts, int32_t* actions);

#define AF_NUM_COUNTERS 13
int af_engine_counters(af_engine* e, void* stream, uint64_t* out);

#define AF_MEMO_STATS 6
int af_engine_memo_enable(af_engine* e, int32_t log2_buckets, int32_t max_stones);
int af_engine_memo_insert(af_engine* e, void* stream, const float* policy_dev, const float* value_dev);
int af_engine_memo_clear(af_engine* e, void* stream);
int af_engine_memo_stats(af_engine* e, void* stream, uint64_t* out);
int64_t af_engine_memo_epoch(af_engine* e);

#define AF_HIST_WORDS 97
int af_engine_tick_histogram(af_engine* e, void* stream, uint64_t* out, int32_t reset);

int af_engine_set_tick_budget(af_engine* e, int32_t selects_per_launch);

int af_engine_progress(af_engine* e, void* stream, uint64_t* out);
int af_engine_progress_async(af_engine* e, void* stream, uint64_t* out_pinned);

#define AF_STAMP_SLOTS 64
int af_engine_stamp(af_engine* e, void* stream, int32_t slot);
int af_engine_stamps_async(af_engine* e, void* stream, uint64_t* out_pinned);

int af_engine_tree_dump(af_engine* e, int32_t game, int32_t cap, uint64_t* keys, int32_t* sum_n, int32_t* n,
                        float* w, float* p, uint8_t* f32);

int af_engine_load_tree(af_engine* e, int32_t game, int32_t count, const uint64_t* keys, const int32_t* sum_n,
                        const int32_t* n, const float* w, const float* p, const uint8_t* f32);

int af_engine_tree_w64(af_engine* e, int32_t game, int32_t cap, double* w);
int af_engine_set_tree_w64(af_engine* e, int32_t game, int32_t count, const double* w);

int af_state_to_key(const char* state, int32_t board_size, uint64_t* key);
int af_key_to_state(const uint64_t* key, int32_t board_size, char* out, int32_t cap);

const char* af_strerror(int code);
int af_abi_version(void);

#ifdef __cplusplus
}
#endif
#endif
```

include/af_net.h:

```cpp
#ifndef AF_NET_H
#define AF_NET_H

#include <stdint.h>

#ifdef __cplusplus
extern "C" {
#endif

typedef struct af_net af_net;

#define AF_NET_OK 0
#define AF_NET_ERR_ARG   (-1)
#define AF_NET_ERR_HIP   (-2)
#define AF_NET_ERR_NAME  (-3)
#define AF_NET_ERR_STATE (-4)

int af_net_create(int32_t board_size, int32_t max_batch, int32_t device, af_net** out);
void af_net_destroy(af_net* n);

int af_net_set_variable(af_net* n, const char* tf_name, const float* host_data, int64_t count);
int af_net_finalize(af_net* n);

int af_net_forward(af_net* n, void* stream, const float* planes_dev, int32_t batch, float* policy_dev, float* value_dev);

int af_net_tune(int32_t key, int32_t value);

int af_net_debug_activation(af_net* n, int32_t which, int32_t batch, float* host_out);

int af_net_small_forward_error(af_net* n);

int64_t af_net_flops_per_position(const af_net* n);
const char* af_net_strerror(int code);

#ifdef __cplusplus
}
#endif
#endif
```

Before: 5974.

## Skip network evaluation for games not needing eval via device live mask

Binds the engine's per-game status buffer into the conv net so the stem, trunk layers and corner kernels skip batch positions whose status differs from NEED_EVAL. Layer kernels build a wave ballot of live positions and iterate and prefetch only those, returning early when none remain. It also defers Dirichlet noise and PUCT scoring in the engine until after the root random pick, so that work is skipped when a cell is already chosen, and it refactors stamped graph capture. The goal is to stop spending convolution work on idle or finished games, at the cost of a mask load and extra control flow per block.

```diff
diff --git a/alphafive_amd/csrc/af_conv_f16s.h b/alphafive_amd/csrc/af_conv_f16s.h
--- a/alphafive_amd/csrc/af_conv_f16s.h
+++ b/alphafive_amd/csrc/af_conv_f16s.h
@@ -21,6 +21,7 @@
 int f16s_small_forward(f16s_net* n, hipStream_t st, const float* planes_dev, int batch, float* value, float* policy);
 int f16s_small_forward_error(f16s_net* n);
 void f16s_set_ablation(f16s_net* n, int bits);
+void f16s_set_live(f16s_net* n, const int32_t* live_dev, int32_t live_value);
 int f16s_read_activation(f16s_net* n, int which, int batch, float* host);
 
 #endif
diff --git a/alphafive_amd/csrc/af_conv_f16s.hip b/alphafive_amd/csrc/af_conv_f16s.hip
--- a/alphafive_amd/csrc/af_conv_f16s.hip
+++ b/alphafive_amd/csrc/af_conv_f16s.hip
@@ -198,6 +198,8 @@
     int* df_done;
     int* df_err;
     int abl;
+    const int32_t* live;
+    int32_t live_value;
 };
 
 template <class G, int NSM, int NSP, int CT, int KS, int PS, bool OUT32, bool XACC, int PJ, int HD, int DIST, int WPE, int NTW, int HSEL, int FU = 0, int DF = 0>
@@ -259,11 +261,30 @@
         else glds16(src + offh + lane * 16, (uint32_t)__builtin_amdgcn_readfirstlane((int)(lds + kLds0 + slot_off + offl)));
     };
     const int q0 = qpos;
+    const int npass = (nq - q0 + gxw - 1) / gxw;
+    const bool filt = DF == 0 && A.live != nullptr && npass <= 64;
+    unsigned long long lmask = 0ull;
+    if (filt) {
+        const int qi = q0 + lane * gxw;
+        const bool in = lane < npass;
+        int word = 0;
+        if (in) word = A.live[(HV == 1 || HSEL >= 0) ? qi : qi / HV];
+        lmask = __ballot(in && word == A.live_value);
+        if (lmask == 0ull) return;
+    }
+    auto ahead = [&](int i, unsigned long long r, int d) -> int {
+        if (!filt) return i + d < npass ? i + d : -1;
+        for (int k = 1; k < d; ++k) r &= r - 1ull;
+        return r ? (int)__builtin_ctzll(r) : -1;
+    };
+    const int ipos0 = filt ? (int)__builtin_ctzll(lmask) : 0;
+    const unsigned long long rem0 = filt ? (lmask & (lmask - 1ull)) : 0ull;
     auto stream_src = [&](uint32_t idx) -> const char* {
-        const int p = q0 + (int)(idx / SPP) * gxw, j = (int)(idx % SPP);
-        return slab_src(p, j);
+        const int k = (int)(idx / SPP), j = (int)(idx % SPP);
+        const int i = k == 0 ? ipos0 : ahead(ipos0, rem0, k);
+        return slab_src(q0 + i * gxw, j);
     };
-    const uint32_t nslabs = (uint32_t)((nq - q0 + gxw - 1) / gxw) * SPP;
+    const uint32_t nslabs = (uint32_t)(filt ? __popcll(lmask) : npass) * SPP;
 
     if (DF == 0) {
 #pragma unroll
@@ -446,7 +467,10 @@
 #ifdef AF_F16S_TIMING
     unsigned long long tacc[8] = {0, 0, 0, 0, 0, 0, 0, 0};
 #endif
-    for (; qpos < nq; qpos += gxw) {
+    int ipos = ipos0;
+    unsigned long long rem = rem0;
+    for (; ipos >= 0; ipos = ahead(ipos, rem, 1), rem &= rem - 1ull) {
+        qpos = q0 + ipos * gxw;
         const int pos = (HV == 1 || HSEL >= 0) ? qpos : qpos / HV;
         AF_T(tp0);
         if (!XPOS) { AF_FIRST_ITEM(cur) }
@@ -475,8 +499,9 @@
             const int NI = proj ? ITP : ITM;
             const int ibase = proj ? pslab * ITP : NSP * ITP + ms * ITM;
             const int seq = proj ? NSM * ITM + pslab * ITP : ms * ITM;
-            const int npos = qpos + ((j + kDist) / SPP) * gxw;
-            const bool more = npos < nq && !(A.abl & 1);
+            const int nidx = (j + kDist) / SPP == 0 ? ipos : ahead(ipos, rem, (j + kDist) / SPP);
+            const int npos = q0 + nidx * gxw;
+            const bool more = nidx >= 0 && !(A.abl & 1);
             const char* nsrc = slab_src((A.abl & 4) ? q0 : (more ? npos : qpos), (j + kDist) % SPP);
             const uint32_t nx1 = cur + kSlotL == kRing * kSlotL ? 0u : cur + kSlotL;
             uint32_t bC[NT], bL[NT], bR[NT];
@@ -806,6 +831,8 @@
     char* out;
     float inv_scale;
     int batch, NCT;
+    const int32_t* live;
+    int32_t live_value;
 };
 template <class G, int KS, bool XACC, int NSM, int NSP>
 __global__ __launch_bounds__(256) void af_corner_f16s(CornerArgs A) {
@@ -886,6 +913,7 @@
         for (int r = 0; r < 16; ++r) acc[0][r] = acc[KS - 1][r] + acc[0][r];
     }
     if (!valid) return;
+    if (A.live != nullptr && A.live[p] != A.live_value) return;
     float v[16];
 #pragma unroll
     for (int r = 0; r < 16; r += 2) {
@@ -968,7 +996,8 @@
 template <class G, bool SC1 = false>
 __device__ __forceinline__ void f16s_stem_body(const float* __restrict__ planes, const uint4* __restrict__ w ,
                                                const float* __restrict__ bias, float inv_scale, char* __restrict__ out, int batch,
-                                               const int bx, const int gx, uint4* ent, _Float16* img) {
+                                               const int bx, const int gx, uint4* ent, _Float16* img,
+                                               const int32_t* __restrict__ live = nullptr, const int32_t live_value = 0) {
     constexpr int S = G::S, NPIX = G::NPIX, SR = S + 4, IW = S + 5;
     constexpr int NPL = 3 * NPIX, NLD = (NPL + 255) / 256;
     constexpr int NTL = (NPIX + 31) / 32, NRND = (NTL + 3) / 4;
@@ -996,16 +1025,20 @@
         if (i < NPL && bx < batch) nx[q] = planes[(size_t)bx * NPL + i];
     }
     for (int pos = bx; pos < batch; pos += gx) {
-        __syncthreads();
-#pragma unroll
-        for (int q = 0; q < NLD; ++q)
-            if ((int)threadIdx.x + 256 * q < NPL) img[at[q]] = (_Float16)nx[q];
+        const bool idle = live != nullptr && live[pos] != live_value;
+        if (!idle) {
+            __syncthreads();
+#pragma unroll
+            for (int q = 0; q < NLD; ++q)
+                if ((int)threadIdx.x + 256 * q < NPL) img[at[q]] = (_Float16)nx[q];
+        }
         if (pos + gx < batch) {
             const float* pl = planes + (size_t)(pos + gx) * NPL;
 #pragma unroll
             for (int q = 0; q < NLD; ++q)
                 if ((int)threadIdx.x + 256 * q < NPL) nx[q] = pl[threadIdx.x + 256 * q];
         }
+        if (idle) continue;
         __syncthreads();
         for (int en = threadIdx.x; en < 3 * SR * S; en += 256) {
             const int cin = en / (SR * S), rem = en - cin * SR * S, yy = rem / S, x = rem - yy * S;
@@ -1057,10 +1090,11 @@
 
 template <class G>
 __global__ __launch_bounds__(256) void af_stem_mfma_f16s(const float* __restrict__ planes, const uint4* __restrict__ w, const float* __restrict__ bias,
-                                                         float inv_scale, char* __restrict__ out, int batch) {
+                                                         float inv_scale, char* __restrict__ out, int batch,
+                                                         const int32_t* __restrict__ live, int32_t live_value) {
     __shared__ __attribute__((aligned(16))) uint4 ent[StemLds<G>::kEnt];
     __shared__ _Float16 img[StemLds<G>::kImg];
-    f16s_stem_body<G>(planes, w, bias, inv_scale, out, batch, (int)blockIdx.x, (int)gridDim.x, ent, img);
+    f16s_stem_body<G>(planes, w, bias, inv_scale, out, batch, (int)blockIdx.x, (int)gridDim.x, ent, img, live, live_value);
 }
 
 template <class G>
@@ -1639,7 +1673,7 @@
     FS_HIP_OK(hipGetLastError());
     CornerArgs c;
     c.stash = a.stash; c.w = a.w; c.bias = a.bias; c.out = a.out; c.inv_scale = a.inv_scale;
-    c.batch = a.batch; c.NCT = gy * CT;
+    c.batch = a.batch; c.NCT = gy * CT; c.live = a.live; c.live_value = a.live_value;
     hipLaunchKernelGGL((af_corner_f16s<G, KS, XACC, NSM, NSP>), dim3((a.batch + 31) / 32, (c.NCT + 3) / 4), dim3(256), 0, st, c);
     FS_HIP_OK(hipGetLastError());
     return 0;
@@ -1668,6 +1702,8 @@
     float* pfx = nullptr;
     char* stash = nullptr;
     int abl = 0;
+    const int32_t* live = nullptr;
+    int32_t live_value = 0;
 };
 
 int f16s_supported(int board_size) { return board_size == 11 || board_size == 15; }
@@ -1823,6 +1859,7 @@
     delete n;
 }
 
+void f16s_set_live(f16s_net* n, const int32_t* live, int32_t live_value) { if (n) { n->live = live; n->live_value = live_value; } }
 void f16s_set_ablation(f16s_net* n, int bits) { if (n) n->abl = bits; }
 
 template <class G>
@@ -1864,6 +1901,7 @@
     if (head >= 0) { a.hw = n->hcw[head]; a.hbias = n->hcb[head]; a.hx = n->hx[head]; a.inv_scale_h = n->hc_inv[head]; }
     a.in = in; a.in2 = in2; a.w = n->w[li]; a.bias = n->bias[li]; a.out = out; a.out32 = out32;
     a.inv_scale = n->inv_scale[li]; a.batch = batch; a.WP = WP; a.PP = PP; a.abl = (n->abl & 0xf0ff) | (li << 8); a.gx0 = 0; a.stash = n->stash;
+    a.live = batch > kSmallBatch ? n->live : nullptr; a.live_value = n->live_value;
     {
         static const int mask = [] { const char* e = getenv("AF_F16S_ABL_LAYERS"); return e ? (int)strtol(e, nullptr, 0) : 0x3ff; }();
         if (!((mask >> li) & 1)) a.abl &= ~0x100f;
@@ -1875,15 +1913,16 @@
 
 int f16s_trunk(f16s_net* n, hipStream_t st, const float* planes, int batch) {
     if (!n || batch < 1 || batch > n->max_batch) return -1;
+    const int32_t* live = batch > kSmallBatch ? n->live : nullptr;
     if (n->abl & 16) {
         if (n->S == 15) hipLaunchKernelGGL(af_stem_f16s<Geo<15>>, dim3(std::min(batch, 2048)), dim3(256), 0, st, planes, n->stem_w, n->stem_b, n->f0, batch);
         else hipLaunchKernelGGL(af_stem_f16s<Geo<11>>, dim3(std::min(batch, 2048)), dim3(256), 0, st, planes, n->stem_w, n->stem_b, n->f0, batch);
     } else if (n->S == 15) {
         hipLaunchKernelGGL(af_stem_mfma_f16s<Geo<15>>, dim3(std::min(batch, 1024)), dim3(256), 0, st, planes, n->stem_wm, n->stem_b, n->stem_inv_scale,
-                           n->f0, batch);
+                           n->f0, batch, live, n->live_value);
     } else {
         hipLaunchKernelGGL(af_stem_mfma_f16s<Geo<11>>, dim3(std::min(batch, 1024)), dim3(256), 0, st, planes, n->stem_wm, n->stem_b, n->stem_inv_scale,
-                           n->f0, batch);
+                           n->f0, batch, live, n->live_value);
     }
     int rc = launch_layer(n, st, 0, n->f0, nullptr, n->g[0], nullptr, batch, 0, 0);
     if (!rc) rc = launch_layer(n, st, 1, n->g[0], n->f0, n->o[0], nullptr, batch, 0, 0);
@@ -1900,6 +1939,7 @@
     a.w2 = n->w[li + 1]; a.bias2 = n->bias[li + 1]; a.inv_scale2 = n->inv_scale[li + 1];
     a.hw = n->hcw[head]; a.hbias = n->hcb[head]; a.hx = n->hx[head]; a.inv_scale_h = n->hc_inv[head];
     a.batch = batch; a.abl = (n->abl & 0xf0ff) | (li << 8); a.stash = n->stash;
+    a.live = batch > kSmallBatch ? n->live : nullptr; a.live_value = n->live_value;
     return a;
 }
 
@@ -1950,6 +1990,7 @@
     memset(&P, 0, sizeof(P));
     P.in = n->o[1]; P.w = n->w[6]; P.bias = n->bias[6]; P.out = n->g[3]; P.inv_scale = n->inv_scale[6];
     P.batch = batch; P.abl = (n->abl & 0xf0ff) | (6 << 8); P.stash = n->stash; P.inv_scale2 = 1.0f; P.inv_scale_h = 1.0f;
+    P.live = small ? nullptr : n->live; P.live_value = n->live_value;
     const F16sArgs V = block_args(n, 4, n->o[1], batch, 0);
     constexpr size_t ldsP = Lds<G, kDist>::kScrOff + (size_t)2 * 1 * 4 * 4096;
     constexpr size_t ldsV = Lds<G, 2>::kScrOff + (size_t)2 * 2 * 4096 * 2 + 36864;
@@ -1977,6 +2018,7 @@
         memset(&Q, 0, sizeof(Q));
         Q.in = n->g[3]; Q.in2 = n->o[1]; Q.w = n->w[7]; Q.bias = n->bias[7]; Q.out = n->o[3]; Q.inv_scale = n->inv_scale[7];
         Q.batch = batch; Q.abl = (n->abl & 0xf0ff) | (7 << 8); Q.stash = n->stash; Q.inv_scale2 = 1.0f; Q.inv_scale_h = 1.0f;
+        Q.live = small ? nullptr : n->live; Q.live_value = n->live_value;
         const VfcArgs F = {n->hx[0], n->hfw[0], n->hfb[0], n->v2w, n->v2b, n->hf_inv[0], value};
         constexpr size_t lds7 = Lds<G, kDist>::kScrOff + (size_t)2 * 1 * 4 * 4096;
         static std::atomic<uint64_t> attr7{0};
diff --git a/alphafive_amd/csrc/af_engine.hip b/alphafive_amd/csrc/af_engine.hip
--- a/alphafive_amd/csrc/af_engine.hip
+++ b/alphafive_amd/csrc/af_engine.hip
@@ -844,109 +844,6 @@
                 ww[k] = r_w[k];
                 pp[k] = r_p[k];
             }
-            double dd[KW];
-            if (P.training) {
-#ifdef AF_TICK_TIMING
-                int tk_myit = 0;
-#endif
-                {
-                    const float a_ = (float)P.alpha, inv_a = 1.0f / a_, one_m_a = 1.0f - a_;
-                    uint32_t todo = 0;
-#pragma unroll
-                    for (int k = 0; k < KW; ++k) { dd[k] = 0.0; todo |= ((legal[k] >> lane) & 1ull) ? (1u << k) : 0u; }
-                    af_u32x4 rk[KW];
-                    uint32_t pend = 0;
-#pragma unroll
-                    for (int k = 0; k < KW; ++k) {
-                        rk[k] = af_philox4x32(sel_id, episode, (AF_STREAM_GAMMA << 24) | (uint32_t)(lane + 64 * k), 0u, k0, k1);
-                        float X;
-                        const int ok = af_gamma_round(a_, inv_a, one_m_a, rk[k].v[0], rk[k].v[1], &X);
-                        const bool lg = (todo >> k) & 1u;
-                        dd[k] = (lg && ok) ? (double)X : 0.0;
-                        pend |= (lg && !ok) ? (1u << k) : 0u;
-                        if (KW > 2 && (k & 1)) __builtin_amdgcn_sched_barrier(0);
-                    }
-#ifdef AF_TICK_TIMING
-                    ++tk_myit;
-#endif
-                    todo = pend;
-                    {
-                    uint32_t it = 1;
-                    af_u32x4 r = rk[0];
-#pragma unroll
-                    for (int q = 1; q < KW; ++q) if (!(todo & ((1u << q) - 1u))) r = rk[q];
-                    while (todo) {
-#ifdef AF_TICK_TIMING
-                        ++tk_myit;
-#endif
-                        const int k = __builtin_ctz(todo);
-                        if ((it & 1u) == 0u) r = af_philox4x32(sel_id, episode, (AF_STREAM_GAMMA << 24) | (uint32_t)(lane + 64 * k), it >> 1, k0, k1);
-                        const uint32_t wu = (it & 1u) ? r.v[2] : r.v[0], wv = (it & 1u) ? r.v[3] : r.v[1];
-                        float X;
-                        const int ok = af_gamma_round(a_, inv_a, one_m_a, wu, wv, &X);
-                        if (ok || it == 0xFFFFu) {
-                            const double Xd = ok ? (double)X : 0.0;
-#pragma unroll
-                            for (int q = 0; q < KW; ++q) dd[q] = q == k ? Xd : dd[q];
-                            todo &= todo - 1u;
-                            it = 1;
-#pragma unroll
-                            for (int q = 1; q < KW; ++q) if (todo && !(todo & ((1u << q) - 1u))) r = rk[q];
-                        } else {
-                            ++it;
-                        }
-                    }
-                    }
-                }
-#ifdef AF_TICK_TIMING
-                tk[12] += (unsigned long long)wave_max_i32(tk_myit);
-#endif
-                TK_T(tk_n1);
-                TK_ACC(8, tk_b, tk_n1);
-                double acc = 0.0;
-#pragma unroll
-                for (int k = 0; k < KW; ++k) acc = k == 0 ? dd[0] : acc + dd[k];
-                acc = wave_sum_f64_tree(acc);
-                if (acc == 0.0) {
-                    int cnt = 0;
-#pragma unroll
-                    for (int k = 0; k < KW; ++k) cnt += __popcll(legal[k]);
-                    const double u = 1.0 / (double)cnt;
-#pragma unroll
-                    for (int k = 0; k < KW; ++k) dd[k] = ((legal[k] >> lane) & 1ull) ? u : 0.0;
-                } else {
-                    const double inv = 1.0 / acc;
-#pragma unroll
-                    for (int k = 0; k < KW; ++k) dd[k] = dd[k] * inv;
-                }
-                TK_T(tk_n1e);
-                TK_ACC(9, tk_n1, tk_n1e);
-            }
-            TK_T(tk_n2);
-            const double sq = sqrt((double)(sum_n + 1));
-            float sc[KW];
-            float mx = -3.0e38f;
-#pragma unroll
-            for (int k = 0; k < KW; ++k) {
-                const bool lg = (legal[k] >> lane) & 1ull;
-                double q64;
-                if (nn[k] == 0) q64 = 0.0;
-                else if (!W64 && ff[k]) q64 = (double)((float)ww[k] / (float)nn[k]);
-                else q64 = (double)ww[k] / (double)nn[k];
-                double t;
-                if (P.training) {
-                    double p_;
-                    if (is_root) p_ = (double)(0.75f * pp[k]) + 0.25 * dd[k];
-                    else p_ = (double)(0.9f * pp[k]) + 0.1 * dd[k];
-                    t = ((P.c_puct * p_) * sq) / (double)(1 + nn[k]);
-                } else {
-                    t = ((double)(P.c_puct32 * pp[k]) * sq) / (double)(1 + nn[k]);
-                }
-                sc[k] = lg ? (float)(q64 + t) : -3.0e38f;
-                mx = sc[k] > mx ? sc[k] : mx;
-            }
-            TK_T(tk_n3);
-            TK_ACC(10, tk_n2, tk_n3);
             int cell = -1;
             if (is_root && P.training) {
                 u64 cand[KW];
@@ -960,7 +857,116 @@
                 }
                 if (m > 0) cell = bb_select_wave<KW>(cand, (int)af_pick((uint32_t)m, sel_id, episode, AF_STREAM_PICK, k0, k1), lane);
             }
+            cell = rfli(cell);
+#ifdef AF_TICK_TIMING
+            unsigned long long tk_n3 = __builtin_readcyclecounter();
+#endif
             if (cell < 0) {
+                double dd[KW];
+                if (P.training) {
+#ifdef AF_TICK_TIMING
+                    int tk_myit = 0;
+#endif
+                    {
+                        const float a_ = (float)P.alpha, inv_a = 1.0f / a_, one_m_a = 1.0f - a_;
+                        uint32_t todo = 0;
+#pragma unroll
+                        for (int k = 0; k < KW; ++k) { dd[k] = 0.0; todo |= ((legal[k] >> lane) & 1ull) ? (1u << k) : 0u; }
+                        af_u32x4 rk[KW];
+                        uint32_t pend = 0;
+#pragma unroll
+                        for (int k = 0; k < KW; ++k) {
+                            rk[k] = af_philox4x32(sel_id, episode, (AF_STREAM_GAMMA << 24) | (uint32_t)(lane + 64 * k), 0u, k0, k1);
+                            float X;
+                            const int ok = af_gamma_round(a_, inv_a, one_m_a, rk[k].v[0], rk[k].v[1], &X);
+                            const bool lg = (todo >> k) & 1u;
+                            dd[k] = (lg && ok) ? (double)X : 0.0;
+                            pend |= (lg && !ok) ? (1u << k) : 0u;
+                            if (KW > 2 && (k & 1)) __builtin_amdgcn_sched_barrier(0);
+                        }
+#ifdef AF_TICK_TIMING
+                        ++tk_myit;
+#endif
+                        todo = pend;
+                        {
+                        uint32_t it = 1;
+                        af_u32x4 r = rk[0];
+#pragma unroll
+                        for (int q = 1; q < KW; ++q) if (!(todo & ((1u << q) - 1u))) r = rk[q];
+                        while (todo) {
+#ifdef AF_TICK_TIMING
+                            ++tk_myit;
+#endif
+                            const int k = __builtin_ctz(todo);
+                            if ((it & 1u) == 0u) r = af_philox4x32(sel_id, episode, (AF_STREAM_GAMMA << 24) | (uint32_t)(lane + 64 * k), it >> 1, k0, k1);
+                            const uint32_t wu = (it & 1u) ? r.v[2] : r.v[0], wv = (it & 1u) ? r.v[3] : r.v[1];
+                            float X;
+                            const int ok = af_gamma_round(a_, inv_a, one_m_a, wu, wv, &X);
+                            if (ok || it == 0xFFFFu) {
+                                const double Xd = ok ? (double)X : 0.0;
+#pragma unroll
+                                for (int q = 0; q < KW; ++q) dd[q] = q == k ? Xd : dd[q];
+                                todo &= todo - 1u;
+                                it = 1;
+#pragma unroll
+                                for (int q = 1; q < KW; ++q) if (todo && !(todo & ((1u << q) - 1u))) r = rk[q];
+                            } else {
+                                ++it;
+                            }
+                        }
+                        }
+                    }
+#ifdef AF_TICK_TIMING
+                    tk[12] += (unsigned long long)wave_max_i32(tk_myit);
+#endif
+                    TK_T(tk_n1);
+                    TK_ACC(8, tk_b, tk_n1);
+                    double acc = 0.0;
+#pragma unroll
+                    for (int k = 0; k < KW; ++k) acc = k == 0 ? dd[0] : acc + dd[k];
+                    acc = wave_sum_f64_tree(acc);
+                    if (acc == 0.0) {
+                        int cnt = 0;
+#pragma unroll
+                        for (int k = 0; k < KW; ++k) cnt += __popcll(legal[k]);
+                        const double u = 1.0 / (double)cnt;
+#pragma unroll
+                        for (int k = 0; k < KW; ++k) dd[k] = ((legal[k] >> lane) & 1ull) ? u : 0.0;
+                    } else {
+                        const double inv = 1.0 / acc;
+#pragma unroll
+                        for (int k = 0; k < KW; ++k) dd[k] = dd[k] * inv;
+                    }
+                    TK_T(tk_n1e);
+                    TK_ACC(9, tk_n1, tk_n1e);
+                }
+                TK_T(tk_n2);
+                const double sq = sqrt((double)(sum_n + 1));
+                float sc[KW];
+                float mx = -3.0e38f;
+#pragma unroll
+                for (int k = 0; k < KW; ++k) {
+                    const bool lg = (legal[k] >> lane) & 1ull;
+                    double q64;
+                    if (nn[k] == 0) q64 = 0.0;
+                    else if (!W64 && ff[k]) q64 = (double)((float)ww[k] / (float)nn[k]);
+                    else q64 = (double)ww[k] / (double)nn[k];
+                    double t;
+                    if (P.training) {
+                        double p_;
+                        if (is_root) p_ = (double)(0.75f * pp[k]) + 0.25 * dd[k];
+                        else p_ = (double)(0.9f * pp[k]) + 0.1 * dd[k];
+                        t = ((P.c_puct * p_) * sq) / (double)(1 + nn[k]);
+                    } else {
+                        t = ((double)(P.c_puct32 * pp[k]) * sq) / (double)(1 + nn[k]);
+                    }
+                    sc[k] = lg ? (float)(q64 + t) : -3.0e38f;
+                    mx = sc[k] > mx ? sc[k] : mx;
+                }
+#ifdef AF_TICK_TIMING
+                tk_n3 = __builtin_readcyclecounter();
+#endif
+                TK_ACC(10, tk_n2, tk_n3);
                 mx = wave_max_f32(mx);
                 u64 cand[KW];
 #pragma unroll
@@ -1413,6 +1419,12 @@
     HIP_OK(hipMemcpyAsync(status_host, e->P.status, (size_t)e->P.G * 4, hipMemcpyDeviceToHost, st));
     HIP_OK(hipStreamSynchronize(st));
     for (int g = 0; g < e->P.G; ++g) if (status_host[g] < 0) return status_host[g];
+    return AF_OK;
+}
+
+int af_engine_status_dev(af_engine* e, const int32_t** status_dev) {
+    if (!e || !status_dev) return AF_ERR_ARG;
+    *status_dev = e->P.status;
     return AF_OK;
 }
 
diff --git a/alphafive_amd/csrc/af_net.hip b/alphafive_amd/csrc/af_net.hip
--- a/alphafive_amd/csrc/af_net.hip
+++ b/alphafive_amd/csrc/af_net.hip
@@ -533,6 +533,11 @@
     float *vc_w, *vc_b, *v1_w, *v1_b, *v2_w, *v2_b, *pc_w, *pc_b, *pf_w, *pf_b;
     float *f0, *g[5], *o[5];
     f16s_net* f16s = nullptr;
+    const int32_t* live = nullptr;
+    int32_t live_value = 0, live_batch = 0;
+    const float* live_planes = nullptr;
+    const float *live_pol = nullptr, *live_val = nullptr;
+    bool live_primed = false;
 };
 
 static int pad32(int c) { return (c + 31) / 32 * 32; }
@@ -651,6 +656,7 @@
     n->allocs.clear();
     f16s_destroy(n->f16s);
     n->f16s = nullptr;
+    n->live_primed = false;
     if (f16s_supported(n->S) && f16s_create(&n->f16s, n->S, n->max_batch, n->device, n->vars) != 0) return AF_NET_ERR_HIP;
     auto& V = n->vars;
     int rc = AF_NET_OK;
@@ -721,8 +727,16 @@
     for (int i = 0; i < 5; ++i) { g[i] = n->g[i] + po * kBlocks[i].cout; o[i] = n->o[i] + po * kBlocks[i].cout; }
     const bool split16 = g_wino == 5 && n->f16s != nullptr;
     const bool fhead = split16 && g_fhead;
+    bool masked = false;
+    if (split16 && n->live && b0 == 0 && planes_all == n->live_planes && batch == n->live_batch) {
+        masked = n->live_primed && policy_all == n->live_pol && value_all == n->live_val && !(g_f16s_abl & 0x8000);
+        n->live_primed = true; n->live_pol = policy_all; n->live_val = value_all;
+    } else {
+        n->live_primed = false;
+    }
     if (split16) {
         f16s_set_ablation(n->f16s, g_f16s_abl);
+        f16s_set_live(n->f16s, masked ? n->live : nullptr, n->live_value);
         if (fhead && f16s_small_forward_ok(n->f16s, batch)) {
             if (f16s_small_forward(n->f16s, st, planes, batch, value, policy)) return AF_NET_ERR_HIP;
             return AF_NET_OK;
@@ -791,6 +805,14 @@
     return forward_range(n, (hipStream_t)stream, planes, 0, batch, policy, value);
 }
 
+int af_net_set_live_mask(af_net* n, const int32_t* status_dev, int32_t live_value, const float* planes_dev, int32_t batch) {
+    if (!n || (status_dev && (!planes_dev || batch < 1 || batch > n->max_batch))) return AF_NET_ERR_ARG;
+    n->live = status_dev; n->live_value = live_value;
+    n->live_planes = status_dev ? planes_dev : nullptr; n->live_batch = status_dev ? batch : 0;
+    n->live_pol = nullptr; n->live_val = nullptr; n->live_primed = false;
+    return AF_NET_OK;
+}
+
 int af_net_tune(int32_t key, int32_t value) {
     if (key == 0) { if (value != 1 && value != 5) return AF_NET_ERR_ARG; g_wino = value; return AF_NET_OK; }
     if (key == 5) { g_phead = value; return AF_NET_OK; }
diff --git a/alphafive_amd/engine.py b/alphafive_amd/engine.py
--- a/alphafive_amd/engine.py
+++ b/alphafive_amd/engine.py
@@ -74,6 +74,7 @@
         L.af_engine_progress_async.argtypes = [vp, vp, vp]
         L.af_engine_stamp.argtypes = [vp, vp, C.c_int32]
         L.af_engine_stamps_async.argtypes = [vp, vp, vp]
+        L.af_engine_status_dev.argtypes = [vp, C.POINTER(vp)]
         L.af_engine_tick_histogram.argtypes = [vp, vp, u64p, C.c_int32]
         L.af_engine_set_tick_budget.argtypes = [vp, C.c_int32]
         L.af_engine_memo_enable.argtypes = [vp, C.c_int32, C.c_int32]
@@ -156,6 +157,11 @@
         rc = lib().af_engine_status(self._h, stream, _p(self._status, C.c_int32))
         _check(rc, "engine status")
         return self._status
+
+    def status_dev(self):
+        p = C.c_void_p()
+        _check(lib().af_engine_status_dev(self._h, C.byref(p)), "af_engine_status_dev")
+        return int(p.value)
 
     def params_key(self):
         p = self._params
@@ -335,7 +341,7 @@
 class SelfPlayEngine:
 
     def __init__(self, cfg, num_games, pv_device, device=0, seed=0, first_game_id=0, training=True, node_cap=0,
-                 value_f64=False, weights_version=None, eval_memo=None):
+                 value_f64=False, weights_version=None, eval_memo=None, live_mask=True):
         import torch
         if not torch.cuda.is_available():
             raise EngineError("SelfPlayEngine needs a HIP device (torch.cuda.is_available() is False)")
@@ -354,6 +360,10 @@
         self._weights_version = self._resolve_weights_version(weights_version)
         if hasattr(pv_device, "bind_outputs"):
             pv_device.bind_outputs(self.policy, self.value)
+        self._live_mask_ptr = None
+        if live_mask and hasattr(pv_device, "bind_live_mask"):
+            self._live_mask_ptr = self.engine.status_dev()
+            pv_device.bind_live_mask(self._live_mask_ptr, STATUS_NEED_EVAL, self.planes)
         self._memo_version = None
         if eval_memo:
             if self._weights_version is None:
@@ -430,20 +440,8 @@
                 self._graph_stamped = None
                 if self._graph is None or self._graph[0] != key:
                     self.run_ticks_graph(n)
-                if self._stamp_host is None:
-                    self._stamp_host = torch.zeros(STAMP_SLOTS, dtype=torch.int64, pin_memory=True)
-                    self._stamp_event = torch.cuda.Event()
-                    self.engine.stamp(0, torch.cuda.current_stream(self.dev).cuda_stream)
-                torch.cuda.synchronize(self.dev)
-                g = torch.cuda.CUDAGraph()
-                with torch.cuda.graph(g, capture_error_mode="thread_local"):
-                    for i in range(n):
-                        self.tick(stamp_base=3 * i)
-                    st = torch.cuda.current_stream(self.dev).cuda_stream
-                    self.engine.stamps_async(self._stamp_host.data_ptr(), st)
-                    self.engine.progress_async(self._prog_host.data_ptr(), st)
-                self.ticks -= n
-                self._graph_stamped = (self._graph_key(n), g, n)
+                if self._graph_stamped is None or self._graph_stamped[0] != key:
+                    self._capture_stamped(n)
             if self._stamp_pending:
                 self._collect_stamps()
             self._graph_stamped[1].replay()
@@ -469,6 +467,8 @@
                 self.engine.progress_async(self._prog_host.data_ptr(), st)
             self.ticks -= n
             self._graph = (self._graph_key(n), g)
+            if 3 * n <= STAMP_SLOTS:
+                self._capture_stamped(n)
         if timed:
             e0, e1 = torch.cuda.Event(enable_timing=True), torch.cuda.Event(enable_timing=True)
             e0.record(torch.cuda.current_stream(self.dev))
@@ -481,6 +481,26 @@
         self._prog_events[self._prog_turn].record(torch.cuda.current_stream(self.dev))
         self._prog_replays += 1
 
+    def _capture_stamped(self, n):
+        torch = self.torch
+        if self._stamp_pending:
+            self._collect_stamps()
+        self._graph_stamped = None
+        if self._stamp_host is None:
+            self._stamp_host = torch.zeros(STAMP_SLOTS, dtype=torch.int64, pin_memory=True)
+            self._stamp_event = torch.cuda.Event()
+            self.engine.stamp(0, torch.cuda.current_stream(self.dev).cuda_stream)
+        torch.cuda.synchronize(self.dev)
+        g = torch.cuda.CUDAGraph()
+        with torch.cuda.graph(g, capture_error_mode="thread_local"):
+            for i in range(n):
+                self.tick(stamp_base=3 * i)
+            st = torch.cuda.current_stream(self.dev).cuda_stream
+            self.engine.stamps_async(self._stamp_host.data_ptr(), st)
+            self.engine.progress_async(self._prog_host.data_ptr(), st)
+        self.ticks -= n
+        self._graph_stamped = (self._graph_key(n), g, n)
+
     def _collect_stamps(self):
         self._stamp_event.synchronize()
         t = self._stamp_host.numpy().astype(np.int64)[:3 * self._graph_stamped[2]].reshape(-1, 3)
@@ -557,4 +577,14 @@
         return [assemble_episode(r, self.S, self.cfg.gamma) for r in self.pop_raw(cap)]
 
     def close(self):
-        self.engine.close()
+        if getattr(self, "_live_mask_ptr", None) is not None:
+            try:
+                self.pv_device.unbind_live_mask(self._live_mask_ptr)
+            except Exception:
+                pass
+            self._live_mask_ptr = None
+        self._graph = self._graph_stamped = None
+        if getattr(self, "engine", None) is not None:
+            self.engine.close()
+
+    __del__ = close
diff --git a/alphafive_amd/net_hip.py b/alphafive_amd/net_hip.py
--- a/alphafive_amd/net_hip.py
+++ b/alphafive_amd/net_hip.py
@@ -30,6 +30,7 @@
         L.af_net_flops_per_position.argtypes = [vp]
         L.af_net_flops_per_position.restype = C.c_int64
         L.af_net_small_forward_error.argtypes = [vp]
+        L.af_net_set_live_mask.argtypes = [vp, vp, C.c_int32, vp, C.c_int32]
         L.af_net_strerror.argtypes = [C.c_int]
         L.af_net_strerror.restype = C.c_char_p
         _lib = L
@@ -71,6 +72,14 @@
         assert policy.shape[0] >= self.max_batch or policy.shape[0] == value.shape[0]
         self.policy, self.value = policy, value
 
+    def set_live_mask(self, status_ptr, live_value=1, planes=None):
+        if not status_ptr:
+            _check(lib().af_net_set_live_mask(self._h, None, 0, None, 0), "af_net_set_live_mask")
+            return
+        assert planes.is_contiguous() and planes.dtype == torch.float32 and planes.shape[0] <= self.max_batch
+        _check(lib().af_net_set_live_mask(self._h, int(status_ptr), int(live_value), planes.data_ptr(), planes.shape[0]),
+               "af_net_set_live_mask")
+
     def __call__(self, planes):
         B = planes.shape[0]
         assert B <= self.max_batch and planes.is_contiguous() and planes.dtype == torch.float32
@@ -97,7 +106,7 @@
     if resnet.device.type != "cuda" or not (3 <= resnet.board_size <= 15):
         return None
     lib()
-    state = {"net": None, "out": None, "version": None}
+    state = {"net": None, "out": None, "version": None, "mask": None}
 
     def pv(planes):
         B = planes.shape[0]
@@ -108,6 +117,8 @@
             state["version"] = getattr(resnet, "version", None)
             if state["out"] is not None and state["out"][0].shape[0] >= B:
                 state["net"].bind_outputs(*state["out"])
+            if state["mask"] is not None and state["mask"][2].shape[0] <= B:
+                state["net"].set_live_mask(*state["mask"])
         elif state["version"] != getattr(resnet, "version", None):
             state["net"].load(resnet.variables)
             state["version"] = getattr(resnet, "version", None)
@@ -118,12 +129,25 @@
         if state["net"] is not None and policy.shape[0] >= state["net"].max_batch:
             state["net"].bind_outputs(policy, value)
 
+    def bind_live_mask(status_ptr, live_value, planes):
+        state["mask"] = (status_ptr, live_value, planes)
+        if state["net"] is not None and planes.shape[0] <= state["net"].max_batch:
+            state["net"].set_live_mask(status_ptr, live_value, planes)
+
+    def unbind_live_mask(status_ptr):
+        if state["mask"] is not None and state["mask"][0] == status_ptr:
+            state["mask"] = None
+            if state["net"] is not None:
+                state["net"].set_live_mask(None)
+
     def close():
         if state["net"] is not None:
             state["net"].close()
             state["net"] = None
 
     pv.bind_outputs = bind_outputs
+    pv.bind_live_mask = bind_live_mask
+    pv.unbind_live_mask = unbind_live_mask
     pv.close = close
     pv.weights_version = lambda: getattr(resnet, "version", None)
     return pv
diff --git a/include/af_engine.h b/include/af_engine.h
--- a/include/af_engine.h
+++ b/include/af_engine.h
@@ -97,6 +97,8 @@
 int af_engine_stamp(af_engine* e, void* stream, int32_t slot);
 int af_engine_stamps_async(af_engine* e, void* stream, uint64_t* out_pinned);
 
+int af_engine_status_dev(af_engine* e, const int32_t** status_dev);
+
 int af_engine_tree_dump(af_engine* e, int32_t game, int32_t cap, uint64_t* keys, int32_t* sum_n, int32_t* n,
                         float* w, float* p, uint8_t* f32);
 
diff --git a/include/af_net.h b/include/af_net.h
--- a/include/af_net.h
+++ b/include/af_net.h
@@ -23,6 +23,8 @@
 
 int af_net_forward(af_net* n, void* stream, const float* planes_dev, int32_t batch, float* policy_dev, float* value_dev);
 
+int af_net_set_live_mask(af_net* n, const int32_t* status_dev, int32_t live_value, const float* planes_dev, int32_t batch);
+
 int af_net_tune(int32_t key, int32_t value);
 
 int af_net_debug_activation(af_net* n, int32_t which, int32_t batch, float* host_out);
```

Result: no change. 6011 (median of 6 runs) (+0.6%).
